# olFi95/image_search

Hardware: AMD Instinct MI355X
Metric: images/sec embedded (ViT-L/14 b=256) + queries/sec cosine top-10 over 10M x 768 (higher is better)
Workload: dtype bf16; 1 GPU; BASELINE config 4: per step, H2D of a pinned batch of 256 224x224x3 f32 images -> bf16 ViT-L/14 (random-init seeded weights) -> 256 rows appended to the table on the device -> cosine top-10 query over 10000000+ x 768 fp32 rows per GPU -> D2H of the k results; fused on HIP streams (the upload runs under the previous batch's tower; the scan is asynchronous to the host and runs between towers); query; batch=256, rows_per_gpu=10000000, k=10

## Files before the change

image_search_amd/_lib.py:

```python
from __future__ import annotations

import ctypes
import os

_PKG = os.path.dirname(os.path.abspath(__file__))
LIB_PATH = os.path.join(_PKG, "libmi355clip.so")

c_f = ctypes.POINTER(ctypes.c_float)
c_u64p = ctypes.POINTER(ctypes.c_uint64)
c_u8p = ctypes.POINTER(ctypes.c_uint8)
c_vp = ctypes.c_void_p



class KnnWhere(ctypes.Structure):
    _fields_ = [("all_of", ctypes.c_uint64), ("any_of", ctypes.c_uint64), ("none_of", ctypes.c_uint64),
                ("stamp_lo", ctypes.c_int64), ("stamp_hi", ctypes.c_int64), ("group", ctypes.c_uint32), ("flags", ctypes.c_uint32)]


c_wherep = ctypes.POINTER(KnnWhere)
MI_KNN_WHERE_GROUP = 1

SYMBOLS = {
    "mi_last_error": (ctypes.c_char_p, []),
    "mi_abi_version": (ctypes.c_int, []),
    "mi_device_count": (ctypes.c_int, []),
    "mi_clip_load": (ctypes.c_int, [ctypes.c_char_p, ctypes.c_int, ctypes.c_int, ctypes.POINTER(c_vp)]),
    "mi_clip_free": (None, [c_vp]),
    "mi_weights_list": (ctypes.c_int, [ctypes.c_char_p, ctypes.c_char_p, ctypes.c_size_t, ctypes.POINTER(ctypes.c_size_t)]),
    "mi_clip_set_option": (ctypes.c_int, [c_vp, ctypes.c_char_p, ctypes.c_int]),
    "mi_clip_info": (ctypes.c_int, [c_vp, ctypes.POINTER(ctypes.c_uint32)]),
    "mi_clip_ln_fold_stats": (ctypes.c_int, [c_vp, ctypes.POINTER(ctypes.c_uint64), ctypes.c_int]),
    "mi_clip_embed": (ctypes.c_int, [c_vp, c_vp, ctypes.c_size_t, c_vp]),
    "mi_clip_embed_device": (ctypes.c_int, [c_vp, c_vp, ctypes.c_size_t, c_vp, c_vp]),
    "mi_clip_embed_rgb8": (ctypes.c_int, [c_vp, c_vp, ctypes.c_size_t, c_vp]),
    "mi_clip_load_text": (ctypes.c_int, [ctypes.c_char_p, ctypes.c_int, ctypes.c_int, ctypes.POINTER(c_vp)]),
    "mi_clip_embed_text": (ctypes.c_int, [c_vp, c_vp, ctypes.c_size_t, c_vp]),
    "mi_preprocess_rgb8": (ctypes.c_int, [c_vp, ctypes.c_size_t, ctypes.c_uint32, ctypes.c_uint32, c_vp]),
    "mi_resize_catmullrom_rgb8": (ctypes.c_int, [ctypes.c_int, c_vp, ctypes.c_uint32, ctypes.c_uint32, ctypes.c_uint32,
                                                 ctypes.c_uint32, c_vp]),
    "mi_image_prepare_resnet": (ctypes.c_int, [ctypes.c_int, c_vp, ctypes.c_uint32, ctypes.c_uint32, c_vp]),
    "mi_clip_embed_images": (ctypes.c_int, [c_vp, ctypes.POINTER(c_vp), ctypes.POINTER(ctypes.c_uint32),
                                            ctypes.POINTER(ctypes.c_uint32), ctypes.c_size_t, c_vp]),
    "mi_knn_create": (ctypes.c_int, [ctypes.c_uint32, ctypes.c_int, ctypes.POINTER(c_vp)]),
    "mi_knn_free": (None, [c_vp]),
    "mi_knn_set_base": (ctypes.c_int, [c_vp, ctypes.c_uint64]),
    "mi_knn_set_option": (ctypes.c_int, [c_vp, ctypes.c_char_p, ctypes.c_int]),
    "mi_knn_prefilter_stats": (ctypes.c_int, [c_vp, c_vp, c_vp]),
    "mi_knn_prefilter_state": (ctypes.c_int, [c_vp, ctypes.POINTER(ctypes.c_uint32)]),
    "mi_knn_reserve": (ctypes.c_int, [c_vp, ctypes.c_uint64]),
    "mi_knn_size": (ctypes.c_int, [c_vp, c_u64p]),
    "mi_knn_append": (ctypes.c_int, [c_vp, c_vp, ctypes.c_uint64]),
    "mi_knn_append_device": (ctypes.c_int, [c_vp, c_vp, ctypes.c_uint64, c_vp]),
    "mi_knn_append_synthetic": (ctypes.c_int, [c_vp, ctypes.c_uint64, ctypes.c_uint64, ctypes.c_uint64]),
    "mi_knn_get_rows": (ctypes.c_int, [c_vp, ctypes.c_uint64, ctypes.c_uint64, c_vp]),
    "mi_knn_save": (ctypes.c_int, [c_vp, ctypes.c_char_p]),
    "mi_knn_load": (ctypes.c_int, [c_vp, ctypes.c_char_p]),
    "mi_knn_delete": (ctypes.c_int, [c_vp, c_vp, ctypes.c_uint64, c_u64p]),
    "mi_knn_deleted": (ctypes.c_int, [c_vp, c_vp, ctypes.c_uint64, c_u64p]),
    "mi_knn_search": (ctypes.c_int, [c_vp, c_vp, ctypes.c_uint32, ctypes.c_uint32, c_vp, c_vp]),
    "mi_knn_search_device": (ctypes.c_int, [c_vp, c_vp, ctypes.c_uint32, ctypes.c_uint32, c_vp, c_vp, c_vp]),
    "mi_knn_search_batched_device": (ctypes.c_int, [c_vp, c_vp, ctypes.c_uint32, ctypes.c_uint32, c_vp, c_vp, c_vp]),
    "mi_knn_search_filtered": (ctypes.c_int, [c_vp, c_vp, ctypes.c_uint32, ctypes.c_uint32, c_vp, ctypes.c_uint64, c_vp, c_vp]),
    "mi_knn_near_pairs": (ctypes.c_int, [c_vp, ctypes.c_float, ctypes.c_uint64, c_vp, c_vp, c_vp, ctypes.c_uint64, c_u64p]),
    "mi_knn_near_pairs_stats": (ctypes.c_int, [c_vp, c_u64p]),
    "mi_knn_assign": (ctypes.c_int, [c_vp, c_vp, ctypes.c_uint32, c_vp, c_vp]),
    "mi_knn_assign_stats": (ctypes.c_int, [c_vp, c_u64p]),
    "mi_knn_assign_multi": (ctypes.c_int, [c_vp, c_vp, ctypes.c_uint32, ctypes.c_uint32, ctypes.c_float, c_vp, c_vp]),
    "mi_knn_assign_multi_stats": (ctypes.c_int, [c_vp, c_u64p]),
    "mi_knn_search_many": (ctypes.c_int, [c_vp, c_vp, ctypes.c_uint32, ctypes.c_uint32, c_vp, c_vp]),
    "mi_knn_search_many_stats": (ctypes.c_int, [c_vp, c_u64p]),
    "mi_knn_neighbors": (ctypes.c_int, [c_vp, ctypes.c_uint64, ctypes.c_uint64, ctypes.c_uint32, c_vp, c_vp]),
    "mi_knn_kmeans": (ctypes.c_int, [c_vp, c_vp, ctypes.c_uint32, ctypes.c_uint32, c_vp, c_vp, ctypes.POINTER(ctypes.c_uint32),
                                     c_u64p, ctypes.POINTER(ctypes.c_double)]),
    "mi_knn_kmeans_seed": (ctypes.c_int, [c_vp, ctypes.c_uint32, ctypes.c_uint64, c_vp, ctypes.c_uint64, c_vp, c_vp,
                                          ctypes.POINTER(ctypes.c_double)]),
    "mi_knn_kmeans_seed_stats": (ctypes.c_int, [c_vp, c_u64p]),
    "mi_knn_search_diverse": (ctypes.c_int, [c_vp, c_vp, ctypes.c_uint32, ctypes.c_uint32, ctypes.c_float, c_vp, ctypes.c_uint64,
                                             c_vp, c_vp, c_vp, c_vp, ctypes.POINTER(ctypes.c_uint32)]),
    "mi_knn_search_diverse_stats": (ctypes.c_int, [c_vp, c_u64p]),
    "mi_knn_search_compound": (ctypes.c_int, [c_vp, c_vp, ctypes.c_uint32, ctypes.c_int, c_vp, c_vp, ctypes.c_uint32, ctypes.c_uint32,
                                              c_vp, ctypes.c_uint64, c_vp, c_vp, c_vp]),
    "mi_knn_search_compound_stats": (ctypes.c_int, [c_vp, c_u64p]),
    "mi_knn_search_page": (ctypes.c_int, [c_vp, c_vp, ctypes.c_uint32, ctypes.c_float, ctypes.c_uint64, ctypes.c_float, c_vp,
                                          ctypes.c_uint64, c_vp, c_vp, c_vp]),
    "mi_knn_set_groups": (ctypes.c_int, [c_vp, c_vp, ctypes.c_uint64, c_vp]),
    "mi_knn_get_groups": (ctypes.c_int, [c_vp, c_vp, ctypes.c_uint64, c_vp]),
    "mi_knn_groups_info": (ctypes.c_int, [c_vp, c_u64p]),
    "mi_knn_search_grouped": (ctypes.c_int, [c_vp, c_vp, ctypes.c_uint32, ctypes.c_float, c_vp, ctypes.c_uint64, c_vp, c_vp, c_vp, c_vp,
                                             c_vp, ctypes.c_uint64, c_vp]),
    "mi_knn_set_attrs": (ctypes.c_int, [c_vp, c_vp, ctypes.c_uint64, c_vp, c_vp]),
    "mi_knn_get_attrs": (ctypes.c_int, [c_vp, c_vp, ctypes.c_uint64, c_vp, c_vp]),
    "mi_knn_count_where": (ctypes.c_int, [c_vp, c_wherep, c_u64p]),
    "mi_knn_rows_where": (ctypes.c_int, [c_vp, c_wherep, c_vp, ctypes.c_uint64, c_u64p]),
    "mi_knn_search_where": (ctypes.c_int, [c_vp, c_vp, ctypes.c_uint32, ctypes.c_uint32, c_wherep, c_vp, c_vp, c_u64p]),
    "mi_pairs_to_groups": (ctypes.c_int, [c_vp, c_vp, ctypes.c_uint64, c_vp, ctypes.c_uint64, c_vp, ctypes.c_uint64, c_u64p,
                                          c_u64p]),
    "mi_index_duplicates": (ctypes.c_int, [c_vp, ctypes.c_float, ctypes.c_uint64, ctypes.c_uint64, c_vp, ctypes.c_uint64, c_vp,
                                           ctypes.c_uint64, c_u64p, c_u64p]),
    "mi_knn_sharded_create": (ctypes.c_int, [ctypes.c_uint32, ctypes.POINTER(ctypes.c_int), ctypes.c_int, ctypes.c_uint32,
                                             ctypes.POINTER(c_vp)]),
    "mi_knn_sharded_free": (None, [c_vp]),
    "mi_knn_sharded_info": (ctypes.c_int, [c_vp, c_u64p, ctypes.POINTER(ctypes.c_uint32), ctypes.POINTER(ctypes.c_uint32),
                                           ctypes.POINTER(ctypes.c_int)]),
    "mi_knn_sharded_stats": (ctypes.c_int, [c_vp, c_u64p]),
    "mi_knn_sharded_reserve": (ctypes.c_int, [c_vp, ctypes.c_uint64]),
    "mi_knn_sharded_set_option": (ctypes.c_int, [c_vp, ctypes.c_char_p, ctypes.c_int]),
    "mi_knn_sharded_append": (ctypes.c_int, [c_vp, c_vp, ctypes.c_uint64, c_u64p]),
    "mi_knn_sharded_append_device": (ctypes.c_int, [c_vp, c_vp, ctypes.c_uint64, ctypes.c_int, c_vp, c_u64p]),
    "mi_knn_sharded_shard": (c_vp, [c_vp, ctypes.c_uint32]),
    "mi_knn_sharded_search_async": (ctypes.c_int, [c_vp, c_vp, ctypes.c_uint32, ctypes.c_uint32, c_vp, c_vp]),
    "mi_knn_sharded_sync": (ctypes.c_int, [c_vp]),
    "mi_knn_sharded_rebalance": (ctypes.c_int, [c_vp, c_vp]),
    "mi_knn_sharded_append_synthetic": (ctypes.c_int, [c_vp, ctypes.c_uint64, ctypes.c_uint64, ctypes.c_uint64]),
    "mi_knn_sharded_get_rows": (ctypes.c_int, [c_vp, ctypes.c_uint64, ctypes.c_uint64, c_vp]),
    "mi_knn_sharded_search": (ctypes.c_int, [c_vp, c_vp, ctypes.c_uint32, ctypes.c_uint32, c_vp, c_vp]),
    "mi_knn_sharded_save": (ctypes.c_int, [c_vp, ctypes.c_char_p]),
    "mi_knn_sharded_load": (ctypes.c_int, [c_vp, ctypes.c_char_p]),
    "mi_knn_sharded_delete": (ctypes.c_int, [c_vp, c_vp, ctypes.c_uint64, c_u64p]),
    "mi_knn_sharded_deleted": (ctypes.c_int, [c_vp, c_vp, ctypes.c_uint64, c_u64p]),
    "mi_knn_sharded_search_filtered": (ctypes.c_int, [c_vp, c_vp, ctypes.c_uint32, ctypes.c_uint32, c_vp, ctypes.c_uint64, c_vp,
                                                      c_vp]),
    "mi_knn_sharded_search_compound": (ctypes.c_int, [c_vp, c_vp, ctypes.c_uint32, ctypes.c_int, c_vp, c_vp, ctypes.c_uint32,
                                                      ctypes.c_uint32, c_vp, ctypes.c_uint64, c_vp, c_vp]),
    "mi_knn_sharded_search_page": (ctypes.c_int, [c_vp, c_vp, ctypes.c_uint32, ctypes.c_float, ctypes.c_uint64, ctypes.c_float, c_vp,
                                                  ctypes.c_uint64, c_vp, c_vp, c_vp]),
    "mi_knn_sharded_set_groups": (ctypes.c_int, [c_vp, c_vp, ctypes.c_uint64, c_vp]),
    "mi_knn_sharded_get_groups": (ctypes.c_int, [c_vp, c_vp, ctypes.c_uint64, c_vp]),
    "mi_knn_sharded_groups_info": (ctypes.c_int, [c_vp, c_u64p]),
    "mi_knn_sharded_search_grouped": (ctypes.c_int, [c_vp, c_vp, ctypes.c_uint32, ctypes.c_float, c_vp, ctypes.c_uint64, c_vp, c_vp,
                                                     c_vp, c_vp, c_vp, ctypes.c_uint64, c_vp]),
    "mi_knn_sharded_set_attrs": (ctypes.c_int, [c_vp, c_vp, ctypes.c_uint64, c_vp, c_vp]),
# ... 115 lines not shown
```

image_search_amd/csrc/handles.h:

```cpp
#pragma once
#include <mutex>
#include <vector>

#include "common.h"

namespace mi {
typedef unsigned short bf16_t;

struct Layer {
    float *ln1w, *ln1b, *ln2w, *ln2b;
    void *wqkv, *wo, *w1, *w2;
    float *bqkv, *bo, *b1, *b2;
    void *wqkv_f = nullptr, *w1_f = nullptr;
    float *cqkv = nullptr, *bqkv_f = nullptr, *c1 = nullptr, *b1_f = nullptr;
};


}

struct mi_clip {
    int device = 0, precision = 0;
    int image = 0, patch = 0, grid = 0, S = 0, D = 0, L = 0, H = 0, FF = 0, E = 0, Kp = 0;
    float eps = 1e-5f;
    std::vector<void*> allocs;
// ... 40 lines not shown
    uint8_t* d_img_src[2] = {nullptr, nullptr};
    float* d_img_tmp = nullptr;
    size_t img_src_cap = 0, img_tmp_cap = 0;
    hipStream_t copy_stream = nullptr;
    hipEvent_t ev_up[2] = {nullptr, nullptr}, ev_used[2] = {nullptr, nullptr};
    hipStream_t stream = nullptr;
    size_t max_batch = 256;
    bool split_ln = false;
    int attn_ver = 2;
    bool q_prescaled = false;
    bool attn_shift = false;
    int qkv_pad = 128;
    int qkv_layout = 0;
    bool front_overlap = false;
    bool store_nt = true;
    bool attn_nt = false;
    int attn_order = 1;
    bool full_last = false;
    bool split_tail = true;
    int gemm_order = 4;
    bool text_fast = true;
    bool attn_f32_mfma = true;
    bool text_fuse = true;
    int ln_nt = 0;
    bool im2col_rows = true;
    mi::WorkOrder order;
    std::mutex mu;
};


struct mi_knn {
    int device = 0;
    uint32_t dim = 0;
    uint64_t base = 0, rows = 0, cap = 0;
    uint32_t cyc_block = 0, cyc_n = 0, cyc_rank = 0;
    float* table = nullptr;
    hipStream_t stream = nullptr;
    int n_cu = 0;
    float* d_q = nullptr;
    uint64_t* d_cand = nullptr;
    uint64_t* d_tmp = nullptr;
    uint64_t* d_keys = nullptr;
    uint64_t* d_idx = nullptr;
    float* d_dist = nullptr;
    size_t cand_keys = 0, tmp_keys = 0, keys_cap = 0, idx_cap = 0, dist_cap = 0;
    bool select_path = true;
    uint32_t* d_keys32 = nullptr;
    uint32_t* d_sel = nullptr;
    size_t keys32_cap = 0, sel_cap = 0;
    int prefilter = 0;
    int coarse_ring = 8;
    bool last_prefiltered = false;
    uint16_t* d_mirror = nullptr;
    float* d_scale8 = nullptr;
    float* d_cfac8 = nullptr;
    float* d_rho8 = nullptr;
    float* d_g8 = nullptr;
    bool g8_ready = false;
    size_t scale8_cap = 0, cfac8_cap = 0, rho8_cap = 0, g8_cap = 0;
    float* d_xx = nullptr;
    bool batch_stage1_mfma = true;
    int8_t* d_digits = nullptr;
    float* d_qs = nullptr;
    size_t digits_cap = 0, qs_cap = 0;
    int pref_sample = 1;
    uint32_t* d_skeys = nullptr;
    size_t skeys_cap = 0;
    uint64_t mirror_rows = 0;
    size_t mirror_cap = 0, xx_cap = 0;
    uint64_t g8_rows = 0;
    static constexpr int PREF_RING = 8, PREF_SKIP = 64;
    bool pref_adaptive = true;
    uint32_t* h_pref_ring = nullptr;
    hipEvent_t pref_ev[PREF_RING] = {};
    bool pref_ev_pending[PREF_RING] = {};
    uint32_t pref_consec = 0, pref_skip_left = 0;
    bool pref_probing = false;
    uint32_t pref_probes_left = 0, pref_reports_due = 0;
    uint64_t pref_seq = 0, pref_skipped = 0;
    uint32_t* d_pref_rows = nullptr;
    uint64_t* d_pref_keys = nullptr;
    uint32_t* d_pref_flag = nullptr;
    size_t pref_rows_cap = 0, pref_keys_cap = 0, pref_flag_cap = 0;
    mi::WorkOrder writes, reads;
    std::vector<uint32_t> dead;
    uint64_t* d_tomb = nullptr;
    uint32_t* d_dead = nullptr;
    size_t tomb_words = 0, dead_cap = 0;
    uint32_t* h_flist = nullptr;
    size_t n_flist = 0, h_flist_cap = 0;
    uint32_t* d_flist = nullptr;
    size_t flist_cap = 0;
    uint32_t join_cap = 1u << 22;
    uint64_t join_stats[4] = {0, 0, 0, 0};
    uint64_t assign_stats[4] = {0, 0, 0, 0};
    uint64_t assign_multi_stats[4] = {0, 0, 0, 0};
    uint64_t search_many_stats[4] = {0, 0, 0, 0};
    int many_segments = 0, many_sample = 0;
    uint64_t kmeans_seed_stats[4] = {0, 0, 0, 0};
    uint64_t diverse_stats[4] = {0, 0, 0, 0};
    uint64_t compound_stats[4] = {0, 0, 0, 0};
    int compound_blocks = 0;
    int page_blocks = 0;
    uint32_t* d_groups = nullptr;
    size_t groups_cap = 0;
    std::vector<uint32_t> h_groups;
    uint32_t n_groups = 0;
    uint64_t n_grouped = 0, groups_epoch = 0;
    uint32_t* d_gslots = nullptr;
    uint32_t* d_gwin = nullptr;
    size_t gslots_cap = 0, gwin_cap = 0;
    bool gslots_valid = false;
    uint32_t gslots_groups = 0;
    int group_blocks = 0, group_lds_max = 4096;
    uint64_t* d_tags = nullptr;
    int64_t* d_stamps = nullptr;
    size_t attrs_cap = 0;
    std::vector<uint64_t> h_tags;
    std::vector<int64_t> h_stamps;
    uint32_t* d_wcounts = nullptr;
    size_t wcounts_cap = 0;
    uint64_t* h_wtotal = nullptr;
    int where_chunk = 0;
    std::mutex mu;
};


typedef struct ncclComm* ncclComm_t;
namespace mi {
struct DevBuf {
    void* p = nullptr;
    size_t cap = 0;
    void reserve(size_t b) {
        if (b <= cap) return;
        if (p) HIP_CHECK(hipFree(p));
        p = nullptr; cap = 0;
        HIP_CHECK(hipMalloc(&p, b));
        cap = b;
    }
};
struct PinnedBuf2 {
    void* p = nullptr;
    size_t cap = 0;
    void reserve(size_t b) {
        if (b <= cap) return;
        if (p) HIP_CHECK(hipHostFree(p));
        p = nullptr; cap = 0;
        HIP_CHECK(hipHostMalloc(&p, b, hipHostMallocPortable));
        cap = b;
    }
};
struct ShardedSlot {
    std::vector<DevBuf> d_q, d_rec;
    std::vector<DevBuf> g_rec;
    DevBuf m_rec;
    PinnedBuf2 h_q, h_rec;
    std::vector<hipEvent_t> ev;
    hipEvent_t done = nullptr;
    uint32_t nq = 0, k = 0;
    uint64_t* user_idx = nullptr;
    float* user_dist = nullptr;
    bool busy = false;
};
}

struct mi_knn_sharded {
    static constexpr int N_SLOTS = 8;
    uint32_t dim = 0, block = 0;
    uint64_t rows = 0;
    std::vector<int> devices;
    std::vector<mi_knn*> shard;
    mi::ShardedSlot slots[N_SLOTS];
    int next_slot = 0;
    std::vector<ncclComm_t> comms;
    bool use_rccl = false;
    struct { uint64_t searches = 0, collectives = 0, copies = 0, merges = 0; } stats;
    uint64_t generation = 0;
    std::vector<hipEvent_t> ev_src;
    std::mutex mu;
    uint32_t n() const { return (uint32_t)shard.size(); }
};

namespace mi {
hipStream_t clip_own_stream(mi_clip* m);
void clip_ensure_workspace(mi_clip* m, size_t n);
void clip_ensure_copy_stream(mi_clip* m);
void clip_forward(mi_clip* m, const float* d_img, size_t n, float* d_out, hipStream_t s, hipStream_t front = nullptr);
hipStream_t knn_own_stream(mi_knn* t);
void knn_grow(mi_knn* t, uint64_t want_rows);
void knn_search_one(mi_knn* t, const float* d_q, uint32_t k, uint64_t* d_idx, float* d_dist, hipStream_t s);
void knn_search_many(mi_knn* t, const float* d_q, uint32_t nq, uint32_t k, uint64_t* d_idx, float* d_dist, hipStream_t s);
void knn_truncate(mi_knn* t, uint64_t rows);
void knn_search_filtered_many(mi_knn* t, const float* d_q, uint32_t nq, uint32_t k, const uint64_t* ids, uint64_t n_ids,
                              uint64_t* d_idx, float* d_dist, hipStream_t s);
void knn_reserve(mi_knn* t, void** p, size_t* have, size_t want, size_t elem);
void knn_filter_rows(mi_knn* t, const uint64_t* ids, uint64_t n_ids);
void knn_filter_upload(mi_knn* t, hipStream_t s);
void knn_filtered_many(mi_knn* t, const float* d_q, uint32_t nq, uint32_t k, uint64_t* d_idx, float* d_dist, hipStream_t s);
void knn_reduce_lists64(mi_knn* t, uint32_t lists, uint32_t k, uint64_t* keys_out, hipStream_t s);
void knn_select_keys32(mi_knn* t, uint64_t n, uint32_t k, uint64_t* keys_out, const uint32_t* list, hipStream_t s);
void knn_merge_lists_device(const uint64_t* d_idx_in, const float* d_dist_in, uint32_t lists, uint32_t nq, uint32_t k,
                            size_t idx_stride, size_t dist_stride, uint64_t* d_idx, float* d_dist, hipStream_t s);
void knn_search_compound(mi_knn* t, const float* pos, uint32_t n_pos, int mode, const float* neg, const float* neg_within, uint32_t n_neg,
                         uint32_t k, const uint64_t* among, uint64_t n_among, uint64_t* idx, float* dist, float* term_dist);
void knn_search_page(mi_knn* t, const float* q, uint32_t k, bool cursor_is_id, float after_dist, uint64_t after_id, uint64_t first_key,
                     float max_dist, const uint64_t* among, uint64_t n_among, uint64_t* idx, float* dist, uint64_t* counts);
void knn_page_scan_keys32(mi_knn* t, hipStream_t s, uint64_t n, const uint32_t* list, const uint64_t* tomb, uint64_t hi, uint32_t k,
                          uint32_t* keys32, unsigned long long* counts);
void knn_groups_fit(mi_knn* t);
void knn_search_grouped(mi_knn* t, const float* q, uint32_t k, float max_dist, const uint64_t* among, uint64_t n_among, uint64_t* idx,
                        float* dist, uint32_t* group, uint64_t* members, uint64_t* facets, uint64_t cap_facets, uint64_t* totals,
                        std::vector<uint32_t>* cnt_out);
void knn_grouped_members(mi_knn* t, const uint32_t* group, uint32_t k, uint32_t* out);
void knn_attrs_fit(mi_knn* t);
void knn_filter_where(mi_knn* t, const mi_knn_where* w, hipStream_t s);
void sharded_place(const mi_knn_sharded* t, uint64_t r, uint32_t* s, uint64_t* local);
uint64_t sharded_rows_of(const mi_knn_sharded* t, uint64_t total, uint32_t s);
void sharded_search_enqueue(mi_knn_sharded* t, const float* q, uint32_t nq, uint32_t k, uint64_t* idx, float* dist,
                            const std::vector<std::vector<uint64_t>>* filter = nullptr,
                            const mi_knn_where* where = nullptr);
void sharded_deliver_all(mi_knn_sharded* t);
}
```

image_search_amd/csrc/knn.hip:

```cpp
#include <algorithm>
#include <cmath>
#include <cstdio>
#include <cstring>
#include <unistd.h>

#include <iterator>
#include <mutex>
#include <string>
#include <vector>

#include "common.h"
#include "handles.h"
#include "knn_kernels.h"
#include "where_host.h"

using namespace mi;

namespace {

constexpr int MAX_BATCH_Q = 8;

IdMap id_map(const mi_knn* t) { return IdMap{t->base, t->cyc_block, t->cyc_n, t->cyc_rank}; }

void ensure(mi_knn* t, void** p, size_t* have, size_t want, size_t elem) {
// ... 113 lines not shown
    const uint64_t off = id - t->base;
    uint64_t l = off;
    if (t->cyc_n > 1 && t->cyc_block) {
        const uint64_t b = off / t->cyc_block;
        if (b % t->cyc_n != t->cyc_rank) return false;
        l = (b / t->cyc_n) * t->cyc_block + off % t->cyc_block;
    }
    if (l >= t->rows) return false;
    *local = l;
    return true;
}

void grow(mi_knn* t, uint64_t want_rows) {
    if (want_rows <= t->cap) return;
    uint64_t ncap = std::max<uint64_t>(want_rows, t->cap + t->cap / 2);
    ncap = (ncap + 63) & ~63ull;
    if (ncap > 0xFFFFFFFFull) fail(MI_ERR_UNSUPPORTED, "a shard holds at most 2^32-1 rows (asked %llu)",
                                    (unsigned long long)want_rows);
    t->writes.sync();
    t->reads.sync();
    float* nt = nullptr;
    HIP_CHECK(hipMalloc((void**)&nt, ncap * t->dim * sizeof(float)));
    if (t->rows) {
        HIP_CHECK(hipMemcpyAsync(nt, t->table, t->rows * t->dim * sizeof(float), hipMemcpyDeviceToDevice, own_stream(t)));
        HIP_CHECK(hipStreamSynchronize(t->stream));
    }
    if (t->table) HIP_CHECK(hipFree(t->table));
    t->table = nt;
    t->cap = ncap;
    if (t->d_tomb) tomb_fit(t);
    if (t->d_groups) groups_fit(t);
    if (t->d_tags) attrs_fit(t);
}

template <class K>
void allow_lds(K kernel, size_t bytes) {
    if (bytes > 48 * 1024)
        HIP_CHECK(hipFuncSetAttribute(reinterpret_cast<const void*>(kernel),
                                      hipFuncAttributeMaxDynamicSharedMemorySize, (int)bytes));
}

template <class Top>
void launch_scan(mi_knn* t, const float* d_q, uint32_t k, const uint64_t* lo, uint64_t* cand, uint32_t blocks,
                 hipStream_t s, const uint32_t* run_if = nullptr, uint32_t gy = 1, QGroup qg = QGroup{}) {
    const size_t lds = (size_t)4 * Top::LDS_KEYS * sizeof(uint64_t);
    const uint64_t* tomb = tomb_of(t);
    switch (t->dim / 64) {
#define MI_CASE(NCH)                                                                                   \
    case NCH:                                                                                          \
        if (tomb) {                                                                                    \
            allow_lds(knn_scan_kernel<NCH, Top, 0, true>, lds);                                        \
            hipLaunchKernelGGL((knn_scan_kernel<NCH, Top, 0, true>), dim3(blocks, gy), dim3(256), lds, s, \
                               t->table, t->rows, d_q, k, lo, cand, (uint32_t*)nullptr, run_if, qg, tomb); \
            break;                                                                                     \
        }                                                                                              \
        allow_lds(knn_scan_kernel<NCH, Top>, lds);                                                     \
        hipLaunchKernelGGL((knn_scan_kernel<NCH, Top>), dim3(blocks, gy), dim3(256), lds, s, t->table, \
                           t->rows, d_q, k, lo, cand, (uint32_t*)nullptr, run_if, qg);                 \
        break;
        MI_CASE(1) MI_CASE(2) MI_CASE(4) MI_CASE(8) MI_CASE(12) MI_CASE(16)
#undef MI_CASE
        default: fail(MI_ERR_UNSUPPORTED, "dim %u: built for dim/64 in {1,2,4,8,12,16}", t->dim);
    }
    HIP_CHECK(hipGetLastError());
}

template <class Top>
void launch_merge(const uint64_t* in, uint32_t n_lists, uint32_t k, uint32_t lpb, uint64_t* out, uint32_t nq,
                  size_t in_stride, size_t out_stride, hipStream_t s, const uint32_t* run_if = nullptr, uint32_t run_stride = 0) {
    const size_t lds = (size_t)4 * Top::LDS_KEYS * sizeof(uint64_t);
    allow_lds(knn_merge_kernel<Top>, lds + 4096);
    const uint32_t blocks = (n_lists + lpb - 1) / lpb;
    hipLaunchKernelGGL((knn_merge_kernel<Top>), dim3(blocks, nq), dim3(256), lds, s, in, n_lists, k, lpb, out,
                       in_stride, out_stride, run_if, run_stride);
    HIP_CHECK(hipGetLastError());
}

template <class Top>
void reduce_wave_lists(mi_knn* t, uint32_t lists, uint32_t kp, uint64_t* keys_out, hipStream_t s, const uint32_t* run_if,
                       uint32_t gy, const QGroup& qg);

template <class Top>
void one_pass(mi_knn* t, const float* d_q, uint32_t kp, const uint64_t* lo, uint64_t* keys_out, hipStream_t s,
              const uint32_t* run_if = nullptr, uint32_t gy = 1, QGroup qg = QGroup{}) {
    const uint32_t bpc = Top::LDS_KEYS == 0 ? 4 : (Top::KP <= 256 ? 4 : 2);
    const uint64_t n_tiles = (t->rows + 63) / 64;
    uint32_t blocks = (uint32_t)std::min<uint64_t>((uint64_t)t->n_cu * bpc, (n_tiles + 3) / 4);
    blocks = std::max(blocks, 1u);
    const uint32_t lists = blocks * 4;
    ensure(t, (void**)&t->d_cand, &t->cand_keys, (size_t)lists * kp * gy, sizeof(uint64_t));
    qg.lists = (uint64_t)lists * kp;
    launch_scan<Top>(t, d_q, kp, lo, t->d_cand, blocks, s, run_if, gy, qg);
    reduce_wave_lists<Top>(t, lists, kp, keys_out, s, run_if, gy, qg);
}

template <class Top>
void reduce_wave_lists(mi_knn* t, uint32_t lists, uint32_t kp, uint64_t* keys_out, hipStream_t s, const uint32_t* run_if,
                       uint32_t gy, const QGroup& qg) {
    if constexpr (Top::LDS_KEYS != 0) {
        constexpr uint32_t LPB = 16;
        ensure(t, (void**)&t->d_tmp, &t->tmp_keys, (size_t)2 * ((lists + LPB - 1) / LPB) * kp, sizeof(uint64_t));
        const uint64_t* in = t->d_cand;
        uint32_t n = lists, lvl = 0;
        while (true) {
            const uint32_t nb = (n + LPB - 1) / LPB;
            uint64_t* out = nb == 1 ? keys_out : t->d_tmp + (size_t)(lvl & 1) * ((lists + LPB - 1) / LPB) * kp;
            hipLaunchKernelGGL((knn_merge_block_kernel<Top::KP>), dim3(nb), dim3(256), 0, s, in, n, kp, LPB, out);
            HIP_CHECK(hipGetLastError());
            if (nb == 1) break;
            in = out; n = nb; ++lvl;
        }
        return;
    }
    if (lists <= 64) {
        launch_merge<Top>(t->d_cand, lists, kp, lists, keys_out, gy, qg.lists, qg.out, s, run_if, qg.flags);
    } else {
        const uint32_t lpb = 32, mid = (lists + lpb - 1) / lpb;
        ensure(t, (void**)&t->d_tmp, &t->tmp_keys, (size_t)mid * kp * gy, sizeof(uint64_t));
        launch_merge<Top>(t->d_cand, lists, kp, lpb, t->d_tmp, gy, qg.lists, (size_t)mid * kp, s, run_if, qg.flags);
        launch_merge<Top>(t->d_tmp, mid, kp, mid, keys_out, gy, (size_t)mid * kp, qg.out, s, run_if, qg.flags);
    }
}

constexpr uint64_t PREF_MIN_ROWS = 1u << 18;
bool prefilter_applies(const mi_knn* t, uint32_t k) {
    const uint32_t width = t->prefilter == 2 ? 256u : 128u;
    return t->prefilter && (k <= 64 || (k <= 4096 && t->select_path)) && t->dim % width == 0 && t->rows >= PREF_MIN_ROWS;
}
template <int NCH>
void launch_coarse8_batched(mi_knn* t, const uint8_t* m8, const float* d_q, float e0, uint32_t nq, uint32_t blocks, hipStream_t s,
                            int sample_shift = 0, uint64_t sample_stride = 0) {
    if constexpr (NCH == 12) {
        if (t->batch_stage1_mfma) {
            hipLaunchKernelGGL(knn_query_digits_kernel, dim3(nq), dim3(256), 0, s, d_q, t->d_g8, (int)t->dim, t->d_digits, t->d_qs, t->d_rho8);
            constexpr int LDS = c8m_lds_bytes(NCH * 64);
            const uint64_t n_tiles = (t->rows + 15) / 16;
            const uint32_t grid = (uint32_t)std::max<uint64_t>(1, std::min<uint64_t>((uint64_t)t->n_cu, (n_tiles + 3) / 4));
#define MI_C8M(NBLK, QPB)                                                                                                         \
    {                                                                                                                             \
        allow_lds(knn_scan_coarse8_mfma_kernel<NCH, NBLK, QPB>, LDS);                                                             \
        hipLaunchKernelGGL((knn_scan_coarse8_mfma_kernel<NCH, NBLK, QPB>), dim3(grid), dim3(256), LDS, s, m8, t->d_xx, t->d_scale8, \
                           t->d_cfac8, t->rows, t->d_digits, t->d_qs, (int)nq, e0, t->d_keys32, (uint64_t)t->cap,                 \
                           sample_shift ? t->d_skeys : (uint32_t*)nullptr, sample_shift, sample_stride);                          \
    }
            if (nq <= 5) MI_C8M(1, 5)
            else if (nq <= 10) MI_C8M(2, 5)
            else if (nq <= 15) MI_C8M(3, 5)
            else MI_C8M(4, 4)
#undef MI_C8M
            HIP_CHECK(hipGetLastError());
            return;
        }
        if (nq == 8)
            hipLaunchKernelGGL((knn_scan_coarse8_batched_kernel<NCH, 8>), dim3(blocks), dim3(256), 0, s, m8, t->d_xx, t->d_scale8, t->d_cfac8,
                               t->d_g8, t->rows, d_q, e0, t->d_keys32, (uint64_t)t->cap, t->d_rho8);
        else if (nq == 2)
            hipLaunchKernelGGL((knn_scan_coarse8_batched_kernel<NCH, 2>), dim3(blocks), dim3(256), 0, s, m8, t->d_xx, t->d_scale8, t->d_cfac8,
                               t->d_g8, t->rows, d_q, e0, t->d_keys32, (uint64_t)t->cap, t->d_rho8);
        else
            hipLaunchKernelGGL((knn_scan_coarse8_batched_kernel<NCH, 4>), dim3(blocks), dim3(256), 0, s, m8, t->d_xx, t->d_scale8, t->d_cfac8,
                               t->d_g8, t->rows, d_q, e0, t->d_keys32, (uint64_t)t->cap, t->d_rho8);
    } else {
        fail(MI_ERR_UNSUPPORTED, "the batched two-stage search is built for dim 768");
    }
}
constexpr uint32_t SEL_WORDS = 6 * SEL_BINS + 64;
constexpr uint32_t KNN_GROUP_MAX = 16;
uint32_t group_size(const mi_knn* t, uint32_t left) {
    if (t->batch_stage1_mfma) return std::min(left, KNN_GROUP_MAX);
    return left >= 8 ? 8 : left >= 4 ? 4 : 2;
}
QGroup group_of(const mi_knn* t, uint32_t gy) {
    QGroup g;
    if (gy <= 1) return g;
    g.q = t->dim; g.keys = t->cap; g.sel = SEL_WORDS; g.flags = 4; g.rows = (uint64_t)2 * PREF_CAP; g.coll = 4096; g.out = 4096; g.rho = 1;
    return g;
}
uint32_t* prefilter_pass(mi_knn* t, const float* d_q, uint32_t k, hipStream_t s, uint32_t nq_batch = 0) {
    const uint32_t gy = std::max(1u, nq_batch);
    const QGroup qg = group_of(t, gy);
    ensure(t, (void**)&t->d_keys32, &t->keys32_cap, (size_t)t->cap * gy, sizeof(uint32_t));
    ensure(t, (void**)&t->d_sel, &t->sel_cap, (size_t)SEL_WORDS * gy, sizeof(uint32_t));
    ensure(t, (void**)&t->d_cand, &t->cand_keys, (size_t)4096 * gy, sizeof(uint64_t));
    ensure(t, (void**)&t->d_pref_rows, &t->pref_rows_cap, (size_t)2 * PREF_CAP * gy, sizeof(uint32_t));
    ensure(t, (void**)&t->d_pref_keys, &t->pref_keys_cap, (size_t)4096 * gy, sizeof(uint64_t));
    ensure(t, (void**)&t->d_pref_flag, &t->pref_flag_cap, (size_t)4 * gy, sizeof(uint32_t));
    const bool bytes = t->prefilter == 2;
    const uint32_t tile_rows = (nq_batch && t->batch_stage1_mfma) ? 16 : 64;
    const uint64_t n_tiles_s = (t->rows + tile_rows - 1) / tile_rows;
    int sample_shift = (bytes && t->pref_sample && k <= 64 && ((nq_batch >= 2 && t->batch_stage1_mfma) || (nq_batch == 0 && t->pref_sample >= 2))) ? 3 : 0;
    uint64_t n_sample = ((n_tiles_s + (1u << sample_shift) - 1) >> sample_shift) * tile_rows;
    if (sample_shift && (t->rows >> sample_shift) < std::max<uint64_t>(4096, 64ull * k)) { sample_shift = 0; n_sample = 0; }
    const uint64_t sample_stride = sample_shift ? ((((t->cap + tile_rows - 1) / tile_rows + (1u << sample_shift) - 1) >> sample_shift) * tile_rows + 63) / 64 * 64 : 0;
    if (sample_shift) ensure(t, (void**)&t->d_skeys, &t->skeys_cap, (size_t)sample_stride * gy, sizeof(uint32_t));
    const size_t mirror_elems = bytes ? ((size_t)t->cap * t->dim + 1) / 2 : (size_t)t->cap * t->dim;
    t->mirror_rows = std::min(t->mirror_rows, t->rows);
    if (bytes && t->g8_ready && t->rows >= 4 * std::max<uint64_t>(t->g8_rows, 1)) t->g8_ready = false;
    if (bytes && !t->g8_ready) t->mirror_rows = 0;
    const size_t keep_m = bytes ? ((size_t)t->mirror_rows * t->dim + 1) / 2 : (size_t)t->mirror_rows * t->dim;
    ensure_keep(t, (void**)&t->d_mirror, &t->mirror_cap, mirror_elems, sizeof(uint16_t), keep_m);
    ensure_keep(t, (void**)&t->d_xx, &t->xx_cap, (size_t)t->cap, sizeof(float), (size_t)t->mirror_rows);
    if (bytes) {
        ensure_keep(t, (void**)&t->d_scale8, &t->scale8_cap, (size_t)t->cap, sizeof(float), (size_t)t->mirror_rows);
        ensure_keep(t, (void**)&t->d_cfac8, &t->cfac8_cap, (size_t)t->cap, sizeof(float), (size_t)t->mirror_rows);
        ensure(t, (void**)&t->d_rho8, &t->rho8_cap, (size_t)KNN_GROUP_MAX, sizeof(float));
        ensure(t, (void**)&t->d_digits, &t->digits_cap, (size_t)KNN_GROUP_MAX * 3 * t->dim + 64, sizeof(int8_t));
        ensure(t, (void**)&t->d_qs, &t->qs_cap, (size_t)KNN_GROUP_MAX * 4, sizeof(float));
        ensure(t, (void**)&t->d_g8, &t->g8_cap, (size_t)2 * t->dim, sizeof(float));
        if (!t->g8_ready) {
            const uint64_t sample = std::min<uint64_t>(t->rows, 1u << 16), stride = t->rows / sample;
            HIP_CHECK(hipMemsetAsync(t->d_g8 + t->dim, 0, t->dim * sizeof(float), s));
            hipLaunchKernelGGL(knn_channel_sumsq_kernel, dim3(256), dim3(256), 0, s, t->table, sample, stride, (int)t->dim, t->d_g8 + t->dim);
            hipLaunchKernelGGL(knn_channel_scale_kernel, dim3((t->dim + 255) / 256), dim3(256), 0, s, t->d_g8 + t->dim, sample,
                               (int)t->dim, t->d_g8);
            t->g8_ready = true;
            t->g8_rows = t->rows;
        }
    }
    const uint64_t n_tiles = (t->rows + 63) / 64;
    const uint32_t blocks = std::max<uint32_t>(1u, (uint32_t)std::min<uint64_t>((uint64_t)t->n_cu * 4, (n_tiles + 3) / 4));
    const uint32_t hb1 = (uint32_t)std::min<uint64_t>((uint64_t)t->n_cu * 8, (t->rows + 255) / 256);
    const uint32_t hb = std::max<uint32_t>(std::min<uint32_t>(hb1, (uint32_t)t->n_cu), (hb1 + gy - 1) / gy);
    uint32_t* flags = t->d_pref_flag;
    uint32_t* key32 = t->d_pref_rows + PREF_CAP;
    uint32_t* count2 = t->d_sel + 6 * SEL_BINS;
    SelState* states = reinterpret_cast<SelState*>(t->d_sel + 6 * SEL_BINS + 4);
    const size_t sel_bytes = (size_t)SEL_WORDS * gy * sizeof(uint32_t);
    HIP_CHECK(hipMemsetAsync(t->d_sel, 0, sel_bytes, s));
    HIP_CHECK(hipMemsetAsync(flags, 0, (size_t)4 * gy * sizeof(uint32_t), s));
    static const uint32_t ring8_bpc = [] { const char* e = std::getenv("MI_KNN_RING_BPC"); return e ? (uint32_t)std::max(1, std::atoi(e)) : 2u; }();
    const float e0 = 4.1f * (float)(t->dim + 8) * 0x1p-24f + 2e-6f;
    const float eps = 0x1p-8f + e0;
    const uint64_t* tomb = tomb_of(t);
    auto kill_keys = [&] {
        if (!tomb) return;
        const uint32_t nd = (uint32_t)t->dead.size();
        hipLaunchKernelGGL(knn_tomb_keys_kernel, dim3(std::max(1u, std::min<uint32_t>((nd + 255) / 256, (uint32_t)t->n_cu * 4))), dim3(256), 0, s,
                           t->d_dead, nd, t->rows, t->d_keys32, (uint64_t)t->cap, gy, sample_shift ? t->d_skeys : (uint32_t*)nullptr,
                           sample_stride, sample_shift, tile_rows);
    };
    if (bytes) {
        uint8_t* m8 = reinterpret_cast<uint8_t*>(t->d_mirror);
        const uint32_t* keys_q = t->d_keys32;
        const uint32_t* keys_h = sample_shift ? t->d_skeys : keys_q;
        const uint64_t n_h = sample_shift ? n_sample : t->rows;
        QGroup qgh = qg;
        if (sample_shift && gy > 1) qgh.keys = sample_stride;
        const uint32_t hbh = sample_shift ? std::max<uint32_t>(1u, (uint32_t)std::min<uint64_t>(hb, (n_h + 1023) / 1024)) : hb;
        switch (t->dim / 64) {
#define MI_CASE(NCH)                                                                                                     \
    case NCH:                                                                                                            \
        if (t->mirror_rows < t->rows) {                                                                                  \
            const uint64_t todo = t->rows - t->mirror_rows;                                                              \
            const uint32_t mb = (uint32_t)std::min<uint64_t>((uint64_t)t->n_cu * 8, (todo + 15) / 16);                   \
            hipLaunchKernelGGL((knn_mirror8_kernel<NCH>), dim3(std::max(mb, 1u)), dim3(256), 0, s, t->table, t->mirror_rows, \
                               t->rows, t->d_g8, m8, t->d_xx, t->d_scale8, t->d_cfac8);                                  \
            t->mirror_rows = t->rows;                                                                                    \
        }                                                                                                                \
        if (nq_batch == 0 && t->coarse_ring == 8)   \
            hipLaunchKernelGGL((knn_scan_coarse8_kernel<NCH, 8>), dim3(std::min(blocks, (uint32_t)t->n_cu * ring8_bpc)), dim3(256), 0, s, m8, t->d_xx, t->d_scale8, \
                               t->d_cfac8, t->d_g8, t->rows, d_q, e0, t->d_keys32, t->d_rho8,                            \
                               sample_shift ? t->d_skeys : (uint32_t*)nullptr, sample_shift);                            \
        else if (nq_batch == 0)                                                                                          \
            hipLaunchKernelGGL((knn_scan_coarse8_kernel<NCH, 4>), dim3(blocks), dim3(256), 0, s, m8, t->d_xx, t->d_scale8, \
                               t->d_cfac8, t->d_g8, t->rows, d_q, e0, t->d_keys32, t->d_rho8,                            \
                               sample_shift ? t->d_skeys : (uint32_t*)nullptr, sample_shift);                            \
        else                                                                                                             \
            launch_coarse8_batched<NCH>(t, m8, d_q, e0, nq_batch, blocks, s, sample_shift, sample_stride);               \
        kill_keys();                                                                                                     \
        for (int p = 0; p < 3; ++p)                                                                                      \
            hipLaunchKernelGGL(knn_select_hist_kernel, dim3(hbh, gy), dim3(256), 0, s, keys_h, n_h, k, p, t->d_sel, states, \
                               (const uint32_t*)nullptr, (const uint32_t*)nullptr, (const uint32_t*)nullptr, qgh, 0);    \
        hipLaunchKernelGGL(knn_prefilter_collect8_kernel, dim3(hb, gy), dim3(256), 0, s, keys_q, t->d_cfac8, t->rows, k, \
                           t->d_sel, states, t->d_rho8, e0, PREF_CAP, t->d_pref_rows, flags, qg, tomb);                  \
        hipLaunchKernelGGL((knn_rescore_kernel<NCH>), dim3(t->n_cu * (gy > 1 ? 2 : 8), gy), dim3(256), 0, s, t->table, d_q, \
                           t->d_pref_rows, flags, PREF_CAP, key32, qg);                                                  \
        break;
            MI_CASE(4) MI_CASE(8) MI_CASE(12) MI_CASE(16)
#undef MI_CASE
            default: fail(MI_ERR_UNSUPPORTED, "dim %u: the byte prefilter is built for dim/64 in {4,8,12,16}", t->dim);
        }
    } else
    switch (t->dim / 64) {
#define MI_CASE(NCH)                                                                                                     \
    case NCH:                                                                                                            \
        if (t->mirror_rows < t->rows) {                                                                                  \
            const uint64_t todo = t->rows - t->mirror_rows;                                                              \
            const uint32_t mb = (uint32_t)std::min<uint64_t>((uint64_t)t->n_cu * 8, (todo + 15) / 16);                   \
            hipLaunchKernelGGL((knn_mirror_kernel<NCH>), dim3(std::max(mb, 1u)), dim3(256), 0, s, t->table, t->mirror_rows, \
                               t->rows, t->d_mirror, t->d_xx);                                                           \
            t->mirror_rows = t->rows;                                                                                    \
        }                                                                                                                \
        hipLaunchKernelGGL((knn_scan_coarse_kernel<NCH>), dim3(blocks), dim3(256), 0, s, t->d_mirror, t->d_xx, t->rows,  \
                           d_q, t->d_keys32);                                                                            \
        kill_keys();                                                                                                     \
        for (int p = 0; p < 3; ++p)                                                                                      \
            hipLaunchKernelGGL(knn_select_hist_kernel, dim3(hb), dim3(256), 0, s, t->d_keys32, t->rows, k, p, t->d_sel, states); \
        hipLaunchKernelGGL(knn_prefilter_collect_kernel, dim3(hb), dim3(256), 0, s, t->d_keys32, t->rows, k, t->d_sel,   \
                           states, 2.0f * eps, PREF_CAP, t->d_pref_rows, flags, tomb);                                   \
        hipLaunchKernelGGL((knn_rescore_kernel<NCH>), dim3(t->n_cu * 8), dim3(256), 0, s, t->table, d_q, t->d_pref_rows, \
                           flags, PREF_CAP, key32);                                                                      \
        break;
        MI_CASE(2) MI_CASE(4) MI_CASE(8) MI_CASE(12) MI_CASE(16)
#undef MI_CASE
        default: fail(MI_ERR_UNSUPPORTED, "dim %u: the prefilter is built for dim/64 in {2,4,8,12,16}", t->dim);
    }
    HIP_CHECK(hipMemsetAsync(t->d_sel, 0, sel_bytes, s));
    const uint32_t* go = flags + 2;
    const uint32_t cb = (uint32_t)t->n_cu * 2;
    for (int p = 0; p < 6; ++p)
        hipLaunchKernelGGL(knn_select_hist_kernel, dim3(cb, gy), dim3(256), 0, s, key32, (uint64_t)PREF_CAP, k, p, t->d_sel, states, go, flags,
                           t->d_pref_rows, qg, 1);
    hipLaunchKernelGGL(knn_select_collect_kernel, dim3(cb, gy), dim3(256), 0, s, key32, (uint64_t)PREF_CAP, k, t->d_sel, states, t->d_cand, count2,
                       go, flags, t->d_pref_rows, qg, 1);
    hipLaunchKernelGGL(knn_select_sort_kernel, dim3(1, gy), dim3(1024), 0, s, t->d_cand, count2, k, t->d_pref_keys, go, qg);
    HIP_CHECK(hipGetLastError());
    return flags + 1;
}

void select_pass(mi_knn* t, const float* d_q, uint32_t k, uint64_t* keys_out, hipStream_t s, const uint32_t* run_if = nullptr, uint32_t gy = 1) {
    const QGroup qg = group_of(t, gy);
    const uint64_t n_tiles = (t->rows + 63) / 64;
    uint32_t blocks = (uint32_t)std::min<uint64_t>((uint64_t)t->n_cu * 4, (n_tiles + 3) / 4);
    blocks = std::max(blocks, 1u);
    ensure(t, (void**)&t->d_keys32, &t->keys32_cap, (size_t)t->cap * gy, sizeof(uint32_t));
    ensure(t, (void**)&t->d_sel, &t->sel_cap, (size_t)SEL_WORDS * gy, sizeof(uint32_t));
    ensure(t, (void**)&t->d_cand, &t->cand_keys, (size_t)4096 * gy, sizeof(uint64_t));
    HIP_CHECK(hipMemsetAsync(t->d_sel, 0, (size_t)SEL_WORDS * gy * sizeof(uint32_t), s));
    const uint64_t* tomb = tomb_of(t);
    const uint64_t n_dead = t->dead.size();
    switch (t->dim / 64) {
#define MI_CASE(NCH)                                                                                          \
    case NCH:                                                                                                 \
        hipLaunchKernelGGL((knn_scan_kernel<NCH, WaveTopReg, 1>), dim3(blocks, gy), dim3(256), 0, s, t->table, t->rows, d_q, k, \
                           (const uint64_t*)nullptr, (uint64_t*)nullptr, t->d_keys32, run_if, qg);            \
        break;
        MI_CASE(1) MI_CASE(2) MI_CASE(4) MI_CASE(8) MI_CASE(12) MI_CASE(16)
#undef MI_CASE
        default: fail(MI_ERR_UNSUPPORTED, "dim %u: built for dim/64 in {1,2,4,8,12,16}", t->dim);
    }
    HIP_CHECK(hipGetLastError());
    if (tomb) {
        const uint32_t nd = (uint32_t)t->dead.size();
        hipLaunchKernelGGL(knn_tomb_keys_kernel, dim3(std::max(1u, std::min<uint32_t>((nd + 255) / 256, (uint32_t)t->n_cu * 4))), dim3(256), 0, s,
                           t->d_dead, nd, t->rows, t->d_keys32, (uint64_t)t->cap, gy, (uint32_t*)nullptr, (uint64_t)0, 0, 64u);
        HIP_CHECK(hipGetLastError());
    }
    const uint32_t hb = (uint32_t)std::min<uint64_t>((uint64_t)t->n_cu * 8, (t->rows + 255) / 256);
    uint32_t* count = t->d_sel + 6 * SEL_BINS;
    SelState* states = reinterpret_cast<SelState*>(t->d_sel + 6 * SEL_BINS + 4);
    for (int p = 0; p < 6; ++p)
        hipLaunchKernelGGL(knn_select_hist_kernel, dim3(hb, gy), dim3(256), 0, s, t->d_keys32, t->rows, k, p, t->d_sel, states, run_if,
                           (const uint32_t*)nullptr, (const uint32_t*)nullptr, qg, 0, tomb, n_dead);
    hipLaunchKernelGGL(knn_select_collect_kernel, dim3(hb, gy), dim3(256), 0, s, t->d_keys32, t->rows, k, t->d_sel, states, t->d_cand, count, run_if,
                       (const uint32_t*)nullptr, (const uint32_t*)nullptr, qg, 0, tomb, n_dead);
    hipLaunchKernelGGL(knn_select_sort_kernel, dim3(1, gy), dim3(1024), 0, s, t->d_cand, count, k, keys_out, run_if, qg);
    HIP_CHECK(hipGetLastError());
}

void pref_window(mi_knn* t) {
    t->pref_skip_left = mi_knn::PREF_SKIP;
    t->pref_consec = 0;
    t->pref_probing = false;
}
void pref_fold(mi_knn* t, uint32_t cand, uint32_t fell_back) {
    t->pref_consec = fell_back ? t->pref_consec + 1 : 0;
    if (t->pref_probing) {
        if (t->pref_reports_due && --t->pref_reports_due == 0) {
            if (t->pref_consec >= 2) pref_window(t);
            else t->pref_probing = false;
        }
        return;
    }
    (void)cand;
    if (t->pref_consec >= 2) pref_window(t);
}
void pref_poll(mi_knn* t) {
    for (uint64_t q = t->pref_seq >= (uint64_t)mi_knn::PREF_RING ? t->pref_seq - mi_knn::PREF_RING : 0; q < t->pref_seq; ++q) {
        const int i = (int)(q % mi_knn::PREF_RING);
        if (!t->pref_ev_pending[i]) continue;
        if (hipEventQuery(t->pref_ev[i]) != hipSuccess) { (void)hipGetLastError(); break; }
        t->pref_ev_pending[i] = false;
        pref_fold(t, t->h_pref_ring[2 * i], t->h_pref_ring[2 * i + 1]);
    }
}
void pref_record(mi_knn* t, hipStream_t s) {
    if (!t->h_pref_ring) HIP_CHECK(hipHostMalloc((void**)&t->h_pref_ring, (size_t)mi_knn::PREF_RING * 2 * sizeof(uint32_t), hipHostMallocDefault));
    const int i = (int)(t->pref_seq % mi_knn::PREF_RING);
    if (t->pref_ev_pending[i]) {
        if (t->pref_probing && t->pref_reports_due && --t->pref_reports_due == 0) t->pref_probing = false;
        return;
    }
    if (!t->pref_ev[i]) HIP_CHECK(hipEventCreateWithFlags(&t->pref_ev[i], hipEventDisableTiming));
    HIP_CHECK(hipMemcpyAsync(t->h_pref_ring + 2 * i, t->d_pref_flag, 2 * sizeof(uint32_t), hipMemcpyDeviceToHost, s));
    HIP_CHECK(hipEventRecord(t->pref_ev[i], s));
    t->pref_ev_pending[i] = true;
    ++t->pref_seq;
}
void pref_reset(mi_knn* t) {
    for (int i = 0; i < mi_knn::PREF_RING; ++i) {
        if (t->pref_ev_pending[i]) (void)hipEventSynchronize(t->pref_ev[i]);
        t->pref_ev_pending[i] = false;
    }
    t->pref_consec = t->pref_skip_left = 0;
    t->pref_probing = false;
    t->pref_probes_left = t->pref_reports_due = 0;
}

uint32_t reg_pass_lists(const mi_knn* t) {
    const uint64_t n_tiles = (t->rows + 63) / 64;
    return 4 * std::max<uint32_t>(1u, (uint32_t)std::min<uint64_t>((uint64_t)t->n_cu * 4, (n_tiles + 3) / 4));
}

void two_stage(mi_knn* t, const float* d_q, uint32_t k, uint64_t* d_idx, float* d_dist, hipStream_t s, uint32_t nq_batch) {
    const uint32_t gy = std::max(1u, nq_batch);
    const QGroup qg = group_of(t, gy);
    if (k <= 64) {
        const uint32_t lists = reg_pass_lists(t);
        ensure(t, (void**)&t->d_cand, &t->cand_keys, std::max<size_t>((size_t)4096 * gy, (size_t)lists * k * gy), sizeof(uint64_t));
        if (lists > 64) ensure(t, (void**)&t->d_tmp, &t->tmp_keys, (size_t)((lists + 31) / 32) * k * gy, sizeof(uint64_t));
    }
    const uint32_t* fallback = prefilter_pass(t, d_q, k, s, nq_batch);
    if (k <= 64) one_pass<WaveTopReg>(t, d_q, k, nullptr, t->d_keys, s, fallback, gy, qg);
    else select_pass(t, d_q, k, t->d_keys, s, fallback, gy);
    hipLaunchKernelGGL(knn_finalize_kernel, dim3((k + 255) / 256, gy), dim3(256), 0, s, t->d_keys, k, id_map(t),
                       d_idx, d_dist, (size_t)qg.out, (size_t)(gy > 1 ? k : 0), t->d_pref_keys, fallback, qg.flags);
    HIP_CHECK(hipGetLastError());
}

bool batched_two_stage_applies(mi_knn* t, uint32_t k) {
    if (!(t->prefilter == 2 && t->dim == 768 && prefilter_applies(t, k))) return false;
    if (!t->pref_adaptive) return true;
    pref_poll(t);
    if (t->pref_skip_left) {
        if (k <= 64) {
            if (--t->pref_skip_left == 0) { t->pref_probing = true; t->pref_probes_left = t->pref_reports_due = 2; t->pref_consec = 0; }
            ++t->pref_skipped;
        }
        return false;
    }
    if (t->pref_probing) {
        if (t->pref_probes_left) { --t->pref_probes_left; return true; }
        if (k <= 64) ++t->pref_skipped;
        return false;
    }
    return true;
}
void search_batched_two_stage(mi_knn* t, const float* d_q, uint32_t nq, uint32_t k, uint64_t* d_idx, float* d_dist, hipStream_t s) {
    ensure(t, (void**)&t->d_keys, &t->keys_cap, (size_t)4096 * nq, sizeof(uint64_t));
    t->last_prefiltered = true;
    two_stage(t, d_q, k, d_idx, d_dist, s, nq);
    if (t->pref_adaptive) pref_record(t, s);
}

void search_one(mi_knn* t, const float* d_q, uint32_t k, uint64_t* d_idx, float* d_dist, hipStream_t s) {
    if (t->rows == 0) {
        hipLaunchKernelGGL(knn_finalize_kernel, dim3((k + 255) / 256, 1), dim3(256), 0, s,
                           (const uint64_t*)nullptr, k, id_map(t), d_idx, d_dist, (size_t)0, (size_t)0);
        HIP_CHECK(hipGetLastError());
        return;
    }
    const uint32_t passes = (k + 1023) / 1024;
    ensure(t, (void**)&t->d_keys, &t->keys_cap, (size_t)std::max<uint32_t>(passes * 1024, 4096), sizeof(uint64_t));
    t->last_prefiltered = prefilter_applies(t, k);
    if (t->last_prefiltered && t->pref_adaptive) {
        pref_poll(t);
        if (t->pref_skip_left) {
            if (--t->pref_skip_left == 0) { t->pref_probing = true; t->pref_probes_left = t->pref_reports_due = 2; t->pref_consec = 0; }
            ++t->pref_skipped;
            t->last_prefiltered = false;
        } else if (t->pref_probing) {
            if (t->pref_probes_left) --t->pref_probes_left;
            else { ++t->pref_skipped; t->last_prefiltered = false; }
        }
    }
    if (t->last_prefiltered) {
        two_stage(t, d_q, k, d_idx, d_dist, s, 0);
        if (t->pref_adaptive) pref_record(t, s);
        return;
    }
    if ((k > 64 || tomb_of(t)) && k <= 4096 && t->select_path) {
        select_pass(t, d_q, k, t->d_keys, s);
        hipLaunchKernelGGL(knn_finalize_kernel, dim3((k + 255) / 256, 1), dim3(256), 0, s, t->d_keys, k, id_map(t),
                           d_idx, d_dist, (size_t)0, (size_t)0);
        HIP_CHECK(hipGetLastError());
        return;
    }
    for (uint32_t p = 0; p < passes; ++p) {
        const uint32_t kp = std::min(1024u, k - p * 1024);
        uint64_t* out = t->d_keys + (size_t)p * 1024;
        const uint64_t* lo = p ? out - 1 : nullptr;
        if (kp <= 64) one_pass<WaveTopReg>(t, d_q, kp, lo, out, s);
        else if (kp <= 256) one_pass<WaveTopLds<256>>(t, d_q, kp, lo, out, s);
        else one_pass<WaveTopLds<1024>>(t, d_q, kp, lo, out, s);
    }
    hipLaunchKernelGGL(knn_finalize_kernel, dim3((k + 255) / 256, 1), dim3(256), 0, s, t->d_keys, k, id_map(t),
                       d_idx, d_dist, (size_t)0, (size_t)0);
    HIP_CHECK(hipGetLastError());
}

template <int NQ>
void launch_batched(mi_knn* t, const float* d_q, uint32_t k, uint64_t* cand, uint32_t blocks, hipStream_t s) {
    switch (t->dim / 64) {
        case 12:
            if (const uint64_t* tomb = tomb_of(t))
                hipLaunchKernelGGL((knn_scan_batched_kernel<12, NQ, true>), dim3(blocks), dim3(256), 0, s, t->table, t->rows,
                                   d_q, k, cand, tomb);
            else
                hipLaunchKernelGGL((knn_scan_batched_kernel<12, NQ>), dim3(blocks), dim3(256), 0, s, t->table, t->rows,
                                   d_q, k, cand);
            break;
        default: fail(MI_ERR_UNSUPPORTED, "batched search is built for dim 768 (got %u)", t->dim);
    }
    HIP_CHECK(hipGetLastError());
}

void search_batched(mi_knn* t, const float* d_q, uint32_t nq, uint32_t k, uint64_t* d_idx, float* d_dist,
                    hipStream_t s) {
    const uint64_t n_tiles = (t->rows + 63) / 64;
    uint32_t blocks = (uint32_t)std::min<uint64_t>((uint64_t)t->n_cu * 2, (n_tiles + 3) / 4);
    blocks = std::max(blocks, 1u);
    const uint32_t lists = blocks * 4;
    ensure(t, (void**)&t->d_cand, &t->cand_keys, (size_t)nq * lists * k, sizeof(uint64_t));
    ensure(t, (void**)&t->d_keys, &t->keys_cap, (size_t)std::max<uint32_t>(1024, nq * k), sizeof(uint64_t));
    if (nq == 2) launch_batched<2>(t, d_q, k, t->d_cand, blocks, s);
    else if (nq == 4) launch_batched<4>(t, d_q, k, t->d_cand, blocks, s);
    else launch_batched<8>(t, d_q, k, t->d_cand, blocks, s);
    const size_t cstride = (size_t)lists * k;
    if (lists <= 64) {
        launch_merge<WaveTopReg>(t->d_cand, lists, k, lists, t->d_keys, nq, cstride, k, s);
    } else {
        const uint32_t lpb = 32, mid = (lists + lpb - 1) / lpb;
        ensure(t, (void**)&t->d_tmp, &t->tmp_keys, (size_t)nq * mid * k, sizeof(uint64_t));
        launch_merge<WaveTopReg>(t->d_cand, lists, k, lpb, t->d_tmp, nq, cstride, (size_t)mid * k, s);
        launch_merge<WaveTopReg>(t->d_tmp, mid, k, mid, t->d_keys, nq, (size_t)mid * k, k, s);
    }
    hipLaunchKernelGGL(knn_finalize_kernel, dim3((k + 255) / 256, nq), dim3(256), 0, s, t->d_keys, k, id_map(t),
                       d_idx, d_dist, (size_t)k, (size_t)k);
    HIP_CHECK(hipGetLastError());
}

void check_search_args(const mi_knn* t, const void* q, uint32_t nq, uint32_t k, const void* idx, const void* dist) {
    if (!t) fail(MI_ERR_INVALID, "null table handle");
    if (nq && (!q || !idx || !dist)) fail(MI_ERR_INVALID, "null query/result pointer");
    if (k == 0) fail(MI_ERR_INVALID, "k must be >= 1");
}

void search_many(mi_knn* t, const float* d_q, uint32_t nq, uint32_t k, uint64_t* d_idx, float* d_dist, hipStream_t s) {
    uint32_t u = 0;
    while (u < nq) {
        const uint32_t left = nq - u;
        if (left >= 2 && t->rows && batched_two_stage_applies(t, k)) {
            const uint32_t b2 = group_size(t, left);
            search_batched_two_stage(t, d_q + (size_t)u * t->dim, b2, k, d_idx + (size_t)u * k, d_dist + (size_t)u * k, s);
            u += b2;
            continue;
        }
        const uint32_t b = (k <= 64 && t->rows && t->dim == 768) ? (left >= 8 ? 8 : left >= 4 ? 4 : left >= 2 ? 2 : 1) : 1;
        if (b == 1) search_one(t, d_q + (size_t)u * t->dim, k, d_idx + (size_t)u * k, d_dist + (size_t)u * k, s);
        else search_batched(t, d_q + (size_t)u * t->dim, b, k, d_idx + (size_t)u * k, d_dist + (size_t)u * k, s);
        u += b;
    }
}

constexpr uint32_t FILTER_K_MAX = 4096;

uint32_t* flist_reserve(mi_knn* t, size_t want) {
    if (want > t->h_flist_cap) {
        if (t->h_flist) HIP_CHECK(hipHostFree(t->h_flist));
        t->h_flist = nullptr;
        t->h_flist_cap = 0;
        const size_t cap = std::max(want, (size_t)4096);
        HIP_CHECK(hipHostMalloc((void**)&t->h_flist, cap * sizeof(uint32_t), hipHostMallocPortable));
        t->h_flist_cap = cap;
    }
    return t->h_flist;
}

void filter_rows(mi_knn* t, const uint64_t* ids, uint64_t n_ids) {
    std::vector<uint32_t> rows((size_t)n_ids);
    for (uint64_t i = 0; i < n_ids; ++i) {
        uint64_t local = 0;
        if (!local_of(t, ids[i], &local))
            fail(MI_ERR_INVALID, "id %llu is not a row of this table (base %llu, %llu rows)", (unsigned long long)ids[i],
                 (unsigned long long)t->base, (unsigned long long)t->rows);
        rows[i] = (uint32_t)local;
    }
    if (n_ids >= t->rows / 1024) {
        std::vector<uint64_t> bits((size_t)((t->rows + 63) / 64), 0ull);
        for (const uint32_t r : rows) bits[r >> 6] |= 1ull << (r & 63);
        for (const uint32_t r : t->dead)
            if (r < t->rows) bits[r >> 6] &= ~(1ull << (r & 63));
        size_t n = 0;
        for (const uint64_t b : bits) n += (size_t)__builtin_popcountll(b);
        uint32_t* out = flist_reserve(t, n);
        size_t at = 0;
        for (size_t w = 0; w < bits.size(); ++w)
            for (uint64_t b = bits[w]; b; b &= b - 1) out[at++] = (uint32_t)(w * 64 + (uint64_t)__builtin_ctzll(b));
        t->n_flist = n;
        return;
    }
    std::sort(rows.begin(), rows.end());
    rows.erase(std::unique(rows.begin(), rows.end()), rows.end());
    uint32_t* out = flist_reserve(t, rows.size());
    t->n_flist = (size_t)(std::set_difference(rows.begin(), rows.end(), t->dead.begin(), t->dead.end(), out) - out);
}

uint32_t gather_blocks(const mi_knn* t, uint32_t n, uint32_t bpc) {
    const uint64_t n_tiles = ((uint64_t)n + 63) / 64;
    return std::max(1u, (uint32_t)std::min<uint64_t>((uint64_t)t->n_cu * bpc, (n_tiles + 3) / 4));
}

template <class Top>
void gather_lists(mi_knn* t, const float* d_q, uint32_t n, uint32_t kp, uint64_t* keys_out, hipStream_t s) {
    const uint32_t blocks = gather_blocks(t, n, Top::LDS_KEYS == 0 ? 4 : (Top::KP <= 256 ? 4 : 2)), lists = blocks * 4;
    ensure(t, (void**)&t->d_cand, &t->cand_keys, (size_t)lists * kp, sizeof(uint64_t));
    const size_t lds = (size_t)4 * Top::LDS_KEYS * sizeof(uint64_t);
    switch (t->dim / 64) {
#define MI_CASE(NCH)                                                                                                    \
    case NCH:                                                                                                           \
        allow_lds(knn_scan_gather_kernel<NCH, Top>, lds);                                                               \
        hipLaunchKernelGGL((knn_scan_gather_kernel<NCH, Top>), dim3(blocks), dim3(256), lds, s, t->table, t->d_flist, n, d_q, kp, \
                           t->d_cand, (uint32_t*)nullptr);                                                              \
        break;
        MI_CASE(1) MI_CASE(2) MI_CASE(4) MI_CASE(8) MI_CASE(12) MI_CASE(16)
#undef MI_CASE
        default: fail(MI_ERR_UNSUPPORTED, "dim %u: built for dim/64 in {1,2,4,8,12,16}", t->dim);
    }
    HIP_CHECK(hipGetLastError());
    QGroup qg;
    qg.lists = (uint64_t)lists * kp;
    reduce_wave_lists<Top>(t, lists, kp, keys_out, s, nullptr, 1, qg);
}

void select_keys32(mi_knn* t, uint64_t n, uint32_t k, uint64_t* keys_out, const uint32_t* list, hipStream_t s) {
    const uint32_t hb = (uint32_t)std::max<uint64_t>(1, std::min<uint64_t>((uint64_t)t->n_cu * 8, (n + 255) / 256));
    uint32_t* count = t->d_sel + 6 * SEL_BINS;
    SelState* states = reinterpret_cast<SelState*>(t->d_sel + 6 * SEL_BINS + 4);
    for (int p = 0; p < 6; ++p)
        hipLaunchKernelGGL(knn_select_hist_kernel, dim3(hb), dim3(256), 0, s, t->d_keys32, n, k, p, t->d_sel, states);
    hipLaunchKernelGGL(knn_select_collect_kernel, dim3(hb), dim3(256), 0, s, t->d_keys32, n, k, t->d_sel, states, t->d_cand, count);
    hipLaunchKernelGGL(knn_select_sort_kernel, dim3(1), dim3(1024), 0, s, t->d_cand, count, k, keys_out);
    if (list) hipLaunchKernelGGL(knn_gather_rows_kernel, dim3((k + 255) / 256), dim3(256), 0, s, keys_out, k, list);
    HIP_CHECK(hipGetLastError());
}

void gather_select(mi_knn* t, const float* d_q, uint32_t n, uint32_t k, uint64_t* keys_out, hipStream_t s) {
    ensure(t, (void**)&t->d_keys32, &t->keys32_cap, (size_t)n, sizeof(uint32_t));
    ensure(t, (void**)&t->d_sel, &t->sel_cap, (size_t)SEL_WORDS, sizeof(uint32_t));
    ensure(t, (void**)&t->d_cand, &t->cand_keys, (size_t)4096, sizeof(uint64_t));
    HIP_CHECK(hipMemsetAsync(t->d_sel, 0, (size_t)SEL_WORDS * sizeof(uint32_t), s));
    const uint32_t blocks = gather_blocks(t, n, 4);
    switch (t->dim / 64) {
#define MI_CASE(NCH)                                                                                                    \
    case NCH:                                                                                                           \
        hipLaunchKernelGGL((knn_scan_gather_kernel<NCH, WaveTopReg, 1>), dim3(blocks), dim3(256), 0, s, t->table, t->d_flist, n, \
                           d_q, k, (uint64_t*)nullptr, t->d_keys32);                                                    \
        break;
        MI_CASE(1) MI_CASE(2) MI_CASE(4) MI_CASE(8) MI_CASE(12) MI_CASE(16)
#undef MI_CASE
        default: fail(MI_ERR_UNSUPPORTED, "dim %u: built for dim/64 in {1,2,4,8,12,16}", t->dim);
    }
    HIP_CHECK(hipGetLastError());
    select_keys32(t, n, k, keys_out, t->d_flist, s);
}

bool filter_takes_lists(const mi_knn* t, uint32_t n, uint32_t k) {
    if (k <= 64) return true;
    if (k > 1024) return false;
    if (!t->select_path) return true;
    const uint64_t waves = 4ull * t->n_cu * 2;
    return (uint64_t)n >= 16ull * k * waves;
}

void filtered_one(mi_knn* t, const float* d_q, uint32_t n, uint32_t k, uint64_t* d_idx, float* d_dist, hipStream_t s) {
    if (n == 0) {
        hipLaunchKernelGGL(knn_finalize_kernel, dim3((k + 255) / 256, 1), dim3(256), 0, s, (const uint64_t*)nullptr, k, id_map(t),
                           d_idx, d_dist, (size_t)0, (size_t)0);
        HIP_CHECK(hipGetLastError());
        return;
    }
    ensure(t, (void**)&t->d_keys, &t->keys_cap, (size_t)FILTER_K_MAX, sizeof(uint64_t));
    if (!filter_takes_lists(t, n, k)) gather_select(t, d_q, n, k, t->d_keys, s);
    else if (k <= 64) gather_lists<WaveTopReg>(t, d_q, n, k, t->d_keys, s);
    else gather_lists<WaveTopLds<1024>>(t, d_q, n, k, t->d_keys, s);
    hipLaunchKernelGGL(knn_finalize_kernel, dim3((k + 255) / 256, 1), dim3(256), 0, s, t->d_keys, k, id_map(t), d_idx, d_dist,
                       (size_t)0, (size_t)0);
    HIP_CHECK(hipGetLastError());
}

void filtered_batched(mi_knn* t, const float* d_q, uint32_t nq, uint32_t n, uint32_t k, uint64_t* d_idx, float* d_dist, hipStream_t s) {
    const uint32_t blocks = gather_blocks(t, n, 2), lists = blocks * 4;
    ensure(t, (void**)&t->d_cand, &t->cand_keys, (size_t)nq * lists * k, sizeof(uint64_t));
    ensure(t, (void**)&t->d_keys, &t->keys_cap, (size_t)std::max<uint32_t>(FILTER_K_MAX, nq * k), sizeof(uint64_t));
    if (nq == 2)
        hipLaunchKernelGGL((knn_scan_gather_batched_kernel<12, 2>), dim3(blocks), dim3(256), 0, s, t->table, t->d_flist, n, d_q, k, t->d_cand);
    else if (nq == 4)
        hipLaunchKernelGGL((knn_scan_gather_batched_kernel<12, 4>), dim3(blocks), dim3(256), 0, s, t->table, t->d_flist, n, d_q, k, t->d_cand);
    else
        hipLaunchKernelGGL((knn_scan_gather_batched_kernel<12, 8>), dim3(blocks), dim3(256), 0, s, t->table, t->d_flist, n, d_q, k, t->d_cand);
    HIP_CHECK(hipGetLastError());
    const size_t cstride = (size_t)lists * k;
    if (lists <= 64) {
        launch_merge<WaveTopReg>(t->d_cand, lists, k, lists, t->d_keys, nq, cstride, k, s);
    } else {
        const uint32_t lpb = 32, mid = (lists + lpb - 1) / lpb;
        ensure(t, (void**)&t->d_tmp, &t->tmp_keys, (size_t)nq * mid * k, sizeof(uint64_t));
        launch_merge<WaveTopReg>(t->d_cand, lists, k, lpb, t->d_tmp, nq, cstride, (size_t)mid * k, s);
        launch_merge<WaveTopReg>(t->d_tmp, mid, k, mid, t->d_keys, nq, (size_t)mid * k, k, s);
    }
    hipLaunchKernelGGL(knn_finalize_kernel, dim3((k + 255) / 256, nq), dim3(256), 0, s, t->d_keys, k, id_map(t), d_idx, d_dist,
                       (size_t)k, (size_t)k);
    HIP_CHECK(hipGetLastError());
}

void upload_filter(mi_knn* t, hipStream_t s) {
    const size_t n = t->n_flist;
    if (n == 0) return;
    ensure(t, (void**)&t->d_flist, &t->flist_cap, n, sizeof(uint32_t));
    HIP_CHECK(hipMemcpyAsync(t->d_flist, t->h_flist, n * sizeof(uint32_t), hipMemcpyHostToDevice, s));
}

void filtered_many(mi_knn* t, const float* d_q, uint32_t nq, uint32_t k, uint64_t* d_idx, float* d_dist, hipStream_t s) {
    const uint32_t n = (uint32_t)t->n_flist;
    uint32_t u = 0;
    while (u < nq) {
        const uint32_t left = nq - u;
        const uint32_t b = (k <= 64 && n && t->dim == 768) ? (left >= 8 ? 8 : left >= 4 ? 4 : left >= 2 ? 2 : 1) : 1;
        if (b == 1) filtered_one(t, d_q + (size_t)u * t->dim, n, k, d_idx + (size_t)u * k, d_dist + (size_t)u * k, s);
        else filtered_batched(t, d_q + (size_t)u * t->dim, b, n, k, d_idx + (size_t)u * k, d_dist + (size_t)u * k, s);
        u += b;
    }
}
}

namespace mi {
void knn_search_filtered_many(mi_knn* t, const float* d_q, uint32_t nq, uint32_t k, const uint64_t* ids, uint64_t n_ids,
                              uint64_t* d_idx, float* d_dist, hipStream_t s) {
    filter_rows(t, ids, n_ids);
    upload_filter(t, s);
    filtered_many(t, d_q, nq, k, d_idx, d_dist, s);
}
hipStream_t knn_own_stream(mi_knn* t) { return own_stream(t); }
void knn_reserve(mi_knn* t, void** p, size_t* have, size_t want, size_t elem) { ensure(t, p, have, want, elem); }
void knn_filter_rows(mi_knn* t, const uint64_t* ids, uint64_t n_ids) { filter_rows(t, ids, n_ids); }
void knn_filter_upload(mi_knn* t, hipStream_t s) { upload_filter(t, s); }
void knn_filtered_many(mi_knn* t, const float* d_q, uint32_t nq, uint32_t k, uint64_t* d_idx, float* d_dist, hipStream_t s) {
    filtered_many(t, d_q, nq, k, d_idx, d_dist, s);
}
void knn_reduce_lists64(mi_knn* t, uint32_t lists, uint32_t k, uint64_t* keys_out, hipStream_t s) {
    QGroup qg;
    qg.lists = (uint64_t)lists * k;
    reduce_wave_lists<WaveTopReg>(t, lists, k, keys_out, s, nullptr, 1, qg);
}
void knn_select_keys32(mi_knn* t, uint64_t n, uint32_t k, uint64_t* keys_out, const uint32_t* list, hipStream_t s) {
    ensure(t, (void**)&t->d_sel, &t->sel_cap, (size_t)SEL_WORDS, sizeof(uint32_t));
    ensure(t, (void**)&t->d_cand, &t->cand_keys, (size_t)4096, sizeof(uint64_t));
    HIP_CHECK(hipMemsetAsync(t->d_sel, 0, (size_t)SEL_WORDS * sizeof(uint32_t), s));
    select_keys32(t, n, k, keys_out, list, s);
}
void knn_search_many(mi_knn* t, const float* d_q, uint32_t nq, uint32_t k, uint64_t* d_idx, float* d_dist, hipStream_t s) {
    search_many(t, d_q, nq, k, d_idx, d_dist, s);
}
void knn_grow(mi_knn* t, uint64_t want_rows) { grow(t, want_rows); }
void knn_groups_fit(mi_knn* t) { groups_fit(t); }
void knn_attrs_fit(mi_knn* t) { attrs_fit(t); }
void knn_search_one(mi_knn* t, const float* d_q, uint32_t k, uint64_t* d_idx, float* d_dist, hipStream_t s) {
    search_one(t, d_q, k, d_idx, d_dist, s);
}
void knn_truncate(mi_knn* t, uint64_t rows) {
    std::lock_guard<std::mutex> l(t->mu);
    if (rows >= t->rows) return;
    t->rows = rows;
    t->mirror_rows = std::min(t->mirror_rows, rows);
    if (t->d_groups && rows < t->groups_cap) {
        DeviceGuard g(t->device);
        t->writes.sync();
        t->reads.sync();
        HIP_CHECK(hipMemsetAsync(t->d_groups + rows, 0xFF, (t->groups_cap - (size_t)rows) * sizeof(uint32_t), own_stream(t)));
        HIP_CHECK(hipStreamSynchronize(t->stream));
        for (size_t r = (size_t)rows; r < t->h_groups.size(); ++r) t->n_grouped -= t->h_groups[r] != MI_KNN_NO_GROUP;
        if (t->h_groups.size() > rows) t->h_groups.resize((size_t)rows);
        ++t->groups_epoch;
    }
    if (t->d_tags && rows < t->attrs_cap) {
        DeviceGuard g(t->device);
        t->writes.sync();
        t->reads.sync();
        HIP_CHECK(hipMemsetAsync(t->d_tags + rows, 0, (t->attrs_cap - (size_t)rows) * sizeof(uint64_t), own_stream(t)));
        HIP_CHECK(hipMemsetAsync(t->d_stamps + rows, 0, (t->attrs_cap - (size_t)rows) * sizeof(int64_t), t->stream));
        HIP_CHECK(hipStreamSynchronize(t->stream));
        if (t->h_tags.size() > rows) t->h_tags.resize((size_t)rows);
        if (t->h_stamps.size() > rows) t->h_stamps.resize((size_t)rows);
    }
    const auto cut = std::lower_bound(t->dead.begin(), t->dead.end(), (uint32_t)std::min<uint64_t>(rows, 0xFFFFFFFFull));
    if (cut != t->dead.end()) {
        t->dead.erase(cut, t->dead.end());
        DeviceGuard g(t->device);
        tomb_rebuild(t);
    }
}
void knn_merge_lists_device(const uint64_t* d_idx_in, const float* d_dist_in, uint32_t lists, uint32_t nq, uint32_t k,
                            size_t idx_stride, size_t dist_stride, uint64_t* d_idx, float* d_dist, hipStream_t s) {
    const uint32_t threads = std::max<uint32_t>(lists * k, k);
    for (uint32_t u0 = 0; u0 < nq; u0 += 65535) {
        const uint32_t nu = std::min<uint32_t>(65535, nq - u0);
        hipLaunchKernelGGL(knn_merge_lists_kernel, dim3((threads + 255) / 256, nu), dim3(256), 0, s, d_idx_in + (size_t)u0 * k,
                           d_dist_in + (size_t)u0 * k, lists, k, idx_stride, dist_stride, d_idx + (size_t)u0 * k, d_dist + (size_t)u0 * k);
        HIP_CHECK(hipGetLastError());
    }
}
}

extern "C" {

int mi_knn_create(uint32_t dim, int device, mi_knn** out) {
    return guarded([&] {
        if (!out) fail(MI_ERR_INVALID, "out is null");
        *out = nullptr;
        if (dim == 0 || dim % 64 != 0) fail(MI_ERR_UNSUPPORTED, "dim must be a positive multiple of 64 (got %u)", dim);
        DeviceGuard g(device);
        auto t = new mi_knn();
        t->device = device; t->dim = dim;
        hipDeviceProp_t prop;
        HIP_CHECK(hipGetDeviceProperties(&prop, device));
        t->n_cu = prop.multiProcessorCount;
        HIP_CHECK(hipMalloc((void**)&t->d_q, (size_t)16 * dim * sizeof(float)));
        if (const char* e = std::getenv("MI_KNN_SELECT")) t->select_path = std::atoi(e) != 0;
        if (const char* e = std::getenv("MI_KNN_RING")) t->coarse_ring = std::atoi(e) == 8 ? 8 : 4;
        if (const char* e = std::getenv("MI_KNN_BATCH_STAGE1")) t->batch_stage1_mfma = std::atoi(e) != 0;
        *out = t;
    });
}

void mi_knn_free(mi_knn* t) {
    if (!t) return;
    (void)hipSetDevice(t->device);
    (void)hipDeviceSynchronize();
    t->writes.destroy();
    t->reads.destroy();
    if (t->stream) { (void)hipStreamSynchronize(t->stream); (void)hipStreamDestroy(t->stream); }
    for (void* p : {(void*)t->table, (void*)t->d_q, (void*)t->d_cand, (void*)t->d_tmp, (void*)t->d_keys,
                    (void*)t->d_idx, (void*)t->d_dist, (void*)t->d_keys32, (void*)t->d_sel, (void*)t->d_mirror,
                    (void*)t->d_xx, (void*)t->d_pref_rows, (void*)t->d_pref_keys, (void*)t->d_pref_flag, (void*)t->d_scale8,
                    (void*)t->d_cfac8, (void*)t->d_rho8, (void*)t->d_g8, (void*)t->d_digits, (void*)t->d_qs, (void*)t->d_skeys, (void*)t->d_tomb, (void*)t->d_dead,
                    (void*)t->d_flist, (void*)t->d_groups, (void*)t->d_gslots, (void*)t->d_gwin, (void*)t->d_tags, (void*)t->d_stamps,
                    (void*)t->d_wcounts})
        if (p) (void)hipFree(p);
    for (hipEvent_t e : t->pref_ev)
        if (e) (void)hipEventDestroy(e);
    if (t->h_pref_ring) (void)hipHostFree(t->h_pref_ring);
    if (t->h_flist) (void)hipHostFree(t->h_flist);
    if (t->h_wtotal) (void)hipHostFree(t->h_wtotal);
    delete t;
}

int mi_knn_set_option(mi_knn* t, const char* key, int value) {
    return guarded([&] {
        if (!t || !key) fail(MI_ERR_INVALID, "null argument");
        std::lock_guard<std::mutex> l(t->mu);
        const std::string k(key);
        if (k == "prefilter") {
            if (value < 0 || value > 2) fail(MI_ERR_INVALID, "prefilter: 0, 1 or 2 (got %d)", value);
            if (value != t->prefilter && t->d_mirror) {
                DeviceGuard g(t->device);
                t->reads.sync();
                for (void** p : {(void**)&t->d_mirror, (void**)&t->d_xx, (void**)&t->d_scale8, (void**)&t->d_cfac8})
                    if (*p) { HIP_CHECK(hipFree(*p)); *p = nullptr; }
                t->mirror_cap = t->xx_cap = t->scale8_cap = t->cfac8_cap = 0;
                t->mirror_rows = 0;
                t->g8_ready = false;
            }
            if (value != t->prefilter) pref_reset(t);
            t->prefilter = value;
        } else if (k == "prefilter_sample") {
            if (value < 0 || value > 2) fail(MI_ERR_INVALID, "prefilter_sample must be 0, 1 or 2");
            t->pref_sample = value;
        } else if (k == "batch_stage1") {
            t->batch_stage1_mfma = value != 0;
        } else if (k == "prefilter_adaptive") {
            pref_reset(t);
            t->pref_adaptive = value != 0;
        } else if (k == "join_cap") {
            if (value < (1 << 14)) fail(MI_ERR_INVALID, "join_cap must be >= 16384 (got %d)", value);
            t->join_cap = (uint32_t)value;
        } else if (k == "many_segments") {
            if (value < 0) fail(MI_ERR_INVALID, "many_segments must be >= 0 (got %d)", value);
            t->many_segments = value;
        } else if (k == "many_sample") {
            if (value < 0) fail(MI_ERR_INVALID, "many_sample must be >= 0 (got %d)", value);
            t->many_sample = value;
        } else if (k == "compound_blocks") {
            if (value < 0) fail(MI_ERR_INVALID, "compound_blocks must be >= 0 (got %d)", value);
            t->compound_blocks = value;
        } else if (k == "page_blocks") {
            if (value < 0) fail(MI_ERR_INVALID, "page_blocks must be >= 0 (got %d)", value);
            t->page_blocks = value;
        } else if (k == "group_blocks") {
            if (value < 0) fail(MI_ERR_INVALID, "group_blocks must be >= 0 (got %d)", value);
            t->group_blocks = value;
        } else if (k == "group_lds_max") {
            if (value < 0 || value > 4096) fail(MI_ERR_INVALID, "group_lds_max must be in [0, 4096] (got %d)", value);
            t->group_lds_max = value;
        } else if (k == "where_chunk") {
            if (!where_chunk_ok(value)) fail(MI_ERR_INVALID, "where_chunk must be 0 or a multiple of 64 up to 65536 (got %d)", value);
            t->where_chunk = value;
        } else {
            fail(MI_ERR_INVALID, "unknown option '%s' (known: prefilter, prefilter_adaptive, prefilter_sample, batch_stage1, join_cap, many_segments, many_sample, compound_blocks, page_blocks, group_blocks, group_lds_max, where_chunk)", key);
        }
    });
}

int mi_knn_prefilter_stats(mi_knn* t, uint32_t* candidates, uint32_t* fell_back) {
    return guarded([&] {
        if (!t || !candidates || !fell_back) fail(MI_ERR_INVALID, "null argument");
        std::lock_guard<std::mutex> l(t->mu);
        *candidates = 0; *fell_back = 0;
        if (!t->last_prefiltered) return;
        DeviceGuard g(t->device);
        t->reads.sync();
        uint32_t w[2] = {0, 0};
        HIP_CHECK(hipMemcpy(w, t->d_pref_flag, sizeof w, hipMemcpyDeviceToHost));
        *candidates = w[0]; *fell_back = w[1];
    });
}

int mi_knn_prefilter_state(mi_knn* t, uint32_t out[4]) {
    return guarded([&] {
        if (!t || !out) fail(MI_ERR_INVALID, "null argument");
        std::lock_guard<std::mutex> l(t->mu);
        DeviceGuard g(t->device);
        t->reads.sync();
        pref_poll(t);
        out[0] = t->pref_skip_left;
        out[1] = t->pref_consec;
        out[2] = (uint32_t)std::min<uint64_t>(t->pref_skipped, 0xFFFFFFFFull);
        out[3] = (uint32_t)std::min<uint64_t>(t->g8_rows, 0xFFFFFFFFull);
    });
}

int mi_knn_set_base(mi_knn* t, uint64_t base) {
    return guarded([&] {
        if (!t) fail(MI_ERR_INVALID, "null table handle");
        std::lock_guard<std::mutex> l(t->mu);
        t->base = base;
    });
}

int mi_knn_reserve(mi_knn* t, uint64_t rows) {
    return guarded([&] {
        if (!t) fail(MI_ERR_INVALID, "null table handle");
        std::lock_guard<std::mutex> l(t->mu);
        DeviceGuard g(t->device);
        grow(t, rows);
    });
}

int mi_knn_size(const mi_knn* t, uint64_t* rows) {
    return guarded([&] {
        if (!t || !rows) fail(MI_ERR_INVALID, "null argument");
        *rows = t->rows;
    });
}

int mi_knn_append(mi_knn* t, const float* rows, uint64_t n) {
    return guarded([&] {
        if (!t) fail(MI_ERR_INVALID, "null table handle");
        if (n == 0) return;
        if (!rows) fail(MI_ERR_INVALID, "rows is null");
        std::lock_guard<std::mutex> l(t->mu);
        DeviceGuard g(t->device);
        own_stream(t);
        grow(t, t->rows + n);
        t->writes.begin(t->stream);
        HIP_CHECK(hipMemcpyAsync(t->table + t->rows * t->dim, rows, n * t->dim * sizeof(float), hipMemcpyHostToDevice,
                                 t->stream));
        t->writes.end(t->stream);
        HIP_CHECK(hipStreamSynchronize(t->stream));
        t->rows += n;
    });
}

int mi_knn_append_device(mi_knn* t, const float* d_rows, uint64_t n, void* stream) {
    return guarded([&] {
        if (!t) fail(MI_ERR_INVALID, "null table handle");
        if (n == 0) return;
        if (!d_rows) fail(MI_ERR_INVALID, "d_rows is null");
        std::lock_guard<std::mutex> l(t->mu);
        DeviceGuard g(t->device);
        hipStream_t s = stream ? (hipStream_t)stream : own_stream(t);
        grow(t, t->rows + n);
        t->writes.begin(s);
        HIP_CHECK(hipMemcpyAsync(t->table + t->rows * t->dim, d_rows, n * t->dim * sizeof(float),
                                 hipMemcpyDeviceToDevice, s));
        t->writes.end(s);
        t->rows += n;
    });
}

int mi_knn_append_synthetic(mi_knn* t, uint64_t seed, uint64_t first_row, uint64_t n) {
    return guarded([&] {
        if (!t) fail(MI_ERR_INVALID, "null table handle");
        if (n == 0) return;
        std::lock_guard<std::mutex> l(t->mu);
        DeviceGuard g(t->device);
        own_stream(t);
// ... 306 lines not shown
```

image_search_amd/csrc/knn_kernels.h:

```cpp
#pragma once
#include <hip/hip_runtime.h>

#include <cstdint>

#include "knn_shared.h"

namespace mi {

typedef __amdgpu_buffer_rsrc_t rsrc_c8;
__device__ __forceinline__ rsrc_c8 c8_rsrc(const void* p, uint32_t bytes) {
    return __builtin_amdgcn_make_buffer_rsrc(const_cast<void*>(p), 0, (int)bytes, 0x00020000);
}
__device__ __forceinline__ void c8_dma16_nt(rsrc_c8 r, uint32_t voff, void* lds_wave_base) {
    __builtin_amdgcn_raw_ptr_buffer_load_lds(r, (__attribute__((address_space(3))) void*)lds_wave_base, 16, voff, 0, 0, 2);
}
__device__ __forceinline__ void c8_dma4(rsrc_c8 r, uint32_t voff, void* lds_wave_base) {
    __builtin_amdgcn_raw_ptr_buffer_load_lds(r, (__attribute__((address_space(3))) void*)lds_wave_base, 4, voff, 0, 0, 0);
}


template <int KP_>
struct WaveTopLds {
    static constexpr int KP = KP_;
    static constexpr int LDS_KEYS = 2 * KP_;
// ... 143 lines not shown
    top.finish();
    top.store(cand + (size_t)wave * k);
}

constexpr int SEL_BINS = 2048;
__device__ __forceinline__ bool tomb_dead(const uint64_t* __restrict__ tomb, uint64_t key) {
    const uint32_t row = (uint32_t)key;
    return (uint32_t)(key >> 32) == 0xFFFFFFFFu && ((tomb[row >> 6] >> (row & 63)) & 1ull);
}
__device__ __forceinline__ int sel_shift(int p) { return p == 0 ? 53 : p == 1 ? 42 : p == 2 ? 32 : p == 3 ? 21 : p == 4 ? 10 : 0; }
__device__ __forceinline__ uint32_t sel_mask(int p) { return (p == 2 || p == 5) ? 0x3FFu : 0x7FFu; }

struct SelState { uint64_t prefix; uint32_t k_rem; int done; int fixed; };
static_assert(sizeof(SelState) == 24, "layout of the state words in d_sel");
__device__ inline SelState sel_advance(const uint32_t* __restrict__ hist, SelState* __restrict__ states, int n_pass, uint32_t k,
                                       uint64_t n_rows) {
    __shared__ uint32_t part[256];
    __shared__ uint32_t s_bin, s_rem, s_cnt;
    SelState st{0ull, k, 0, 0};
    if (n_rows < k) { st.done = 1; return st; }
    if (n_pass == 0) return st;
    if (n_pass >= 2) st = states[n_pass - 2];
    if (st.done) {
        if (threadIdx.x == 0) states[n_pass - 1] = st;
        return st;
    }
    const int p = n_pass - 1;
    const uint32_t* h = hist + p * SEL_BINS;
    uint32_t mine[8], loc = 0;
#pragma unroll
    for (int j = 0; j < 8; ++j) { mine[j] = h[threadIdx.x * 8 + j]; loc += mine[j]; }
    part[threadIdx.x] = loc;
    __syncthreads();
    for (int d = 1; d < 256; d <<= 1) {
        const uint32_t v = threadIdx.x >= (unsigned)d ? part[threadIdx.x - d] : 0u;
        __syncthreads();
        part[threadIdx.x] += v;
        __syncthreads();
    }
    const uint32_t incl = part[threadIdx.x], excl = incl - loc;
    if (excl < st.k_rem && st.k_rem <= incl) {
        uint32_t acc = excl;
        int j = 0;
        while (j < 7 && acc + mine[j] < st.k_rem) acc += mine[j++];
        s_bin = threadIdx.x * 8 + j; s_rem = st.k_rem - acc; s_cnt = mine[j];
    }
    __syncthreads();
    st.prefix |= (uint64_t)s_bin << sel_shift(p);
    st.k_rem = s_rem;
    st.done = s_cnt == s_rem;
    st.fixed = p + 1;
    if (threadIdx.x == 0) states[p] = st;
    __syncthreads();
    return st;
}

__global__ __launch_bounds__(256) void knn_select_hist_kernel(const uint32_t* __restrict__ keys, uint64_t n_rows, uint32_t k,
                                                              int p, uint32_t* __restrict__ hist, SelState* __restrict__ states,
                                                              const uint32_t* __restrict__ run_if = nullptr,
                                                              const uint32_t* __restrict__ n_dev = nullptr,
                                                              const uint32_t* __restrict__ row_of = nullptr, QGroup qg = QGroup{},
                                                              int keys_are_rows = 0, const uint64_t* __restrict__ tomb = nullptr,
                                                              uint64_t n_dead = 0) {
    __shared__ uint32_t lh[SEL_BINS];
    keys += (size_t)blockIdx.y * (keys_are_rows ? qg.rows : qg.keys);
    hist += (size_t)blockIdx.y * qg.sel;
    states = reinterpret_cast<SelState*>(reinterpret_cast<uint32_t*>(states) + (size_t)blockIdx.y * qg.sel);
    if (run_if) run_if += (size_t)blockIdx.y * qg.flags;
    if (n_dev) n_dev += (size_t)blockIdx.y * qg.flags;
    if (row_of) row_of += (size_t)blockIdx.y * qg.rows;
    if (run_if && *run_if == 0u) return;
    if (n_dev) n_rows = min(n_rows, (uint64_t)*n_dev);
    const SelState st = sel_advance(hist, states, p, k, n_rows - n_dead);
    if (st.done) return;
    for (int j = threadIdx.x; j < SEL_BINS; j += 256) lh[j] = 0;
    __syncthreads();
    const int sh = sel_shift(p);
    const uint32_t mk = sel_mask(p);
    const uint64_t hi_mask = p == 0 ? 0ull : ~0ull << sel_shift(p - 1);
    auto count_key = [&](uint64_t key, bool live) {
        if (tomb && live) live = !tomb_dead(tomb, key);
        const bool hit = live && (key & hi_mask) == st.prefix;
        const uint32_t bin = (uint32_t)(key >> sh) & mk;
        const unsigned long long hits = __ballot(hit);
        if (hits == 0ull) return;
        const uint32_t first = __builtin_amdgcn_readfirstlane(__shfl((int)bin, __ffsll((long long)hits) - 1, 64));
        if (__ballot(hit && bin != first) == 0ull) {
            if ((threadIdx.x & 63) == 0) atomicAdd(&lh[first], (uint32_t)__popcll(hits));
        } else if (hit) {
            atomicAdd(&lh[bin], 1u);
        }
    };
    const uint64_t n4 = n_rows >> 2;
    for (uint64_t q4 = (uint64_t)blockIdx.x * 256 + threadIdx.x; q4 < ((n4 + 63) & ~63ull); q4 += (uint64_t)gridDim.x * 256) {
        const bool live = q4 < n4;
        uint4 v = {0u, 0u, 0u, 0u};
        const uint64_t r0 = q4 << 2;
        uint4 lo = {(uint32_t)r0, (uint32_t)(r0 + 1), (uint32_t)(r0 + 2), (uint32_t)(r0 + 3)};
        if (live) {
            v = reinterpret_cast<const uint4*>(keys)[q4];
            if (row_of) lo = reinterpret_cast<const uint4*>(row_of)[q4];
        }
        count_key(((uint64_t)v.x << 32) | lo.x, live);
        count_key(((uint64_t)v.y << 32) | lo.y, live);
        count_key(((uint64_t)v.z << 32) | lo.z, live);
        count_key(((uint64_t)v.w << 32) | lo.w, live);
    }
    if (blockIdx.x == 0 && threadIdx.x < 64) {
        const uint64_t r = (n4 << 2) + threadIdx.x;
        const bool live = threadIdx.x < (n_rows & 3);
        count_key(live ? (((uint64_t)keys[r] << 32) | (row_of ? row_of[r] : (uint32_t)r)) : 0ull, live);
    }
    __syncthreads();
    for (int j = threadIdx.x; j < SEL_BINS; j += 256)
        if (lh[j]) atomicAdd(&hist[p * SEL_BINS + j], lh[j]);
}

__global__ __launch_bounds__(256) void knn_select_collect_kernel(const uint32_t* __restrict__ keys, uint64_t n_rows, uint32_t k,
                                                                 const uint32_t* __restrict__ hist, SelState* __restrict__ states,
                                                                 uint64_t* __restrict__ out, uint32_t* __restrict__ count,
                                                                 const uint32_t* __restrict__ run_if = nullptr,
                                                                 const uint32_t* __restrict__ n_dev = nullptr,
                                                                 const uint32_t* __restrict__ row_of = nullptr, QGroup qg = QGroup{},
                                                                 int keys_are_rows = 0, const uint64_t* __restrict__ tomb = nullptr,
                                                                 uint64_t n_dead = 0) {
    keys += (size_t)blockIdx.y * (keys_are_rows ? qg.rows : qg.keys);
    hist += (size_t)blockIdx.y * qg.sel;
    states = reinterpret_cast<SelState*>(reinterpret_cast<uint32_t*>(states) + (size_t)blockIdx.y * qg.sel);
    out += (size_t)blockIdx.y * qg.coll;
    count += (size_t)blockIdx.y * qg.sel;
    if (run_if) run_if += (size_t)blockIdx.y * qg.flags;
    if (n_dev) n_dev += (size_t)blockIdx.y * qg.flags;
    if (row_of) row_of += (size_t)blockIdx.y * qg.rows;
    if (run_if && *run_if == 0u) return;
    if (n_dev) n_rows = min(n_rows, (uint64_t)*n_dev);
    const SelState st = sel_advance(hist, states, 6, k, n_rows - n_dead);
    uint64_t T = KEY_MAX;
    if (n_rows - n_dead >= k) T = st.fixed == 6 ? st.prefix : (st.prefix | ((1ull << sel_shift(st.fixed - 1)) - 1ull));
    for (uint64_t r = (uint64_t)blockIdx.x * 256 + threadIdx.x; r < n_rows; r += (uint64_t)gridDim.x * 256) {
        const uint64_t key = ((uint64_t)keys[r] << 32) | (row_of ? row_of[r] : (uint32_t)r);
        if (key <= T && !(tomb && tomb_dead(tomb, key))) {
            const uint32_t at = atomicAdd(count, 1u);
            if (at < k) out[at] = key;
        }
    }
}

__global__ __launch_bounds__(1024) void knn_select_sort_kernel(const uint64_t* __restrict__ in, const uint32_t* __restrict__ count,
                                                               uint32_t k, uint64_t* __restrict__ out,
                                                               const uint32_t* __restrict__ run_if = nullptr, QGroup qg = QGroup{}) {
    __shared__ uint64_t buf[4096];
    in += (size_t)blockIdx.y * qg.coll;
    count += (size_t)blockIdx.y * qg.sel;
    out += (size_t)blockIdx.y * qg.out;
    if (run_if) run_if += (size_t)blockIdx.y * qg.flags;
    if (run_if && *run_if == 0u) return;
    const uint32_t n = min(*count, k);
    int np = 64;
    while ((uint32_t)np < k) np <<= 1;
    for (int j = threadIdx.x; j < np; j += 1024) buf[j] = (uint32_t)j < n ? in[j] : KEY_MAX;
    __syncthreads();
    for (int kk = 2; kk <= np; kk <<= 1)
        for (int j = kk >> 1; j > 0; j >>= 1) {
            for (int p = threadIdx.x; p < np / 2; p += 1024) {
                const int a = ((p & ~(j - 1)) << 1) | (p & (j - 1)), b = a | j;
                const uint64_t x = buf[a], y = buf[b];
                const bool up = (a & kk) == 0;
                if ((x > y) == up) { buf[a] = y; buf[b] = x; }
            }
            __syncthreads();
        }
    for (uint32_t j = threadIdx.x; j < k; j += 1024) out[j] = buf[j];
}

#ifndef PREF_DEPTH
#define PREF_DEPTH 3
#endif
constexpr uint32_t PREF_MARK = 0xFFFFFFFEu;
template <int NCH>
__global__ __launch_bounds__(256, 2) void knn_scan_coarse_kernel(const uint16_t* __restrict__ mirror, const float* __restrict__ xx,
                                                              uint64_t n_rows, const float* __restrict__ q,
                                                              uint32_t* __restrict__ all_keys) {
    static_assert(NCH % 2 == 0, "rows of whole 256-byte bf16 chunks");
    constexpr int DIM = NCH * 64, U = NCH / 2;
    const int lane = threadIdx.x & 63, wib = threadIdx.x >> 6;
    const int i = lane & 15, g = lane >> 4;
    const uint32_t wave = blockIdx.x * 4 + wib, n_waves = gridDim.x * 4;
    float qf[U][8];
    float sq;
    {
        float s = 0.0f;
#pragma unroll
        for (int u = 0; u < U; ++u)
#pragma unroll
            for (int e = 0; e < 8; ++e) {
                qf[u][e] = q[128 * u + 8 * i + e];
                s = __builtin_fmaf(qf[u][e], qf[u][e], s);
            }
        sq = sqrtf(row16_sum(s));
    }
    const uint64_t n_tiles = (n_rows + 63) >> 6;
    auto load_row = [&](u32x4 (&x)[U], uint64_t r) {
        r = r < n_rows ? r : n_rows - 1;
        const u32x4* p = reinterpret_cast<const u32x4*>(mirror + r * DIM) + i;
#pragma unroll
        for (int u = 0; u < U; ++u) x[u] = __builtin_nontemporal_load(p + 16 * u);
    };
    for (uint64_t tile = wave; tile < n_tiles; tile += n_waves) {
        float mydot = 0.0f;
        const uint64_t row0 = (tile << 6) + 16 * g;
        auto reduce_row = [&](const u32x4 (&x)[U], int it) {
            float a[8] = {0.0f, 0.0f, 0.0f, 0.0f, 0.0f, 0.0f, 0.0f, 0.0f};
#pragma unroll
            for (int u = 0; u < U; ++u) {
                const uint32_t w[4] = {x[u].x, x[u].y, x[u].z, x[u].w};
#pragma unroll
                for (int j = 0; j < 4; ++j) {
                    a[2 * j] = __builtin_fmaf(qf[u][2 * j], __uint_as_float(w[j] << 16), a[2 * j]);
                    a[2 * j + 1] = __builtin_fmaf(qf[u][2 * j + 1], __uint_as_float(w[j] & 0xFFFF0000u), a[2 * j + 1]);
                }
            }
            const float d = row16_sum(((a[0] + a[1]) + (a[2] + a[3])) + ((a[4] + a[5]) + (a[6] + a[7])));
            if (i == it) mydot = d;
        };
        u32x4 xr[PREF_DEPTH][U];
#pragma unroll
        for (int d = 0; d < PREF_DEPTH - 1; ++d) load_row(xr[d], row0 + d);
#pragma unroll
        for (int it = 0; it < 16; ++it) {
            if (it + PREF_DEPTH - 1 < 16) load_row(xr[(it + PREF_DEPTH - 1) % PREF_DEPTH], row0 + it + PREF_DEPTH - 1);
            reduce_row(xr[it % PREF_DEPTH], it);
        }
        const uint64_t r = (tile << 6) + lane;
        if (r < n_rows) {
            const float s = xx[r];
            all_keys[r] = s < 0.0f ? PREF_MARK : dist_to_u32(1.0f - mydot / (sq * sqrtf(s)));
        }
    }
}

__global__ __launch_bounds__(256) void knn_prefilter_collect_kernel(const uint32_t* __restrict__ keys, uint64_t n_rows, uint32_t k,
                                                                    const uint32_t* __restrict__ hist, SelState* __restrict__ states,
                                                                    float band, uint32_t cap, uint32_t* __restrict__ cand_rows,
                                                                    uint32_t* __restrict__ count, const uint64_t* __restrict__ tomb = nullptr) {
    const SelState st = sel_advance(hist, states, 3, k, n_rows);
    uint32_t B = 0xFFFFFFFFu;
    if (n_rows >= k && st.fixed >= 1) {
        const uint64_t T = st.prefix | ((1ull << sel_shift(st.fixed - 1)) - 1ull);
        const uint32_t T32 = (uint32_t)(T >> 32);
        const float t = u32_to_dist(T32);
        if (T32 < PREF_MARK && t == t) B = dist_to_u32(t + band);
    }
    const uint64_t stride = (uint64_t)gridDim.x * 256;
    for (uint64_t r0 = (uint64_t)blockIdx.x * 256 + (threadIdx.x & ~63u); r0 < n_rows; r0 += stride) {
        const uint64_t r = r0 + (threadIdx.x & 63);
        const uint32_t key = r < n_rows ? keys[r] : 0xFFFFFFFFu;
        const bool take = r < n_rows && (key <= B || key == PREF_MARK) && !(tomb && tomb_dead(tomb, ((uint64_t)key << 32) | r));
// ... 19 lines not shown
        }
        atomicAdd(&acc[c], s);
    }
}
__global__ void knn_channel_scale_kernel(const float* __restrict__ acc, uint64_t n_rows, int dim, float* __restrict__ g) {
    const int c = blockIdx.x * blockDim.x + threadIdx.x;
    if (c >= dim) return;
    const float rms = sqrtf(acc[c] / (float)n_rows);
    g[c] = (rms >= 1.0e-18f && rms <= 1.0e18f) ? rms : 1.0f;
}

__device__ __forceinline__ float row16_max(float v) {
    v = fmaxf(v, dpp_mov<0xB1>(v));
    v = fmaxf(v, dpp_mov<0x4E>(v));
    v = fmaxf(v, dpp_mov<0x141>(v));
    v = fmaxf(v, dpp_mov<0x140>(v));
    return v;
}

template <int NCH>
__global__ __launch_bounds__(256) void knn_mirror8_kernel(const float* __restrict__ table, uint64_t first, uint64_t end,
                                                          const float* __restrict__ gch, uint8_t* __restrict__ mirror,
                                                          float* __restrict__ xx, float* __restrict__ scale,
                                                          float* __restrict__ cfac) {
    constexpr int DIM = NCH * 64;
    const int lane = threadIdx.x & 63, i = lane & 15;
    const uint64_t group = ((uint64_t)blockIdx.x * 256 + threadIdx.x) >> 4, n_groups = ((uint64_t)gridDim.x * 256) >> 4;
    f32x4 ginv[NCH];
#pragma unroll
    for (int t = 0; t < NCH; ++t) {
        const f32x4 gv = *reinterpret_cast<const f32x4*>(gch + 64 * t + 4 * i);
        ginv[t] = f32x4{1.0f / gv.x, 1.0f / gv.y, 1.0f / gv.z, 1.0f / gv.w};
    }
    for (uint64_t r0 = first + group; r0 < ((end - first + n_groups - 1) / n_groups) * n_groups + first; r0 += n_groups) {
        const bool live = r0 < end;
        const uint64_t r = live ? r0 : end - 1;
        const f32x4* p = reinterpret_cast<const f32x4*>(table + r * DIM) + i;
        f32x4 v[NCH];
        float s2 = 0.0f, a = 0.0f;
        bool bad = false;
#pragma unroll
        for (int t = 0; t < NCH; ++t) {
            v[t] = p[16 * t];
            const float e[4] = {v[t].x, v[t].y, v[t].z, v[t].w};
#pragma unroll
            for (int j = 0; j < 4; ++j) {
                bad |= !(fabsf(e[j]) <= 3.0e38f);
                s2 = __builtin_fmaf(e[j], e[j], s2);
            }
            v[t] = v[t] * ginv[t];
            a = fmaxf(a, fmaxf(fmaxf(fabsf(v[t].x), fabsf(v[t].y)), fmaxf(fabsf(v[t].z), fabsf(v[t].w))));
        }
        s2 = row16_sum(s2);
        a = row16_max(a);
        bad |= !(a <= 3.0e38f && a >= 1.0e-30f);
        const unsigned long long bm = __ballot(bad);
        const bool marked = ((bm >> (lane & 48)) & 0xFFFFull) != 0ull || !(s2 >= 1.0e-30f && s2 <= 1.0e30f);
        const float inv = marked ? 0.0f : 127.0f / a, sc = marked ? 0.0f : a / 127.0f;
#pragma unroll
        for (int t = 0; t < NCH; ++t) {
            const float e[4] = {v[t].x, v[t].y, v[t].z, v[t].w};
            uint32_t w = 0;
#pragma unroll
            for (int j = 0; j < 4; ++j) {
                const int q8 = (int)rintf(fminf(fmaxf(e[j] * inv, -127.0f), 127.0f)) + 128;
                w |= (uint32_t)(q8 & 0xFF) << (8 * j);
            }
            if (live) *reinterpret_cast<uint32_t*>(mirror + r * DIM + 64 * t + 4 * i) = w;
        }
        if (live && i == 0) {
            xx[r] = marked ? -1.0f : s2;
            scale[r] = sc;
            cfac[r] = marked ? 0.0f : 0.53f * sc / sqrtf(s2) * 1.000001f;
        }
    }
}

template <int NCH, int RING = 4>
__global__ __launch_bounds__(256, 2) void knn_scan_coarse8_kernel(const uint8_t* __restrict__ mirror, const float* __restrict__ xx,
                                                               const float* __restrict__ scale, const float* __restrict__ cfac,
                                                               const float* __restrict__ gch, uint64_t n_rows,
                                                               const float* __restrict__ q, float e0,
                                                               uint32_t* __restrict__ all_keys, float* __restrict__ rho_out,
                                                               uint32_t* __restrict__ sample_keys = nullptr, int sample_shift = 0) {
    static_assert(NCH % 4 == 0, "rows of whole 256-byte chunks of bytes");
    constexpr int DIM = NCH * 64, U = NCH / 4;
    const int lane = threadIdx.x & 63, wib = threadIdx.x >> 6;
    const int i = lane & 15, g = lane >> 4;
    const uint32_t wave = blockIdx.x * 4 + wib, n_waves = gridDim.x * 4;
    float qf[U][16];
    float sq, rho, qsum128;
    {
        float s2 = 0.0f, s1 = 0.0f, ss = 0.0f;
#pragma unroll
        for (int u = 0; u < U; ++u)
#pragma unroll
            for (int e = 0; e < 16; ++e) {
                const float qe = q[256 * u + 16 * i + e];
                s2 = __builtin_fmaf(qe, qe, s2);
                qf[u][e] = qe * gch[256 * u + 16 * i + e];
                s1 += fabsf(qf[u][e]);
                ss += qf[u][e];
            }
        sq = sqrtf(row16_sum(s2));
        rho = row16_sum(s1) / sq * 1.000001f;
        qsum128 = 128.0f * row16_sum(ss);
        if (blockIdx.x == 0 && threadIdx.x == 0) rho_out[0] = rho;
    }
    const uint64_t n_tiles = (n_rows + 63) >> 6;
    auto load_row = [&](u32x4 (&x)[U], uint64_t r) {
        r = r < n_rows ? r : n_rows - 1;
        const u32x4* p = reinterpret_cast<const u32x4*>(mirror + r * DIM) + i;
#pragma unroll
        for (int u = 0; u < U; ++u) x[u] = __builtin_nontemporal_load(p + 16 * u);
    };
    for (uint64_t tile = wave; tile < n_tiles; tile += n_waves) {
        float mydot = 0.0f;
        const uint64_t row0 = (tile << 6) + 16 * g;
        auto reduce_row = [&](const u32x4 (&x)[U], int it) {
            float a[4] = {0.0f, 0.0f, 0.0f, 0.0f};
#pragma unroll
            for (int u = 0; u < U; ++u) {
                const uint32_t w[4] = {x[u].x, x[u].y, x[u].z, x[u].w};
#pragma unroll
                for (int j = 0; j < 4; ++j) {
                    a[0] = __builtin_fmaf(qf[u][4 * j + 0], (float)(w[j] & 0xFFu), a[0]);
                    a[1] = __builtin_fmaf(qf[u][4 * j + 1], (float)((w[j] >> 8) & 0xFFu), a[1]);
                    a[2] = __builtin_fmaf(qf[u][4 * j + 2], (float)((w[j] >> 16) & 0xFFu), a[2]);
                    a[3] = __builtin_fmaf(qf[u][4 * j + 3], (float)(w[j] >> 24), a[3]);
                }
            }
            const float d = row16_sum((a[0] + a[1]) + (a[2] + a[3]));
            if (i == it) mydot = d;
        };
        u32x4 xr[RING][U];
#pragma unroll
        for (int d = 0; d < RING - 1; ++d) load_row(xr[d], row0 + d);
#pragma unroll
        for (int it = 0; it < 16; ++it) {
            if (it + RING - 1 < 16) load_row(xr[(it + RING - 1) % RING], row0 + it + RING - 1);
            reduce_row(xr[it % RING], it);
        }
        const uint64_t r = (tile << 6) + lane;
        if (r < n_rows) {
            const float s = xx[r];
            const float dot = scale[r] * (mydot - qsum128);
            const float upper = (1.0f - dot / (sq * sqrtf(s))) + (cfac[r] * rho + e0);
            all_keys[r] = s < 0.0f ? PREF_MARK : dist_to_u32(upper);
        }
        if (sample_keys && (tile & ((1ull << sample_shift) - 1)) == 0) {
            uint32_t key = 0xFFFFFFFFu;
            if (r < n_rows) {
                const float s = xx[r];
                const float dot = scale[r] * (mydot - qsum128);
                const float upper = (1.0f - dot / (sq * sqrtf(s))) + (cfac[r] * rho + e0);
                key = s < 0.0f ? PREF_MARK : dist_to_u32(upper);
            }
            sample_keys[((tile >> sample_shift) << 6) + lane] = key;
        }
    }
}

template <int NCH, int NQ>
__global__ __launch_bounds__(256, 2) void knn_scan_coarse8_batched_kernel(const uint8_t* __restrict__ mirror, const float* __restrict__ xx,
                                                                        const float* __restrict__ scale, const float* __restrict__ cfac,
                                                                        const float* __restrict__ gch, uint64_t n_rows,
                                                                        const float* __restrict__ q, float e0,
                                                                        uint32_t* __restrict__ all_keys, uint64_t key_stride,
                                                                        float* __restrict__ rho_out) {
    static_assert(NCH % 4 == 0 && (NQ == 2 || NQ == 4 || NQ == 8), "whole 256-byte chunks; 2, 4 or 8 queries");
    constexpr int DIM = NCH * 64, U = NCH / 4, GQ = NQ < 4 ? NQ : 4, QPG = NQ / GQ, RPS = 4 / GQ, STEPS = 64 / RPS;
    constexpr int AHEAD = NQ == 8 ? 4 : 8;
    typedef float f32x2 __attribute__((ext_vector_type(2)));
    const int lane = threadIdx.x & 63, wib = threadIdx.x >> 6;
    const int i = lane & 15, g = lane >> 4;
    const int qg = g % GQ, rs = g / GQ;
    const uint32_t wave = blockIdx.x * 4 + wib, n_waves = gridDim.x * 4;
    f32x2 qf[QPG][U][8];
    float sq[QPG], rho[QPG], qsum128[QPG];
#pragma unroll
    for (int c = 0; c < QPG; ++c) {
        const float* qq = q + (size_t)(qg + GQ * c) * DIM;
        float s2 = 0.0f, s1 = 0.0f, ss = 0.0f;
#pragma unroll
        for (int u = 0; u < U; ++u)
#pragma unroll
            for (int e = 0; e < 16; ++e) {
                const float qe = qq[256 * u + 16 * i + e];
                s2 = __builtin_fmaf(qe, qe, s2);
                const float qg = qe * gch[256 * u + 16 * i + e];
                qf[c][u][e >> 1][e & 1] = qg;
                s1 += fabsf(qg);
                ss += qg;
            }
        sq[c] = sqrtf(row16_sum(s2));
        rho[c] = row16_sum(s1) / sq[c] * 1.000001f;
        qsum128[c] = 128.0f * row16_sum(ss);
        if (blockIdx.x == 0 && wib == 0 && i == 0 && rs == 0) rho_out[qg + GQ * c] = rho[c];
    }
    const uint64_t n_tiles = (n_rows + 63) >> 6;
    auto load_row = [&](u32x4 (&x)[U], uint64_t r) {
        r = r < n_rows ? r : n_rows - 1;
        const u32x4* p = reinterpret_cast<const u32x4*>(mirror + r * DIM) + i;
#pragma unroll
        for (int u = 0; u < U; ++u) x[u] = __builtin_nontemporal_load(p + 16 * u);
    };
    for (uint64_t tile = wave; tile < n_tiles; tile += n_waves) {
        const uint64_t row0 = tile << 6;
        u32x4 xr[AHEAD][U];
#pragma unroll
        for (int d = 0; d < AHEAD; ++d) load_row(xr[d], row0 + RPS * d + rs);
        float mydot[QPG];
#pragma unroll
        for (int c = 0; c < QPG; ++c) mydot[c] = 0.0f;
#pragma unroll 1
        for (int s0 = 0; s0 < STEPS; s0 += AHEAD) {
#pragma unroll
            for (int e = 0; e < AHEAD; ++e) {
                const int it = s0 + e, row = RPS * it + rs;
                u32x4(&x)[U] = xr[e];
                f32x2 a01[QPG], a23[QPG];
#pragma unroll
                for (int c = 0; c < QPG; ++c) { a01[c] = (f32x2){0.0f, 0.0f}; a23[c] = (f32x2){0.0f, 0.0f}; }
#pragma unroll
                for (int u = 0; u < U; ++u) {
                    const uint32_t w[4] = {x[u].x, x[u].y, x[u].z, x[u].w};
#pragma unroll
                    for (int j = 0; j < 4; ++j) {
                        const f32x2 b01 = (f32x2){(float)(w[j] & 0xFFu), (float)((w[j] >> 8) & 0xFFu)};
                        const f32x2 b23 = (f32x2){(float)((w[j] >> 16) & 0xFFu), (float)(w[j] >> 24)};
#pragma unroll
                        for (int c = 0; c < QPG; ++c) {
                            a01[c] = __builtin_elementwise_fma(qf[c][u][2 * j], b01, a01[c]);
                            a23[c] = __builtin_elementwise_fma(qf[c][u][2 * j + 1], b23, a23[c]);
                        }
                    }
                }
                if (it + AHEAD < STEPS) load_row(x, row0 + RPS * (it + AHEAD) + rs);
#pragma unroll
                for (int c = 0; c < QPG; ++c) {
                    const float d = row16_sum((a01[c].x + a01[c].y) + (a23[c].x + a23[c].y));
                    if (i == (row & 15)) mydot[c] = d;
// ... 531 lines not shown
                top.offer(wave_best[w][lane]);
            } else {
                const uint64_t* other = reinterpret_cast<uint64_t*>(smem) + (size_t)w * Top::LDS_KEYS;
                for (uint32_t j = 0; j < (uint32_t)Top::KP; j += 64) {
                    const uint32_t idx = j + lane;
                    top.offer(idx < k ? other[idx] : KEY_MAX);
                }
            }
        }
        top.finish();
        top.store(out + (size_t)blockIdx.x * k);
    }
}

template <int KP>
__global__ __launch_bounds__(256) void knn_merge_block_kernel(const uint64_t* __restrict__ in, uint32_t n_lists,
                                                              uint32_t k, uint32_t lpb, uint64_t* __restrict__ out) {
    __shared__ uint64_t buf[2 * KP];
    __shared__ uint64_t s_thr;
    __shared__ uint32_t s_cnt;
    const int tid = threadIdx.x, lane = tid & 63;
    const uint32_t l0 = blockIdx.x * lpb;
    const uint32_t l1 = l0 + lpb < n_lists ? l0 + lpb : n_lists;
    const uint64_t* src = in + (size_t)l0 * k;
    const uint32_t n_keys = (l1 - l0) * k;
    for (int j = tid; j < 2 * KP; j += 256) buf[j] = KEY_MAX;
    {
        const uint32_t nl = l1 - l0, m = (k + nl - 1) / nl;
        uint64_t v = 0;
        for (uint32_t l = tid; l < nl; l += 256) { const uint64_t x = src[(size_t)l * k + (m - 1)]; v = x > v ? x : v; }
#pragma unroll
        for (int off = 1; off < 64; off <<= 1) { const uint64_t o = shfl_xor64(v, off); v = o > v ? o : v; }
        if (lane == 0) buf[tid >> 6] = v;
        __syncthreads();
        if (tid == 0) {
            uint64_t t0 = buf[0];
            for (int w = 1; w < 4; ++w) t0 = buf[w] > t0 ? buf[w] : t0;
            s_thr = t0 == KEY_MAX ? KEY_MAX : t0 + 1;
            s_cnt = 0;
        }
        __syncthreads();
        if (tid < 4) buf[tid] = KEY_MAX;
    }
    __syncthreads();
    auto block_sort = [&]() {
        for (int kk = 2; kk <= 2 * KP; kk <<= 1)
            for (int j = kk >> 1; j > 0; j >>= 1) {
                for (int p = tid; p < KP; p += 256) {
                    const int a = ((p & ~(j - 1)) << 1) | (p & (j - 1));
                    const int b = a | j;
                    const uint64_t x = buf[a], y = buf[b];
                    const bool up = (a & kk) == 0;
                    if ((x > y) == up) { buf[a] = y; buf[b] = x; }
                }
                __syncthreads();
            }
        if (tid == 0) { s_thr = buf[k - 1]; s_cnt = 0; }
        for (int j = KP + tid; j < 2 * KP; j += 256) buf[j] = KEY_MAX;
        __syncthreads();
    };
    for (uint32_t j0 = 0; j0 < n_keys; j0 += 256) {
        const uint32_t j = j0 + tid;
        const uint64_t key = j < n_keys ? src[j] : KEY_MAX;
        const bool pass = key < s_thr;
        const unsigned long long mask = __ballot(pass);
        uint32_t base = 0;
        if (lane == 0 && mask) base = atomicAdd(&s_cnt, (uint32_t)__popcll(mask));
        base = __shfl(base, 0, 64);
        if (pass) {
            const uint32_t rank = __builtin_amdgcn_mbcnt_hi((uint32_t)(mask >> 32), __builtin_amdgcn_mbcnt_lo((uint32_t)mask, 0));
            buf[KP + base + rank] = key;
        }
        __syncthreads();
        if (s_cnt + 256 > (uint32_t)KP) block_sort();
    }
    if (s_cnt) block_sort();
    for (uint32_t j = tid; j < k; j += 256) out[(size_t)blockIdx.x * k + j] = buf[j];
}

__global__ void knn_finalize_kernel(const uint64_t* __restrict__ keys, uint32_t n, IdMap map,
                                    uint64_t* __restrict__ idx, float* __restrict__ dist,
                                    size_t key_stride, size_t out_stride,
                                    const uint64_t* __restrict__ prefilter_keys = nullptr,
                                    const uint32_t* __restrict__ fallback = nullptr, uint32_t fallback_stride = 0) {
    const uint32_t j = blockIdx.x * blockDim.x + threadIdx.x;
    if (j >= n) return;
    if (fallback) fallback += (size_t)blockIdx.y * fallback_stride;
    if (fallback && *fallback == 0u) keys = prefilter_keys;
    const uint64_t key = keys ? keys[blockIdx.y * key_stride + j] : KEY_MAX;
    uint64_t* oi = idx + blockIdx.y * out_stride;
    float* od = dist + blockIdx.y * out_stride;
    if (key == KEY_MAX) {
        oi[j] = MI_KNN_NO_ID;
        od[j] = __uint_as_float(0x7F800000u);
    } else {
        oi[j] = id_of_local(map, (uint32_t)key);
        od[j] = u32_to_dist((uint32_t)(key >> 32));
    }
}

__device__ __forceinline__ bool merge_less(uint32_t ka, uint64_t ia, uint32_t kb, uint64_t ib) {
    return ka < kb || (ka == kb && ia < ib);
}
__global__ __launch_bounds__(256) void knn_merge_lists_kernel(const uint64_t* __restrict__ idx_in, const float* __restrict__ dist_in,
                                                              uint32_t lists, uint32_t k, size_t idx_stride, size_t dist_stride,
                                                              uint64_t* __restrict__ idx, float* __restrict__ dist) {
    const uint32_t u = blockIdx.y;
    const uint64_t* qi = idx_in + (size_t)u * k;
    const float* qd = dist_in + (size_t)u * k;
    const uint32_t e = blockIdx.x * blockDim.x + threadIdx.x;
    if (e < k) {
        uint32_t valid = 0;
        for (uint32_t l = 0; l < lists; ++l) {
            const uint64_t* li = qi + l * idx_stride;
            uint32_t lo = 0, hi = k;
            while (lo < hi) {
                const uint32_t mid = (lo + hi) >> 1;
                if (li[mid] != MI_KNN_NO_ID) lo = mid + 1; else hi = mid;
            }
            valid += lo;
        }
        if (e >= valid) {
            idx[(size_t)u * k + e] = MI_KNN_NO_ID;
            dist[(size_t)u * k + e] = __uint_as_float(0x7F800000u);
        }
    }
    if (e >= lists * k) return;
    const uint32_t l = e / k, p = e % k;
    const uint64_t id = qi[l * idx_stride + p];
    if (id == MI_KNN_NO_ID) return;
    const float d = qd[l * dist_stride + p];
    const uint32_t key = dist_to_u32(d);
    uint32_t rank = p;
    for (uint32_t o = 0; o < lists && rank < k; ++o) {
        if (o == l) continue;
        const uint64_t* li = qi + o * idx_stride;
        const float* ld = qd + o * dist_stride;
        uint32_t lo = 0, hi = k;
        while (lo < hi) {
            const uint32_t mid = (lo + hi) >> 1;
            const uint64_t mi_ = li[mid];
            const uint32_t mk = dist_to_u32(ld[mid]);
            const bool front = mi_ != MI_KNN_NO_ID && (o < l ? !merge_less(key, id, mk, mi_) : merge_less(mk, mi_, key, id));
            if (front) lo = mid + 1; else hi = mid;
        }
        rank += lo;
    }
    if (rank < k) {
        idx[(size_t)u * k + rank] = id;
        dist[(size_t)u * k + rank] = d;
    }
}

__device__ __forceinline__ uint64_t mix64(uint64_t z) {
    z = (z ^ (z >> 30)) * 0xBF58476D1CE4E5B9ull;
    z = (z ^ (z >> 27)) * 0x94D049BB133111EBull;
    return z ^ (z >> 31);
}
__device__ __forceinline__ float gen1(uint64_t key, uint64_t i, float scale) {
    const uint64_t h = mix64(i + key);
    const int s = (int)((h & 0xffff) + ((h >> 16) & 0xffff) + ((h >> 32) & 0xffff) + (h >> 48));
    return (float)(s - 131070) * scale;
}
__global__ void gen_f32_kernel(float* __restrict__ out, uint64_t key, uint64_t first, uint64_t n, float scale) {
    const uint64_t stride = (uint64_t)gridDim.x * blockDim.x * 4;
    for (uint64_t j = ((uint64_t)blockIdx.x * blockDim.x + threadIdx.x) * 4; j < n; j += stride) {
        f32x4 v;
        v.x = gen1(key, first + j, scale); v.y = gen1(key, first + j + 1, scale);
        v.z = gen1(key, first + j + 2, scale); v.w = gen1(key, first + j + 3, scale);
        *reinterpret_cast<f32x4*>(out + j) = v;
// ... 5 lines not shown
```

image_search_amd/csrc/pipeline.hip:

```cpp
#include <cstdlib>
#include <cstring>
#include <mutex>
#include <vector>

#include "common.h"
#include "handles.h"

using namespace mi;

namespace {
constexpr int N_SLOTS = 16;
constexpr int N_SPANS = 32;
struct QuerySlot {
    float* h_q = nullptr;
    float* d_q = nullptr;
    uint64_t *d_idx = nullptr, *h_idx = nullptr;
    float *d_dist = nullptr, *h_dist = nullptr;
    uint32_t cap_k = 0, k = 0;
    uint64_t* user_idx = nullptr;
    float* user_dist = nullptr;
    hipEvent_t done = nullptr;
    bool busy = false;
};
struct Span { hipEvent_t a = nullptr, b = nullptr; bool used = false; };
struct Lane {
    mi_clip* m = nullptr;
    mi_knn* t = nullptr;
    int device = 0;
    hipStream_t ingest = nullptr, copy = nullptr;
    hipEvent_t ev_up[2] = {nullptr, nullptr}, ev_used[2] = {nullptr, nullptr};
    float* d_in[2] = {nullptr, nullptr};
    size_t in_cap = 0;
    uint64_t seq = 0;
    Span fwd[N_SPANS];
    uint64_t n_fwd = 0;
};
}

struct mi_pipeline {
    std::vector<Lane> lanes;
    mi_knn_sharded* st = nullptr;
    int device = 0;
    hipStream_t search = nullptr;
    QuerySlot slots[N_SLOTS];
    int next_slot = 0;
    Span scan[N_SPANS];
    uint64_t n_scan = 0;
    double st_n[2] = {0, 0}, st_ms[2] = {0, 0};
    std::vector<std::pair<int, int>> prev_uploads;
    std::mutex mu;
};

namespace {

void deliver(QuerySlot& s) {
    if (!s.busy) return;
    HIP_CHECK(hipEventSynchronize(s.done));
    if (s.user_idx) {
        std::memcpy(s.user_idx, s.h_idx, (size_t)s.k * sizeof(uint64_t));
        std::memcpy(s.user_dist, s.h_dist, (size_t)s.k * sizeof(float));
    }
    s.busy = false;
}

void slot_reserve(QuerySlot& s, uint32_t dim, uint32_t k) {
    if (!s.done) HIP_CHECK(hipEventCreateWithFlags(&s.done, hipEventDisableTiming));
    if (!s.h_q) {
        HIP_CHECK(hipHostMalloc((void**)&s.h_q, (size_t)dim * 4, hipHostMallocDefault));
        HIP_CHECK(hipMalloc((void**)&s.d_q, (size_t)dim * 4));
    }
    if (k <= s.cap_k) return;
    if (s.d_idx) { HIP_CHECK(hipFree(s.d_idx)); HIP_CHECK(hipFree(s.d_dist)); HIP_CHECK(hipHostFree(s.h_idx)); HIP_CHECK(hipHostFree(s.h_dist)); }
    s.d_idx = nullptr; s.d_dist = nullptr; s.h_idx = nullptr; s.h_dist = nullptr; s.cap_k = 0;
    const uint32_t cap = (k + 63) / 64 * 64;
    HIP_CHECK(hipMalloc((void**)&s.d_idx, (size_t)cap * 8));
    HIP_CHECK(hipMalloc((void**)&s.d_dist, (size_t)cap * 4));
    HIP_CHECK(hipHostMalloc((void**)&s.h_idx, (size_t)cap * 8, hipHostMallocDefault));
    HIP_CHECK(hipHostMalloc((void**)&s.h_dist, (size_t)cap * 4, hipHostMallocDefault));
    s.cap_k = cap;
}

void collect(mi_pipeline* p, Span& sp, int kind) {
    if (!sp.used) return;
    HIP_CHECK(hipEventSynchronize(sp.b));
    float ms = 0.0f;
    HIP_CHECK(hipEventElapsedTime(&ms, sp.a, sp.b));
    p->st_n[kind] += 1;
    p->st_ms[kind] += ms;
    sp.used = false;
}

Span& span_begin(mi_pipeline* p, Span* ring, uint64_t* count, int kind, hipStream_t s) {
    Span& sp = ring[(*count)++ % N_SPANS];
    collect(p, sp, kind);
    if (!sp.a) { HIP_CHECK(hipEventCreate(&sp.a)); HIP_CHECK(hipEventCreate(&sp.b)); }
    HIP_CHECK(hipEventRecord(sp.a, s));
    return sp;
}

void span_end(Span& sp, hipStream_t s) {
    HIP_CHECK(hipEventRecord(sp.b, s));
    sp.used = true;
}

void free_spans(Span* ring) {
    for (int i = 0; i < N_SPANS; ++i) {
        if (ring[i].a) (void)hipEventDestroy(ring[i].a);
        if (ring[i].b) (void)hipEventDestroy(ring[i].b);
    }
}

void free_pipeline(mi_pipeline* p) {
    if (!p) return;
    for (Lane& ln : p->lanes) {
        (void)hipSetDevice(ln.device);
        for (hipStream_t s : {ln.ingest, ln.copy})
            if (s) (void)hipStreamSynchronize(s);
    }
    if (p->st) (void)mi_knn_sharded_sync(p->st);
    (void)hipSetDevice(p->device);
    if (p->search) (void)hipStreamSynchronize(p->search);
    free_spans(p->scan);
    for (auto& s : p->slots) {
        if (s.done) (void)hipEventDestroy(s.done);
        if (s.h_q) (void)hipHostFree(s.h_q);
        if (s.d_q) (void)hipFree(s.d_q);
        if (s.d_idx) (void)hipFree(s.d_idx);
        if (s.d_dist) (void)hipFree(s.d_dist);
        if (s.h_idx) (void)hipHostFree(s.h_idx);
        if (s.h_dist) (void)hipHostFree(s.h_dist);
    }
    if (p->search) (void)hipStreamDestroy(p->search);
    for (Lane& ln : p->lanes) {
        (void)hipSetDevice(ln.device);
        free_spans(ln.fwd);
        for (int b = 0; b < 2; ++b) {
            if (ln.ev_up[b]) (void)hipEventDestroy(ln.ev_up[b]);
            if (ln.ev_used[b]) (void)hipEventDestroy(ln.ev_used[b]);
            if (ln.d_in[b]) (void)hipFree(ln.d_in[b]);
        }
        for (hipStream_t s : {ln.ingest, ln.copy})
            if (s) (void)hipStreamDestroy(s);
    }
    delete p;
}

void lane_init(Lane& ln, mi_clip* model, mi_knn* table) {
    if (!model || !table) fail(MI_ERR_INVALID, "null handle");
    if (model->text) fail(MI_ERR_INVALID, "the pipeline ingests images: pass the image tower");
    if (model->device != table->device)
        fail(MI_ERR_INVALID, "model on device %d, table shard on device %d: a tower replica feeds the shard on its own GPU", model->device,
             table->device);
    if ((uint32_t)model->E != table->dim)
        fail(MI_ERR_INVALID, "the model embeds into %d dimensions, the table holds %u", model->E, table->dim);
    ln.m = model; ln.t = table; ln.device = model->device;
    DeviceGuard g(ln.device);
    HIP_CHECK(hipStreamCreateWithFlags(&ln.ingest, hipStreamNonBlocking));
    HIP_CHECK(hipStreamCreateWithFlags(&ln.copy, hipStreamNonBlocking));
    for (int b = 0; b < 2; ++b) {
        HIP_CHECK(hipEventCreateWithFlags(&ln.ev_up[b], hipEventDisableTiming));
        HIP_CHECK(hipEventCreateWithFlags(&ln.ev_used[b], hipEventDisableTiming));
    }
}

void lane_ingest(mi_pipeline* p, int li, const float* nchw, size_t n) {
    Lane& ln = p->lanes[(size_t)li];
    mi_clip* m = ln.m;
    mi_knn* t = ln.t;
    std::scoped_lock l(m->mu, t->mu);
    DeviceGuard g(ln.device);
    const size_t px = (size_t)m->image * m->image * 3;
    const size_t chunk = std::min(n, m->max_batch);
    clip_ensure_workspace(m, chunk);
    if (chunk > ln.in_cap) {
        for (hipStream_t s : {ln.ingest, ln.copy}) HIP_CHECK(hipStreamSynchronize(s));
        for (int b = 0; b < 2; ++b) {
            if (ln.d_in[b]) HIP_CHECK(hipFree(ln.d_in[b]));
            ln.d_in[b] = nullptr;
            HIP_CHECK(hipMalloc((void**)&ln.d_in[b], chunk * px * 4));
        }
        ln.in_cap = chunk;
    }
    knn_grow(t, t->rows + n);
    for (size_t i = 0; i < n; i += chunk) {
        const size_t c = std::min(chunk, n - i);
        const int b = (int)(ln.seq & 1);
        if (ln.seq >= 1) HIP_CHECK(hipEventSynchronize(ln.ev_up[b ^ 1]));
        if (ln.seq >= 2) HIP_CHECK(hipStreamWaitEvent(ln.copy, ln.ev_used[b], 0));
        HIP_CHECK(hipMemcpyAsync(ln.d_in[b], nchw + i * px, c * px * 4, hipMemcpyHostToDevice, ln.copy));
        HIP_CHECK(hipEventRecord(ln.ev_up[b], ln.copy));
        p->prev_uploads.emplace_back(li, b);
        m->order.begin(ln.ingest);
        t->writes.begin(ln.ingest);
        HIP_CHECK(hipStreamWaitEvent(ln.ingest, ln.ev_up[b], 0));
        auto& sp = span_begin(p, ln.fwd, &ln.n_fwd, 0, ln.ingest);
        clip_forward(m, ln.d_in[b], c, t->table + t->rows * t->dim, ln.ingest, m->front_overlap ? ln.copy : nullptr);
        span_end(sp, ln.ingest);
        HIP_CHECK(hipEventRecord(ln.ev_used[b], ln.ingest));
        m->order.end(ln.ingest);
        t->writes.end(ln.ingest);
        t->rows += c;
        ++ln.seq;
    }
}

}

extern "C" {

int mi_pipeline_create(mi_clip* model, mi_knn* table, mi_pipeline** out) {
    mi_pipeline* p = nullptr;
    const int rc = guarded([&] {
        if (!out) fail(MI_ERR_INVALID, "out is null");
// ... 6 lines not shown
        HIP_CHECK(hipStreamCreateWithFlags(&p->search, hipStreamNonBlocking));
        *out = p;
    });
    if (rc != MI_OK && p) free_pipeline(p);
    return rc;
}

int mi_pipeline_create_sharded(mi_clip* const* models, int n_models, mi_knn_sharded* table, mi_pipeline** out) {
    mi_pipeline* p = nullptr;
    const int rc = guarded([&] {
        if (!out) fail(MI_ERR_INVALID, "out is null");
        *out = nullptr;
        if (!models || !table) fail(MI_ERR_INVALID, "null handle");
        if (n_models != (int)table->n()) fail(MI_ERR_INVALID, "%d models for %u shards: one tower replica per shard", n_models, table->n());
        p = new mi_pipeline();
        p->st = table;
        p->lanes.resize((size_t)n_models);
        for (int s = 0; s < n_models; ++s) lane_init(p->lanes[(size_t)s], models[s], table->shard[(size_t)s]);
        p->device = p->lanes[0].device;
        *out = p;
    });
    if (rc != MI_OK && p) free_pipeline(p);
    return rc;
}

void mi_pipeline_free(mi_pipeline* p) { free_pipeline(p); }

int mi_pipeline_ingest(mi_pipeline* p, const float* nchw, size_t n, uint64_t* first_id) {
    return guarded([&] {
        if (!p) fail(MI_ERR_INVALID, "null pipeline handle");
        std::lock_guard<std::mutex> lp(p->mu);
        for (auto [li, b] : p->prev_uploads) HIP_CHECK(hipEventSynchronize(p->lanes[(size_t)li].ev_up[b]));
        p->prev_uploads.clear();
        if (!p->st) {
            mi_knn* t = p->lanes[0].t;
            if (first_id) *first_id = t->base + t->rows;
            if (n == 0) return;
            if (!nchw) fail(MI_ERR_INVALID, "nchw is null");
            lane_ingest(p, 0, nchw, n);
            return;
        }
        mi_knn_sharded* st = p->st;
        std::lock_guard<std::mutex> lt(st->mu);
        if (first_id) *first_id = st->rows;
        if (n == 0) return;
        if (!nchw) fail(MI_ERR_INVALID, "nchw is null");
        const size_t px = (size_t)p->lanes[0].m->image * p->lanes[0].m->image * 3;
        uint64_t r = st->rows;
        const uint64_t end = st->rows + n;
        try {
            while (r < end) {
                const uint64_t len = std::min<uint64_t>(st->block - r % st->block, end - r);
                uint32_t s; uint64_t local;
                sharded_place(st, r, &s, &local);
                if (local != st->shard[s]->rows) fail(MI_ERR_INVALID, "shard %u out of step (%llu rows, expected %llu)", s,
                                                      (unsigned long long)st->shard[s]->rows, (unsigned long long)local);
                lane_ingest(p, (int)s, nchw + (r - st->rows) * px, (size_t)len);
                r += len;
            }
        } catch (...) {
            for (uint32_t s = 0; s < st->n(); ++s) knn_truncate(st->shard[s], sharded_rows_of(st, st->rows, s));
            throw;
        }
        st->rows = end;
    });
}

int mi_pipeline_query(mi_pipeline* p, const float* q, uint32_t k, uint64_t* idx, float* dist) {
    return guarded([&] {
        if (!p) fail(MI_ERR_INVALID, "null pipeline handle");
        if (!q || !idx || !dist) fail(MI_ERR_INVALID, "null query/result pointer");
        if (k == 0) fail(MI_ERR_INVALID, "k must be >= 1");
        std::lock_guard<std::mutex> lp(p->mu);
        if (p->st) {
            std::lock_guard<std::mutex> lt(p->st->mu);
            sharded_search_enqueue(p->st, q, 1, k, idx, dist);
            return;
        }
        mi_knn* t = p->lanes[0].t;
        std::lock_guard<std::mutex> l(t->mu);
        DeviceGuard g(p->device);
        QuerySlot& s = p->slots[p->next_slot];
        p->next_slot = (p->next_slot + 1) % N_SLOTS;
        deliver(s);
        slot_reserve(s, t->dim, k);
        std::memcpy(s.h_q, q, (size_t)t->dim * 4);
        s.k = k; s.user_idx = idx; s.user_dist = dist;
        HIP_CHECK(hipMemcpyAsync(s.d_q, s.h_q, (size_t)t->dim * 4, hipMemcpyHostToDevice, p->search));
        t->writes.begin(p->search);
        t->reads.begin(p->search);
        auto& sp = span_begin(p, p->scan, &p->n_scan, 1, p->search);
        knn_search_one(t, s.d_q, k, s.d_idx, s.d_dist, p->search);
        span_end(sp, p->search);
        t->reads.end(p->search);
        HIP_CHECK(hipMemcpyAsync(s.h_idx, s.d_idx, (size_t)k * 8, hipMemcpyDeviceToHost, p->search));
        HIP_CHECK(hipMemcpyAsync(s.h_dist, s.d_dist, (size_t)k * 4, hipMemcpyDeviceToHost, p->search));
        HIP_CHECK(hipEventRecord(s.done, p->search));
        s.busy = true;
    });
}

int mi_pipeline_query_device(mi_pipeline* p, const float* q, uint32_t k, uint64_t* d_idx, float* d_dist, void* consumer_stream) {
    return guarded([&] {
        if (!p) fail(MI_ERR_INVALID, "null pipeline handle");
        if (!q || !d_idx || !d_dist) fail(MI_ERR_INVALID, "null query/result pointer");
        if (k == 0) fail(MI_ERR_INVALID, "k must be >= 1");
        std::lock_guard<std::mutex> lp(p->mu);
        if (p->st) fail(MI_ERR_UNSUPPORTED, "a sharded pipeline gathers and merges its shards' lists itself: use mi_pipeline_query");
        mi_knn* t = p->lanes[0].t;
        std::lock_guard<std::mutex> l(t->mu);
        DeviceGuard g(p->device);
        QuerySlot& s = p->slots[p->next_slot];
        p->next_slot = (p->next_slot + 1) % N_SLOTS;
        deliver(s);
        slot_reserve(s, t->dim, 0);
        std::memcpy(s.h_q, q, (size_t)t->dim * 4);
        s.k = k; s.user_idx = nullptr; s.user_dist = nullptr;
        HIP_CHECK(hipMemcpyAsync(s.d_q, s.h_q, (size_t)t->dim * 4, hipMemcpyHostToDevice, p->search));
        t->writes.begin(p->search);
        t->reads.begin(p->search);
        auto& sp = span_begin(p, p->scan, &p->n_scan, 1, p->search);
        knn_search_one(t, s.d_q, k, d_idx, d_dist, p->search);
        span_end(sp, p->search);
        t->reads.end(p->search);
        HIP_CHECK(hipEventRecord(s.done, p->search));
        HIP_CHECK(hipStreamWaitEvent((hipStream_t)consumer_stream, s.done, 0));
        s.busy = true;
    });
}

int mi_pipeline_sync(mi_pipeline* p) {
    return guarded([&] {
        if (!p) fail(MI_ERR_INVALID, "null pipeline handle");
        std::lock_guard<std::mutex> lp(p->mu);
        for (Lane& ln : p->lanes) {
            DeviceGuard g(ln.device);
            HIP_CHECK(hipStreamSynchronize(ln.copy));
            HIP_CHECK(hipStreamSynchronize(ln.ingest));
            for (auto& sp : ln.fwd) collect(p, sp, 0);
        }
        p->prev_uploads.clear();
        if (p->st) {
            std::lock_guard<std::mutex> lt(p->st->mu);
            sharded_deliver_all(p->st);
            return;
        }
        DeviceGuard g(p->device);
        HIP_CHECK(hipStreamSynchronize(p->search));
        for (auto& s : p->slots) deliver(s);
        for (auto& sp : p->scan) collect(p, sp, 1);
    });
}

int mi_pipeline_drain(mi_pipeline* p, uint32_t leave_pending) {
    return guarded([&] {
        if (!p) fail(MI_ERR_INVALID, "null pipeline handle");
        std::lock_guard<std::mutex> lp(p->mu);
        if (p->st) {
            std::lock_guard<std::mutex> lt(p->st->mu);
            sharded_deliver_all(p->st);
            return;
        }
        DeviceGuard g(p->device);
        uint32_t busy = 0;
        for (auto& s : p->slots) busy += s.busy ? 1 : 0;
        for (int i = 0; i < N_SLOTS && busy > leave_pending; ++i) {
            QuerySlot& s = p->slots[(p->next_slot + i) % N_SLOTS];
            if (s.busy) { deliver(s); --busy; }
        }
    });
}

int mi_pipeline_stats(mi_pipeline* p, double out[4], int reset) {
    return guarded([&] {
        if (!p || !out) fail(MI_ERR_INVALID, "null argument");
        std::lock_guard<std::mutex> lp(p->mu);
        out[0] = p->st_n[0]; out[1] = p->st_ms[0]; out[2] = p->st_n[1]; out[3] = p->st_ms[1];
        if (reset) { p->st_n[0] = p->st_n[1] = 0; p->st_ms[0] = p->st_ms[1] = 0; }
    });
}

int mi_host_alloc(size_t bytes, void** out) {
    return guarded([&] {
        if (!out) fail(MI_ERR_INVALID, "out is null");
        *out = nullptr;
        int n = 0;
        if (hipGetDeviceCount(&n) != hipSuccess || n <= 0) fail(MI_ERR_NO_DEVICE, "no HIP device visible: pinned memory needs the runtime");
        HIP_CHECK(hipHostMalloc(out, std::max<size_t>(bytes, 1), hipHostMallocPortable));
    });
}

void mi_host_free(void* p) {
    if (p) (void)hipHostFree(p);
}

}
```

image_search_amd/search.py:

```python
from __future__ import annotations

import ctypes
from typing import Optional, Sequence

import numpy as np

from ._lib import MI_KNN_WHERE_GROUP, KnnWhere, c_f, c_vp, check, lib

K_REFERENCE = 1000
NO_ID = np.uint64(0xFFFFFFFFFFFFFFFF)
NO_LABEL = np.uint32(0xFFFFFFFF)


def _f32(a) -> np.ndarray:
    return np.ascontiguousarray(a, dtype=np.float32)


COMPOUND_MODES = {"all": 0, "any": 1}


def _compound_args(dim: int, terms, mode, without, without_within):
    if mode not in COMPOUND_MODES:
        raise ValueError(f"mode must be 'all' or 'any' (got {mode!r})")
    pos = _f32(terms).reshape(-1, dim)
# ... 119 lines not shown


def _search_where(fn, h, dim, reference, k, where):
    q = _f32(reference)
    single = q.ndim == 1
    q = q.reshape(-1, dim)
    k = int(k)
    idx, dist = np.empty((q.shape[0], max(k, 1)), np.uint64), np.empty((q.shape[0], max(k, 1)), np.float32)
    matched = ctypes.c_uint64()
    check(fn(h, q.ctypes.data, q.shape[0], k, ctypes.byref(where), idx.ctypes.data, dist.ctypes.data, ctypes.byref(matched)))
    idx, dist = idx[:, :k], dist[:, :k]
    return (idx[0], dist[0], matched.value) if single else (idx, dist, matched.value)


def _ptrs(vecs):
    arr = (c_f * len(vecs))()
    for i, v in enumerate(vecs):
        arr[i] = v.ctypes.data_as(c_f)
    return arr


def average_slices(vectors: Sequence[np.ndarray]) -> np.ndarray:
    if len(vectors) == 0:
        raise AssertionError("Input must not be empty")
    vecs = [_f32(v).reshape(-1) for v in vectors]
    n = vecs[0].size
    if any(v.size != n for v in vecs):
        raise AssertionError("All vectors must have the same length")
    out = np.empty(n, np.float32)
    check(lib().mi_average_slices(_ptrs(vecs), len(vecs), n, out.ctypes.data_as(c_f)))
    return out


def refine_query(text_embedding: np.ndarray, selected: Sequence[np.ndarray]) -> np.ndarray:
    text = _f32(text_embedding).reshape(-1)
    sel = [_f32(v).reshape(-1) for v in selected]
    if any(v.size != text.size for v in sel):
        raise AssertionError("All vectors must have the same length")
    out = np.empty_like(text)
    check(lib().mi_refine(text.ctypes.data_as(c_f), _ptrs(sel), len(sel), text.size, out.ctypes.data_as(c_f)))
    return out


class EmbeddingTable:

    def __init__(self, dim: int = 768, device: int = 0, base: int = 0):
        self._h = c_vp()
        self.dim, self.device = dim, device
        check(lib().mi_knn_create(dim, device, ctypes.byref(self._h)))
        if base:
            self.set_base(base)

    def close(self):
        if getattr(self, "_h", None) and self._h.value:
            lib().mi_knn_free(self._h)
            self._h = c_vp()

    __del__ = close

    def __len__(self) -> int:
        n = ctypes.c_uint64()
        check(lib().mi_knn_size(self._h, ctypes.byref(n)))
        return n.value

    def set_base(self, base: int):
        check(lib().mi_knn_set_base(self._h, base))
        self._base_id = int(base)

    def reserve(self, rows: int):
        check(lib().mi_knn_reserve(self._h, rows))

    def set_option(self, key: str, value: int):
        check(lib().mi_knn_set_option(self._h, key.encode(), int(value)))

    def prefilter_stats(self):
        c, f = ctypes.c_uint32(), ctypes.c_uint32()
        check(lib().mi_knn_prefilter_stats(self._h, ctypes.byref(c), ctypes.byref(f)))
        return c.value, bool(f.value)

    def prefilter_state(self):
        out = (ctypes.c_uint32 * 4)()
        check(lib().mi_knn_prefilter_state(self._h, out))
        return {"skips_left": out[0], "consecutive_fallbacks": out[1], "searches_skipped": out[2], "scales_taken_at_rows": out[3]}

    def insert(self, embeddings: np.ndarray):
        e = _f32(embeddings).reshape(-1, self.dim)
        check(lib().mi_knn_append(self._h, e.ctypes.data, e.shape[0]))

    def insert_device(self, d_ptr: int, n: int, stream: int = 0):
        check(lib().mi_knn_append_device(self._h, d_ptr, n, stream))

    def insert_synthetic(self, seed: int, first_row: int, n: int):
        check(lib().mi_knn_append_synthetic(self._h, seed, first_row, n))

    def rows(self, first: int, n: int) -> np.ndarray:
        out = np.empty((n, self.dim), np.float32)
        check(lib().mi_knn_get_rows(self._h, first, n, out.ctypes.data))
        return out

    def delete(self, ids) -> int:
        return _delete(lib().mi_knn_delete, self._h, ids)

    def deleted(self) -> np.ndarray:
        return _deleted(lib().mi_knn_deleted, self._h)

    def knn(self, reference: np.ndarray, k: int = K_REFERENCE, within=None):
        q = _f32(reference)
        single = q.ndim == 1
        q = q.reshape(-1, self.dim)
        idx = np.empty((q.shape[0], k), np.uint64)
        dist = np.empty((q.shape[0], k), np.float32)
        if within is None:
            check(lib().mi_knn_search(self._h, q.ctypes.data, q.shape[0], k, idx.ctypes.data, dist.ctypes.data))
        else:
            ids = _ids(within)
            check(lib().mi_knn_search_filtered(self._h, q.ctypes.data, q.shape[0], k, ids.ctypes.data if ids.size else None,
                                               ids.size, idx.ctypes.data, dist.ctypes.data))
        return (idx[0], dist[0]) if single else (idx, dist)

    def knn_device(self, d_q: int, nq: int, k: int, d_idx: int, d_dist: int, stream: int = 0, batched: bool = False):
        fn = lib().mi_knn_search_batched_device if batched else lib().mi_knn_search_device
        check(fn(self._h, d_q, nq, k, d_idx, d_dist, stream))

    def near_pairs(self, max_dist: float, first_new: int = 0, cap: int = 1 << 20):
        a, b = np.empty(cap, np.uint64), np.empty(cap, np.uint64)
        dist = np.empty(cap, np.float32)
        n = ctypes.c_uint64()
        check(lib().mi_knn_near_pairs(self._h, float(max_dist), int(first_new), a.ctypes.data if cap else None,
                                      b.ctypes.data if cap else None, dist.ctypes.data if cap else None, cap, ctypes.byref(n)))
        return a[:n.value].copy(), b[:n.value].copy(), dist[:n.value].copy()

    def near_pairs_stats(self):
        out = (ctypes.c_uint64 * 4)()
        check(lib().mi_knn_near_pairs_stats(self._h, out))
        return {"candidates": out[0], "pairs": out[1], "strips": out[2], "tiles": out[3]}

    def assign(self, vectors: np.ndarray):
        v = _f32(vectors).reshape(-1, self.dim)
        n = len(self)
        labels, dist = np.empty(n, np.uint32), np.empty(n, np.float32)
        check(lib().mi_knn_assign(self._h, v.ctypes.data, v.shape[0], labels.ctypes.data, dist.ctypes.data))
        return labels, dist

    def assign_stats(self):
        out = (ctypes.c_uint64 * 4)()
        check(lib().mi_knn_assign_stats(self._h, out))
        return {"candidates": out[0], "rows": out[1], "launches": out[2], "tiles": out[3]}

    def assign_multi(self, vectors: np.ndarray, m: int, max_dist: float = float("inf")):
        v = _f32(vectors).reshape(-1, self.dim)
        n = len(self)
        labels, dist = np.empty((n, int(m)), np.uint32), np.empty((n, int(m)), np.float32)
        check(lib().mi_knn_assign_multi(self._h, v.ctypes.data, v.shape[0], int(m), float(max_dist), labels.ctypes.data,
                                        dist.ctypes.data))
        return labels, dist

    def assign_multi_stats(self):
        out = (ctypes.c_uint64 * 4)()
        check(lib().mi_knn_assign_multi_stats(self._h, out))
        return {"candidates": out[0], "hits": out[1], "launches": out[2], "tiles": out[3]}

    def knn_many(self, queries: np.ndarray, k: int):
        q = _f32(queries).reshape(-1, self.dim)
        idx, dist = np.empty((q.shape[0], int(k)), np.uint64), np.empty((q.shape[0], int(k)), np.float32)
        check(lib().mi_knn_search_many(self._h, q.ctypes.data, q.shape[0], int(k), idx.ctypes.data, dist.ctypes.data))
        return idx, dist
# ... 979 lines not shown
```

include/mi355clip.h:

```cpp
#ifndef MI355CLIP_H
#define MI355CLIP_H

#include <stddef.h>
#include <stdint.h>

#ifdef __cplusplus
extern "C" {
#endif

#define MI_OK 0
#define MI_ERR_INVALID (-1)
#define MI_ERR_IO (-2)
#define MI_ERR_HIP (-3)
#define MI_ERR_NO_DEVICE (-4)
#define MI_ERR_UNSUPPORTED (-5)
#define MI_ERR_OOM (-6)

#define MI_PRECISION_F32 0
#define MI_PRECISION_BF16 1
#define MI_PRECISION_BF16_SPLIT 2
#define MI_PRECISION_BF16X3 3

#define MI_KNN_NO_ID UINT64_MAX

typedef struct mi_clip mi_clip;
typedef struct mi_knn mi_knn;
typedef struct mi_pipeline mi_pipeline;
typedef struct mi_knn_sharded mi_knn_sharded;
typedef struct mi_index mi_index;

const char* mi_last_error(void);
int mi_abi_version(void);
int mi_device_count(void);


int mi_clip_load(const char* weights_path, int device, int precision, mi_clip** out);
void mi_clip_free(mi_clip* m);
int mi_weights_list(const char* weights_path, char* buf, size_t cap, size_t* needed);

int mi_clip_set_option(mi_clip* m, const char* key, int value);

int mi_clip_info(const mi_clip* m, uint32_t out[8]);

int mi_clip_ln_fold_stats(mi_clip* m, uint64_t out[2], int reset);

int mi_clip_embed(mi_clip* m, const float* nchw, size_t n, float* out);

int mi_clip_embed_device(mi_clip* m, const float* d_nchw, size_t n, float* d_out, void* stream);

int mi_clip_embed_rgb8(mi_clip* m, const uint8_t* rgb8, size_t n, float* out);

int mi_preprocess_rgb8(const uint8_t* rgb8, size_t n, uint32_t height, uint32_t width, float* chw);

int mi_resize_catmullrom_rgb8(int device, const uint8_t* rgb8, uint32_t width, uint32_t height, uint32_t new_width,
                              uint32_t new_height, uint8_t* out);

int mi_image_prepare_resnet(int device, const uint8_t* rgb8, uint32_t width, uint32_t height, float* chw);

int mi_clip_embed_images(mi_clip* m, const uint8_t* const* rgb8, const uint32_t* widths, const uint32_t* heights,
                         size_t n, float* out);

int mi_clip_load_text(const char* weights_path, int device, int precision, mi_clip** out);
int mi_clip_embed_text(mi_clip* m, const int32_t* input_ids, size_t n, float* out);


int mi_knn_create(uint32_t dim, int device, mi_knn** out);
void mi_knn_free(mi_knn* t);
int mi_knn_set_base(mi_knn* t, uint64_t base);
int mi_knn_set_option(mi_knn* t, const char* key, int value);
int mi_knn_prefilter_stats(mi_knn* t, uint32_t* candidates, uint32_t* fell_back);
int mi_knn_prefilter_state(mi_knn* t, uint32_t out[4]);
int mi_knn_reserve(mi_knn* t, uint64_t rows);
int mi_knn_size(const mi_knn* t, uint64_t* rows);

int mi_knn_append(mi_knn* t, const float* rows, uint64_t n);
int mi_knn_append_device(mi_knn* t, const float* d_rows, uint64_t n, void* stream);
int mi_knn_append_synthetic(mi_knn* t, uint64_t seed, uint64_t first_row, uint64_t n);
int mi_knn_get_rows(mi_knn* t, uint64_t first, uint64_t n, float* out);

int mi_knn_save(mi_knn* t, const char* path);
int mi_knn_load(mi_knn* t, const char* path);

int mi_knn_delete(mi_knn* t, const uint64_t* ids, uint64_t n, uint64_t* newly);
int mi_knn_deleted(mi_knn* t, uint64_t* ids, uint64_t cap, uint64_t* count);

int mi_knn_search(mi_knn* t, const float* q, uint32_t nq, uint32_t k, uint64_t* idx, float* dist);
int mi_knn_search_device(mi_knn* t, const float* d_q, uint32_t nq, uint32_t k, uint64_t* d_idx,
                         float* d_dist, void* stream);
int mi_knn_search_batched_device(mi_knn* t, const float* d_q, uint32_t nq, uint32_t k, uint64_t* d_idx,
                                 float* d_dist, void* stream);
int mi_knn_search_filtered(mi_knn* t, const float* q, uint32_t nq, uint32_t k, const uint64_t* ids, uint64_t n_ids,
                           uint64_t* idx, float* dist);
int mi_knn_near_pairs(mi_knn* t, float max_dist, uint64_t first_new, uint64_t* a, uint64_t* b, float* dist,
                      uint64_t cap, uint64_t* count);
int mi_knn_near_pairs_stats(mi_knn* t, uint64_t out[4]);
#define MI_KNN_NO_LABEL UINT32_MAX
int mi_knn_assign(mi_knn* t, const float* vectors, uint32_t C, uint32_t* labels, float* dist);
int mi_knn_assign_stats(mi_knn* t, uint64_t out[4]);
int mi_knn_assign_multi(mi_knn* t, const float* vectors, uint32_t C, uint32_t m, float max_dist, uint32_t* labels, float* dist);
int mi_knn_assign_multi_stats(mi_knn* t, uint64_t out[4]);
int mi_knn_search_many(mi_knn* t, const float* q, uint32_t nq, uint32_t k, uint64_t* idx, float* dist);
int mi_knn_search_many_stats(mi_knn* t, uint64_t out[4]);
int mi_knn_neighbors(mi_knn* t, uint64_t first, uint64_t n, uint32_t k, uint64_t* idx, float* dist);
int mi_knn_kmeans(mi_knn* t, float* centroids, uint32_t C, uint32_t max_iters, uint32_t* labels, float* dist,
                  uint32_t* iters_run, uint64_t* changed_last, double* objective);
int mi_knn_kmeans_seed(mi_knn* t, uint32_t C, uint64_t seed, const uint64_t* among, uint64_t n_among, uint64_t* rows,
                       float* centroids, double* potential);
int mi_knn_kmeans_seed_stats(mi_knn* t, uint64_t out[4]);
int mi_knn_search_diverse(mi_knn* t, const float* q, uint32_t k, uint32_t pool, float min_gap, const uint64_t* among,
                          uint64_t n_among, uint64_t* idx, float* dist, uint32_t* hidden, uint32_t* rep, uint32_t* n_kept);
int mi_knn_search_diverse_stats(mi_knn* t, uint64_t out[4]);
#define MI_COMPOUND_ALL 0
#define MI_COMPOUND_ANY 1
int mi_knn_search_compound(mi_knn* t, const float* pos, uint32_t n_pos, int mode, const float* neg, const float* neg_within,
                           uint32_t n_neg, uint32_t k, const uint64_t* among, uint64_t n_among, uint64_t* idx, float* dist,
                           float* term_dist );
int mi_knn_search_compound_stats(mi_knn* t, uint64_t out[4]);
int mi_knn_search_page(mi_knn* t, const float* q, uint32_t k,
                       float after_dist, uint64_t after_id,
                       float max_dist,
                       const uint64_t* among, uint64_t n_among,
                       uint64_t* idx, float* dist, uint64_t counts[4] );
#define MI_KNN_NO_GROUP 0xFFFFFFFFu
#define MI_KNN_GROUPS_MAX (1u << 24)
int mi_knn_set_groups(mi_knn* t, const uint64_t* ids, uint64_t n, const uint32_t* groups);
int mi_knn_get_groups(mi_knn* t, const uint64_t* ids, uint64_t n, uint32_t* groups);
int mi_knn_groups_info(mi_knn* t, uint64_t info[2]);
int mi_knn_search_grouped(mi_knn* t, const float* q, uint32_t k, float max_dist, const uint64_t* among, uint64_t n_among,
                          uint64_t* idx, float* dist, uint32_t* group , uint64_t* members ,
                          uint64_t* facets , uint64_t cap_facets, uint64_t totals[4] );
int mi_knn_set_attrs(mi_knn* t, const uint64_t* ids, uint64_t n, const uint64_t* tags ,
                     const int64_t* stamps );
int mi_knn_get_attrs(mi_knn* t, const uint64_t* ids, uint64_t n, uint64_t* tags , int64_t* stamps );
#define MI_KNN_WHERE_GROUP 1u
typedef struct mi_knn_where {
    uint64_t all_of, any_of, none_of;
    int64_t stamp_lo, stamp_hi;
    uint32_t group;
    uint32_t flags;
} mi_knn_where;
int mi_knn_count_where(mi_knn* t, const mi_knn_where* w, uint64_t* count);
int mi_knn_rows_where(mi_knn* t, const mi_knn_where* w, uint64_t* ids, uint64_t cap, uint64_t* count);
int mi_knn_search_where(mi_knn* t, const float* q, uint32_t nq, uint32_t k, const mi_knn_where* w, uint64_t* idx, float* dist,
                        uint64_t* matched );
int mi_pairs_to_groups(const uint64_t* a, const uint64_t* b, uint64_t n_pairs, uint64_t* ids, uint64_t cap_ids,
                       uint64_t* group_start, uint64_t cap_groups, uint64_t* n_ids, uint64_t* n_groups);


int mi_knn_sharded_create(uint32_t dim, const int* devices, int n_dev, uint32_t block_rows, mi_knn_sharded** out);
void mi_knn_sharded_free(mi_knn_sharded* t);
int mi_knn_sharded_info(const mi_knn_sharded* t, uint64_t* rows, uint32_t* n_shards, uint32_t* block_rows, int* transport);
int mi_knn_sharded_stats(const mi_knn_sharded* t, uint64_t out[4]);
int mi_knn_sharded_set_option(mi_knn_sharded* t, const char* key, int value);
int mi_knn_sharded_reserve(mi_knn_sharded* t, uint64_t rows);
// ... 109 lines not shown
```

Before: 6453 images/s.

## Shorten kNN prefilter kernel chain using feedback from the previous query

The single-query prefilter path now uses the candidate count and fallback flag reported by the previous query. When the last query had few candidates it runs one small-select kernel instead of the six-pass histogram select. It also fuses the first histogram pass into the coarse8 scan kernel, and skips the selection-state memsets when the previous chain left them clean. When no fallback is expected, the guarded fallback one_pass is launched with only a few blocks. The per-query report is copied back together with idx and dist in a single D2H copy from a merged buffer. The changes depend on the previous query's state and on atomics in the scan kernel, which risks correctness or extra work if the candidate count jumps.

```diff
diff --git a/image_search_amd/_lib.py b/image_search_amd/_lib.py
--- a/image_search_amd/_lib.py
+++ b/image_search_amd/_lib.py
@@ -48,6 +48,7 @@
     "mi_knn_set_option": (ctypes.c_int, [c_vp, ctypes.c_char_p, ctypes.c_int]),
     "mi_knn_prefilter_stats": (ctypes.c_int, [c_vp, c_vp, c_vp]),
     "mi_knn_prefilter_state": (ctypes.c_int, [c_vp, ctypes.POINTER(ctypes.c_uint32)]),
+    "mi_knn_chain_stats": (ctypes.c_int, [c_vp, c_u64p]),
     "mi_knn_reserve": (ctypes.c_int, [c_vp, ctypes.c_uint64]),
     "mi_knn_size": (ctypes.c_int, [c_vp, c_u64p]),
     "mi_knn_append": (ctypes.c_int, [c_vp, c_vp, ctypes.c_uint64]),
diff --git a/image_search_amd/csrc/handles.h b/image_search_amd/csrc/handles.h
--- a/image_search_amd/csrc/handles.h
+++ b/image_search_amd/csrc/handles.h
@@ -146,6 +146,13 @@
     uint64_t* d_pref_keys = nullptr;
     uint32_t* d_pref_flag = nullptr;
     size_t pref_rows_cap = 0, pref_keys_cap = 0, pref_flag_cap = 0;
+    static constexpr uint32_t PREF_REPORT = 64;
+    bool chain_clean = false;
+    uint64_t pref_min_rows = 1u << 18;
+    uint32_t pref_cap = 1u << 22;
+    uint32_t pref_last_cand = 0;
+    bool pref_last_fell = false;
+    uint64_t chain_stats[4] = {0, 0, 0, 0};
     mi::WorkOrder writes, reads;
     std::vector<uint32_t> dead;
     uint64_t* d_tomb = nullptr;
@@ -252,7 +259,8 @@
 void clip_forward(mi_clip* m, const float* d_img, size_t n, float* d_out, hipStream_t s, hipStream_t front = nullptr);
 hipStream_t knn_own_stream(mi_knn* t);
 void knn_grow(mi_knn* t, uint64_t want_rows);
-void knn_search_one(mi_knn* t, const float* d_q, uint32_t k, uint64_t* d_idx, float* d_dist, hipStream_t s);
+bool knn_search_one(mi_knn* t, const float* d_q, uint32_t k, uint64_t* d_idx, float* d_dist, hipStream_t s, uint32_t* d_report = nullptr);
+void knn_pref_report(mi_knn* t, uint32_t candidates, uint32_t fell_back);
 void knn_search_many(mi_knn* t, const float* d_q, uint32_t nq, uint32_t k, uint64_t* d_idx, float* d_dist, hipStream_t s);
 void knn_truncate(mi_knn* t, uint64_t rows);
 void knn_search_filtered_many(mi_knn* t, const float* d_q, uint32_t nq, uint32_t k, const uint64_t* ids, uint64_t n_ids,
diff --git a/image_search_amd/csrc/knn.hip b/image_search_amd/csrc/knn.hip
--- a/image_search_amd/csrc/knn.hip
+++ b/image_search_amd/csrc/knn.hip
@@ -219,10 +219,11 @@
 
 template <class Top>
 void one_pass(mi_knn* t, const float* d_q, uint32_t kp, const uint64_t* lo, uint64_t* keys_out, hipStream_t s,
-              const uint32_t* run_if = nullptr, uint32_t gy = 1, QGroup qg = QGroup{}) {
+              const uint32_t* run_if = nullptr, uint32_t gy = 1, QGroup qg = QGroup{}, uint32_t max_blocks = 0) {
     const uint32_t bpc = Top::LDS_KEYS == 0 ? 4 : (Top::KP <= 256 ? 4 : 2);
     const uint64_t n_tiles = (t->rows + 63) / 64;
     uint32_t blocks = (uint32_t)std::min<uint64_t>((uint64_t)t->n_cu * bpc, (n_tiles + 3) / 4);
+    if (max_blocks) blocks = std::min(blocks, max_blocks);
     blocks = std::max(blocks, 1u);
     const uint32_t lists = blocks * 4;
     ensure(t, (void**)&t->d_cand, &t->cand_keys, (size_t)lists * kp * gy, sizeof(uint64_t));
@@ -259,10 +260,9 @@
     }
 }
 
-constexpr uint64_t PREF_MIN_ROWS = 1u << 18;
 bool prefilter_applies(const mi_knn* t, uint32_t k) {
     const uint32_t width = t->prefilter == 2 ? 256u : 128u;
-    return t->prefilter && (k <= 64 || (k <= 4096 && t->select_path)) && t->dim % width == 0 && t->rows >= PREF_MIN_ROWS;
+    return t->prefilter && (k <= 64 || (k <= 4096 && t->select_path)) && t->dim % width == 0 && t->rows >= t->pref_min_rows;
 }
 template <int NCH>
 void launch_coarse8_batched(mi_knn* t, const uint8_t* m8, const float* d_q, float e0, uint32_t nq, uint32_t blocks, hipStream_t s,
@@ -313,15 +313,17 @@
     g.q = t->dim; g.keys = t->cap; g.sel = SEL_WORDS; g.flags = 4; g.rows = (uint64_t)2 * PREF_CAP; g.coll = 4096; g.out = 4096; g.rho = 1;
     return g;
 }
-uint32_t* prefilter_pass(mi_knn* t, const float* d_q, uint32_t k, hipStream_t s, uint32_t nq_batch = 0) {
+uint32_t* prefilter_pass(mi_knn* t, const float* d_q, uint32_t k, hipStream_t s, uint32_t nq_batch, bool* select_left_clean) {
     const uint32_t gy = std::max(1u, nq_batch);
     const QGroup qg = group_of(t, gy);
+    const size_t sel_was = t->sel_cap, flag_was = t->pref_flag_cap;
     ensure(t, (void**)&t->d_keys32, &t->keys32_cap, (size_t)t->cap * gy, sizeof(uint32_t));
     ensure(t, (void**)&t->d_sel, &t->sel_cap, (size_t)SEL_WORDS * gy, sizeof(uint32_t));
     ensure(t, (void**)&t->d_cand, &t->cand_keys, (size_t)4096 * gy, sizeof(uint64_t));
     ensure(t, (void**)&t->d_pref_rows, &t->pref_rows_cap, (size_t)2 * PREF_CAP * gy, sizeof(uint32_t));
     ensure(t, (void**)&t->d_pref_keys, &t->pref_keys_cap, (size_t)4096 * gy, sizeof(uint64_t));
-    ensure(t, (void**)&t->d_pref_flag, &t->pref_flag_cap, (size_t)4 * gy, sizeof(uint32_t));
+    ensure(t, (void**)&t->d_pref_flag, &t->pref_flag_cap, (size_t)mi_knn::PREF_REPORT + 4, sizeof(uint32_t));
+    if (t->sel_cap != sel_was || t->pref_flag_cap != flag_was) t->chain_clean = false;
     const bool bytes = t->prefilter == 2;
     const uint32_t tile_rows = (nq_batch && t->batch_stage1_mfma) ? 16 : 64;
     const uint64_t n_tiles_s = (t->rows + tile_rows - 1) / tile_rows;
@@ -360,11 +362,17 @@
     const uint32_t hb = std::max<uint32_t>(std::min<uint32_t>(hb1, (uint32_t)t->n_cu), (hb1 + gy - 1) / gy);
     uint32_t* flags = t->d_pref_flag;
     uint32_t* key32 = t->d_pref_rows + PREF_CAP;
+    const uint32_t pcap = t->pref_cap;
     uint32_t* count2 = t->d_sel + 6 * SEL_BINS;
     SelState* states = reinterpret_cast<SelState*>(t->d_sel + 6 * SEL_BINS + 4);
     const size_t sel_bytes = (size_t)SEL_WORDS * gy * sizeof(uint32_t);
-    HIP_CHECK(hipMemsetAsync(t->d_sel, 0, sel_bytes, s));
-    HIP_CHECK(hipMemsetAsync(flags, 0, (size_t)4 * gy * sizeof(uint32_t), s));
+    if (!t->chain_clean) {
+        HIP_CHECK(hipMemsetAsync(t->d_sel, 0, t->sel_cap * sizeof(uint32_t), s));
+        HIP_CHECK(hipMemsetAsync(flags, 0, t->pref_flag_cap * sizeof(uint32_t), s));
+    }
+    t->chain_clean = false;
+    static const bool stage1_hist = [] { const char* e = std::getenv("MI_KNN_STAGE1_HIST"); return e ? std::atoi(e) != 0 : true; }();
+    const bool fuse_hist0 = stage1_hist && bytes && nq_batch == 0 && !sample_shift && !tomb_of(t);
     static const uint32_t ring8_bpc = [] { const char* e = std::getenv("MI_KNN_RING_BPC"); return e ? (uint32_t)std::max(1, std::atoi(e)) : 2u; }();
     const float e0 = 4.1f * (float)(t->dim + 8) * 0x1p-24f + 2e-6f;
     const float eps = 0x1p-8f + e0;
@@ -397,21 +405,21 @@
         if (nq_batch == 0 && t->coarse_ring == 8)   \
             hipLaunchKernelGGL((knn_scan_coarse8_kernel<NCH, 8>), dim3(std::min(blocks, (uint32_t)t->n_cu * ring8_bpc)), dim3(256), 0, s, m8, t->d_xx, t->d_scale8, \
                                t->d_cfac8, t->d_g8, t->rows, d_q, e0, t->d_keys32, t->d_rho8,                            \
-                               sample_shift ? t->d_skeys : (uint32_t*)nullptr, sample_shift);                            \
+                               sample_shift ? t->d_skeys : (uint32_t*)nullptr, sample_shift, fuse_hist0 ? t->d_sel : (uint32_t*)nullptr); \
         else if (nq_batch == 0)                                                                                          \
             hipLaunchKernelGGL((knn_scan_coarse8_kernel<NCH, 4>), dim3(blocks), dim3(256), 0, s, m8, t->d_xx, t->d_scale8, \
                                t->d_cfac8, t->d_g8, t->rows, d_q, e0, t->d_keys32, t->d_rho8,                            \
-                               sample_shift ? t->d_skeys : (uint32_t*)nullptr, sample_shift);                            \
+                               sample_shift ? t->d_skeys : (uint32_t*)nullptr, sample_shift, fuse_hist0 ? t->d_sel : (uint32_t*)nullptr); \
         else                                                                                                             \
             launch_coarse8_batched<NCH>(t, m8, d_q, e0, nq_batch, blocks, s, sample_shift, sample_stride);               \
         kill_keys();                                                                                                     \
-        for (int p = 0; p < 3; ++p)                                                                                      \
+        for (int p = fuse_hist0 ? 1 : 0; p < 3; ++p)                                                                       \
             hipLaunchKernelGGL(knn_select_hist_kernel, dim3(hbh, gy), dim3(256), 0, s, keys_h, n_h, k, p, t->d_sel, states, \
                                (const uint32_t*)nullptr, (const uint32_t*)nullptr, (const uint32_t*)nullptr, qgh, 0);    \
         hipLaunchKernelGGL(knn_prefilter_collect8_kernel, dim3(hb, gy), dim3(256), 0, s, keys_q, t->d_cfac8, t->rows, k, \
-                           t->d_sel, states, t->d_rho8, e0, PREF_CAP, t->d_pref_rows, flags, qg, tomb);                  \
+                           t->d_sel, states, t->d_rho8, e0, pcap, t->d_pref_rows, flags, qg, tomb);                      \
         hipLaunchKernelGGL((knn_rescore_kernel<NCH>), dim3(t->n_cu * (gy > 1 ? 2 : 8), gy), dim3(256), 0, s, t->table, d_q, \
-                           t->d_pref_rows, flags, PREF_CAP, key32, qg);                                                  \
+                           t->d_pref_rows, flags, pcap, key32, qg);                                                      \
         break;
             MI_CASE(4) MI_CASE(8) MI_CASE(12) MI_CASE(16)
 #undef MI_CASE
@@ -434,21 +442,36 @@
         for (int p = 0; p < 3; ++p)                                                                                      \
             hipLaunchKernelGGL(knn_select_hist_kernel, dim3(hb), dim3(256), 0, s, t->d_keys32, t->rows, k, p, t->d_sel, states); \
         hipLaunchKernelGGL(knn_prefilter_collect_kernel, dim3(hb), dim3(256), 0, s, t->d_keys32, t->rows, k, t->d_sel,   \
-                           states, 2.0f * eps, PREF_CAP, t->d_pref_rows, flags, tomb);                                   \
+                           states, 2.0f * eps, pcap, t->d_pref_rows, flags, tomb);                                       \
         hipLaunchKernelGGL((knn_rescore_kernel<NCH>), dim3(t->n_cu * 8), dim3(256), 0, s, t->table, d_q, t->d_pref_rows, \
-                           flags, PREF_CAP, key32);                                                                      \
+                           flags, pcap, key32);                                                                          \
         break;
         MI_CASE(2) MI_CASE(4) MI_CASE(8) MI_CASE(12) MI_CASE(16)
 #undef MI_CASE
         default: fail(MI_ERR_UNSUPPORTED, "dim %u: the prefilter is built for dim/64 in {2,4,8,12,16}", t->dim);
     }
+    if (t->pref_last_cand <= SMALL_SELECT_MAX) {
+        const uint32_t nt = k <= 256 ? 256u : 1024u;
+        uint32_t np = nt;
+        while (np < k) np <<= 1;
+        const size_t lds = (size_t)2 * np * sizeof(uint64_t);
+        allow_lds(knn_select_small_kernel, lds);
+        hipLaunchKernelGGL(knn_select_small_kernel, dim3(1, gy), dim3(nt), lds, s, t->d_pref_rows, key32, flags, pcap, k, np,
+                           t->d_pref_keys, t->d_sel, SEL_WORDS, qg);
+        HIP_CHECK(hipGetLastError());
+        ++t->chain_stats[0];
+        *select_left_clean = true;
+        return flags + 1;
+    }
+    ++t->chain_stats[1];
+    *select_left_clean = false;
     HIP_CHECK(hipMemsetAsync(t->d_sel, 0, sel_bytes, s));
     const uint32_t* go = flags + 2;
     const uint32_t cb = (uint32_t)t->n_cu * 2;
     for (int p = 0; p < 6; ++p)
-        hipLaunchKernelGGL(knn_select_hist_kernel, dim3(cb, gy), dim3(256), 0, s, key32, (uint64_t)PREF_CAP, k, p, t->d_sel, states, go, flags,
+        hipLaunchKernelGGL(knn_select_hist_kernel, dim3(cb, gy), dim3(256), 0, s, key32, (uint64_t)pcap, k, p, t->d_sel, states, go, flags,
                            t->d_pref_rows, qg, 1);
-    hipLaunchKernelGGL(knn_select_collect_kernel, dim3(cb, gy), dim3(256), 0, s, key32, (uint64_t)PREF_CAP, k, t->d_sel, states, t->d_cand, count2,
+    hipLaunchKernelGGL(knn_select_collect_kernel, dim3(cb, gy), dim3(256), 0, s, key32, (uint64_t)pcap, k, t->d_sel, states, t->d_cand, count2,
                        go, flags, t->d_pref_rows, qg, 1);
     hipLaunchKernelGGL(knn_select_sort_kernel, dim3(1, gy), dim3(1024), 0, s, t->d_cand, count2, k, t->d_pref_keys, go, qg);
     HIP_CHECK(hipGetLastError());
@@ -463,6 +486,7 @@
     ensure(t, (void**)&t->d_keys32, &t->keys32_cap, (size_t)t->cap * gy, sizeof(uint32_t));
     ensure(t, (void**)&t->d_sel, &t->sel_cap, (size_t)SEL_WORDS * gy, sizeof(uint32_t));
     ensure(t, (void**)&t->d_cand, &t->cand_keys, (size_t)4096 * gy, sizeof(uint64_t));
+    t->chain_clean = false;
     HIP_CHECK(hipMemsetAsync(t->d_sel, 0, (size_t)SEL_WORDS * gy * sizeof(uint32_t), s));
     const uint64_t* tomb = tomb_of(t);
     const uint64_t n_dead = t->dead.size();
@@ -501,6 +525,9 @@
     t->pref_probing = false;
 }
 void pref_fold(mi_knn* t, uint32_t cand, uint32_t fell_back) {
+    t->pref_last_cand = cand;
+    t->pref_last_fell = fell_back != 0;
+    if (!t->pref_adaptive) return;
     t->pref_consec = fell_back ? t->pref_consec + 1 : 0;
     if (t->pref_probing) {
         if (t->pref_reports_due && --t->pref_reports_due == 0) {
@@ -529,7 +556,7 @@
         return;
     }
     if (!t->pref_ev[i]) HIP_CHECK(hipEventCreateWithFlags(&t->pref_ev[i], hipEventDisableTiming));
-    HIP_CHECK(hipMemcpyAsync(t->h_pref_ring + 2 * i, t->d_pref_flag, 2 * sizeof(uint32_t), hipMemcpyDeviceToHost, s));
+    HIP_CHECK(hipMemcpyAsync(t->h_pref_ring + 2 * i, t->d_pref_flag + mi_knn::PREF_REPORT, 2 * sizeof(uint32_t), hipMemcpyDeviceToHost, s));
     HIP_CHECK(hipEventRecord(t->pref_ev[i], s));
     t->pref_ev_pending[i] = true;
     ++t->pref_seq;
@@ -542,6 +569,8 @@
     t->pref_consec = t->pref_skip_left = 0;
     t->pref_probing = false;
     t->pref_probes_left = t->pref_reports_due = 0;
+    t->pref_last_cand = 0;
+    t->pref_last_fell = false;
 }
 
 uint32_t reg_pass_lists(const mi_knn* t) {
@@ -549,7 +578,9 @@
     return 4 * std::max<uint32_t>(1u, (uint32_t)std::min<uint64_t>((uint64_t)t->n_cu * 4, (n_tiles + 3) / 4));
 }
 
-void two_stage(mi_knn* t, const float* d_q, uint32_t k, uint64_t* d_idx, float* d_dist, hipStream_t s, uint32_t nq_batch) {
+constexpr uint32_t TOKEN_FALLBACK_BLOCKS = 16;
+void two_stage(mi_knn* t, const float* d_q, uint32_t k, uint64_t* d_idx, float* d_dist, hipStream_t s, uint32_t nq_batch,
+               uint32_t* d_report = nullptr) {
     const uint32_t gy = std::max(1u, nq_batch);
     const QGroup qg = group_of(t, gy);
     if (k <= 64) {
@@ -557,18 +588,28 @@
         ensure(t, (void**)&t->d_cand, &t->cand_keys, std::max<size_t>((size_t)4096 * gy, (size_t)lists * k * gy), sizeof(uint64_t));
         if (lists > 64) ensure(t, (void**)&t->d_tmp, &t->tmp_keys, (size_t)((lists + 31) / 32) * k * gy, sizeof(uint64_t));
     }
-    const uint32_t* fallback = prefilter_pass(t, d_q, k, s, nq_batch);
-    if (k <= 64) one_pass<WaveTopReg>(t, d_q, k, nullptr, t->d_keys, s, fallback, gy, qg);
-    else select_pass(t, d_q, k, t->d_keys, s, fallback, gy);
+    bool clean = false;
+    uint32_t* fallback = prefilter_pass(t, d_q, k, s, nq_batch, &clean);
+    if (k <= 64) {
+        const bool token = !(t->pref_last_fell || t->pref_consec || t->pref_probing);
+        ++t->chain_stats[token ? 2 : 3];
+        one_pass<WaveTopReg>(t, d_q, k, nullptr, t->d_keys, s, fallback, gy, qg, token ? TOKEN_FALLBACK_BLOCKS : 0u);
+    } else {
+        ++t->chain_stats[3];
+        select_pass(t, d_q, k, t->d_keys, s, fallback, gy);
+        clean = false;
+    }
     hipLaunchKernelGGL(knn_finalize_kernel, dim3((k + 255) / 256, gy), dim3(256), 0, s, t->d_keys, k, id_map(t),
-                       d_idx, d_dist, (size_t)qg.out, (size_t)(gy > 1 ? k : 0), t->d_pref_keys, fallback, qg.flags);
+                       d_idx, d_dist, (size_t)qg.out, (size_t)(gy > 1 ? k : 0), t->d_pref_keys, fallback, qg.flags,
+                       fallback - 1, t->d_pref_flag + mi_knn::PREF_REPORT, d_report);
     HIP_CHECK(hipGetLastError());
+    t->chain_clean = clean;
 }
 
 bool batched_two_stage_applies(mi_knn* t, uint32_t k) {
     if (!(t->prefilter == 2 && t->dim == 768 && prefilter_applies(t, k))) return false;
+    pref_poll(t);
     if (!t->pref_adaptive) return true;
-    pref_poll(t);
     if (t->pref_skip_left) {
         if (k <= 64) {
             if (--t->pref_skip_left == 0) { t->pref_probing = true; t->pref_probes_left = t->pref_reports_due = 2; t->pref_consec = 0; }
@@ -587,21 +628,21 @@
     ensure(t, (void**)&t->d_keys, &t->keys_cap, (size_t)4096 * nq, sizeof(uint64_t));
     t->last_prefiltered = true;
     two_stage(t, d_q, k, d_idx, d_dist, s, nq);
-    if (t->pref_adaptive) pref_record(t, s);
-}
-
-void search_one(mi_knn* t, const float* d_q, uint32_t k, uint64_t* d_idx, float* d_dist, hipStream_t s) {
+    pref_record(t, s);
+}
+
+bool search_one(mi_knn* t, const float* d_q, uint32_t k, uint64_t* d_idx, float* d_dist, hipStream_t s, uint32_t* d_report = nullptr) {
     if (t->rows == 0) {
         hipLaunchKernelGGL(knn_finalize_kernel, dim3((k + 255) / 256, 1), dim3(256), 0, s,
                            (const uint64_t*)nullptr, k, id_map(t), d_idx, d_dist, (size_t)0, (size_t)0);
         HIP_CHECK(hipGetLastError());
-        return;
+        return false;
     }
     const uint32_t passes = (k + 1023) / 1024;
     ensure(t, (void**)&t->d_keys, &t->keys_cap, (size_t)std::max<uint32_t>(passes * 1024, 4096), sizeof(uint64_t));
     t->last_prefiltered = prefilter_applies(t, k);
+    if (t->last_prefiltered) pref_poll(t);
     if (t->last_prefiltered && t->pref_adaptive) {
-        pref_poll(t);
         if (t->pref_skip_left) {
             if (--t->pref_skip_left == 0) { t->pref_probing = true; t->pref_probes_left = t->pref_reports_due = 2; t->pref_consec = 0; }
             ++t->pref_skipped;
@@ -612,16 +653,16 @@
         }
     }
     if (t->last_prefiltered) {
-        two_stage(t, d_q, k, d_idx, d_dist, s, 0);
-        if (t->pref_adaptive) pref_record(t, s);
-        return;
+        two_stage(t, d_q, k, d_idx, d_dist, s, 0, d_report);
+        if (!d_report) pref_record(t, s);
+        return true;
     }
     if ((k > 64 || tomb_of(t)) && k <= 4096 && t->select_path) {
         select_pass(t, d_q, k, t->d_keys, s);
         hipLaunchKernelGGL(knn_finalize_kernel, dim3((k + 255) / 256, 1), dim3(256), 0, s, t->d_keys, k, id_map(t),
                            d_idx, d_dist, (size_t)0, (size_t)0);
         HIP_CHECK(hipGetLastError());
-        return;
+        return false;
     }
     for (uint32_t p = 0; p < passes; ++p) {
         const uint32_t kp = std::min(1024u, k - p * 1024);
@@ -634,6 +675,7 @@
     hipLaunchKernelGGL(knn_finalize_kernel, dim3((k + 255) / 256, 1), dim3(256), 0, s, t->d_keys, k, id_map(t),
                        d_idx, d_dist, (size_t)0, (size_t)0);
     HIP_CHECK(hipGetLastError());
+    return false;
 }
 
 template <int NQ>
@@ -786,6 +828,7 @@
     ensure(t, (void**)&t->d_keys32, &t->keys32_cap, (size_t)n, sizeof(uint32_t));
     ensure(t, (void**)&t->d_sel, &t->sel_cap, (size_t)SEL_WORDS, sizeof(uint32_t));
     ensure(t, (void**)&t->d_cand, &t->cand_keys, (size_t)4096, sizeof(uint64_t));
+    t->chain_clean = false;
     HIP_CHECK(hipMemsetAsync(t->d_sel, 0, (size_t)SEL_WORDS * sizeof(uint32_t), s));
     const uint32_t blocks = gather_blocks(t, n, 4);
     switch (t->dim / 64) {
@@ -893,6 +936,7 @@
 void knn_select_keys32(mi_knn* t, uint64_t n, uint32_t k, uint64_t* keys_out, const uint32_t* list, hipStream_t s) {
     ensure(t, (void**)&t->d_sel, &t->sel_cap, (size_t)SEL_WORDS, sizeof(uint32_t));
     ensure(t, (void**)&t->d_cand, &t->cand_keys, (size_t)4096, sizeof(uint64_t));
+    t->chain_clean = false;
     HIP_CHECK(hipMemsetAsync(t->d_sel, 0, (size_t)SEL_WORDS * sizeof(uint32_t), s));
     select_keys32(t, n, k, keys_out, list, s);
 }
@@ -902,9 +946,10 @@
 void knn_grow(mi_knn* t, uint64_t want_rows) { grow(t, want_rows); }
 void knn_groups_fit(mi_knn* t) { groups_fit(t); }
 void knn_attrs_fit(mi_knn* t) { attrs_fit(t); }
-void knn_search_one(mi_knn* t, const float* d_q, uint32_t k, uint64_t* d_idx, float* d_dist, hipStream_t s) {
-    search_one(t, d_q, k, d_idx, d_dist, s);
-}
+bool knn_search_one(mi_knn* t, const float* d_q, uint32_t k, uint64_t* d_idx, float* d_dist, hipStream_t s, uint32_t* d_report) {
+    return search_one(t, d_q, k, d_idx, d_dist, s, d_report);
+}
+void knn_pref_report(mi_knn* t, uint32_t candidates, uint32_t fell_back) { pref_fold(t, candidates, fell_back); }
 void knn_truncate(mi_knn* t, uint64_t rows) {
     std::lock_guard<std::mutex> l(t->mu);
     if (rows >= t->rows) return;
@@ -1018,6 +1063,12 @@
         } else if (k == "prefilter_adaptive") {
             pref_reset(t);
             t->pref_adaptive = value != 0;
+        } else if (k == "prefilter_min_rows") {
+            if (value < 1) fail(MI_ERR_INVALID, "prefilter_min_rows must be >= 1 (got %d)", value);
+            t->pref_min_rows = (uint64_t)value;
+        } else if (k == "prefilter_cap") {
+            if (value < 1 || (uint32_t)value > PREF_CAP) fail(MI_ERR_INVALID, "prefilter_cap must be in [1, %u] (got %d)", PREF_CAP, value);
+            t->pref_cap = (uint32_t)value;
         } else if (k == "join_cap") {
             if (value < (1 << 14)) fail(MI_ERR_INVALID, "join_cap must be >= 16384 (got %d)", value);
             t->join_cap = (uint32_t)value;
@@ -1043,7 +1094,7 @@
             if (!where_chunk_ok(value)) fail(MI_ERR_INVALID, "where_chunk must be 0 or a multiple of 64 up to 65536 (got %d)", value);
             t->where_chunk = value;
         } else {
-            fail(MI_ERR_INVALID, "unknown option '%s' (known: prefilter, prefilter_adaptive, prefilter_sample, batch_stage1, join_cap, many_segments, many_sample, compound_blocks, page_blocks, group_blocks, group_lds_max, where_chunk)", key);
+            fail(MI_ERR_INVALID, "unknown option '%s' (known: prefilter, prefilter_adaptive, prefilter_sample, prefilter_min_rows, prefilter_cap, batch_stage1, join_cap, many_segments, many_sample, compound_blocks, page_blocks, group_blocks, group_lds_max, where_chunk)", key);
         }
     });
 }
@@ -1057,8 +1108,20 @@
         DeviceGuard g(t->device);
         t->reads.sync();
         uint32_t w[2] = {0, 0};
-        HIP_CHECK(hipMemcpy(w, t->d_pref_flag, sizeof w, hipMemcpyDeviceToHost));
+        HIP_CHECK(hipMemcpy(w, t->d_pref_flag + mi_knn::PREF_REPORT, sizeof w, hipMemcpyDeviceToHost));
         *candidates = w[0]; *fell_back = w[1];
+    });
+}
+
+int mi_knn_chain_stats(mi_knn* t, uint64_t out[6]) {
+    return guarded([&] {
+        if (!t || !out) fail(MI_ERR_INVALID, "null argument");
+        std::lock_guard<std::mutex> l(t->mu);
+        DeviceGuard g(t->device);
+        pref_poll(t);
+        for (int i = 0; i < 4; ++i) out[i] = t->chain_stats[i];
+        out[4] = t->pref_last_cand;
+        out[5] = t->pref_last_fell ? 1 : 0;
     });
 }
 
diff --git a/image_search_amd/csrc/knn_kernels.h b/image_search_amd/csrc/knn_kernels.h
--- a/image_search_amd/csrc/knn_kernels.h
+++ b/image_search_amd/csrc/knn_kernels.h
@@ -249,14 +249,14 @@
         if (tomb && live) live = !tomb_dead(tomb, key);
         const bool hit = live && (key & hi_mask) == st.prefix;
         const uint32_t bin = (uint32_t)(key >> sh) & mk;
-        const unsigned long long hits = __ballot(hit);
-        if (hits == 0ull) return;
-        const uint32_t first = __builtin_amdgcn_readfirstlane(__shfl((int)bin, __ffsll((long long)hits) - 1, 64));
-        if (__ballot(hit && bin != first) == 0ull) {
-            if ((threadIdx.x & 63) == 0) atomicAdd(&lh[first], (uint32_t)__popcll(hits));
-        } else if (hit) {
-            atomicAdd(&lh[bin], 1u);
-        }
+        unsigned long long left = __ballot(hit);
+        for (int round = 0; round < (p == 0 ? 4 : 1) && left; ++round) {
+            const uint32_t first = __builtin_amdgcn_readfirstlane(__shfl((int)bin, __ffsll((long long)left) - 1, 64));
+            const unsigned long long same = __ballot(hit && bin == first) & left;
+            if ((threadIdx.x & 63) == 0) atomicAdd(&lh[first], (uint32_t)__popcll(same));
+            left &= ~same;
+        }
+        if ((left >> (threadIdx.x & 63)) & 1ull) atomicAdd(&lh[bin], 1u);
     };
     const uint64_t n4 = n_rows >> 2;
     for (uint64_t q4 = (uint64_t)blockIdx.x * 256 + threadIdx.x; q4 < ((n4 + 63) & ~63ull); q4 += (uint64_t)gridDim.x * 256) {
@@ -340,6 +340,68 @@
     for (uint32_t j = threadIdx.x; j < k; j += 1024) out[j] = buf[j];
 }
 
+constexpr uint32_t SMALL_SELECT_MAX = 4096;
+__global__ __launch_bounds__(1024) void knn_select_small_kernel(const uint32_t* __restrict__ cand_rows, const uint32_t* __restrict__ key32,
+                                                                const uint32_t* __restrict__ flags, uint32_t cap, uint32_t k, uint32_t np,
+                                                                uint64_t* __restrict__ out, uint32_t* __restrict__ zero,
+                                                                uint32_t zero_words, QGroup qg = QGroup{}) {
+    extern __shared__ __attribute__((aligned(16))) unsigned char smem[];
+    __shared__ uint32_t s_cnt;
+    uint64_t* buf = reinterpret_cast<uint64_t*>(smem);
+    cand_rows += (size_t)blockIdx.y * qg.rows;
+    key32 += (size_t)blockIdx.y * qg.rows;
+    flags += (size_t)blockIdx.y * qg.flags;
+    out += (size_t)blockIdx.y * qg.out;
+    const uint32_t tid = threadIdx.x, nt = blockDim.x, lane = tid & 63;
+    if (zero) {
+        zero += (size_t)blockIdx.y * qg.sel;
+        for (uint32_t j = tid; j < zero_words; j += nt) zero[j] = 0u;
+    }
+    if (flags[2] == 0u) return;
+    const uint32_t C = min(flags[0], cap);
+    uint32_t have = 0;
+    uint64_t thr = KEY_MAX;
+    if (tid == 0) s_cnt = 0;
+    __syncthreads();
+    auto flush = [&](uint32_t cnt) {
+        const uint32_t tot = have + cnt;
+        uint32_t m = 64;
+        while (m < tot) m <<= 1;
+        for (uint32_t j = tot + tid; j < m; j += nt) buf[j] = KEY_MAX;
+        __syncthreads();
+        for (uint32_t kk = 2; kk <= m; kk <<= 1)
+            for (uint32_t j = kk >> 1; j > 0; j >>= 1) {
+                for (uint32_t p = tid; p < m / 2; p += nt) {
+                    const uint32_t a = ((p & ~(j - 1)) << 1) | (p & (j - 1)), b = a | j;
+                    const uint64_t x = buf[a], y = buf[b];
+                    const bool up = (a & kk) == 0;
+                    if ((x > y) == up) { buf[a] = y; buf[b] = x; }
+                }
+                __syncthreads();
+            }
+        have = min(tot, k);
+        thr = have == k ? buf[k - 1] : KEY_MAX;
+        if (tid == 0) s_cnt = 0;
+        __syncthreads();
+    };
+    for (uint32_t c0 = 0; c0 < C; c0 += nt) {
+        const uint32_t c = c0 + tid;
+        const uint64_t key = c < C ? (((uint64_t)key32[c] << 32) | cand_rows[c]) : KEY_MAX;
+        const bool pass = c < C && key < thr;
+        const unsigned long long mask = __ballot(pass);
+        uint32_t base = 0;
+        if (lane == 0 && mask) base = atomicAdd(&s_cnt, (uint32_t)__popcll(mask));
+        base = __shfl(base, 0, 64);
+        if (pass) buf[have + base + __builtin_amdgcn_mbcnt_hi((uint32_t)(mask >> 32), __builtin_amdgcn_mbcnt_lo((uint32_t)mask, 0))] = key;
+        __syncthreads();
+        const uint32_t cnt = s_cnt;
+        __syncthreads();
+        if (have + cnt + nt > 2 * np) flush(cnt);
+    }
+    if (s_cnt) flush(s_cnt);
+    for (uint32_t j = tid; j < k; j += nt) out[j] = j < have ? buf[j] : KEY_MAX;
+}
+
 #ifndef PREF_DEPTH
 #define PREF_DEPTH 3
 #endif
@@ -525,12 +587,18 @@
                                                                const float* __restrict__ gch, uint64_t n_rows,
                                                                const float* __restrict__ q, float e0,
                                                                uint32_t* __restrict__ all_keys, float* __restrict__ rho_out,
-                                                               uint32_t* __restrict__ sample_keys = nullptr, int sample_shift = 0) {
+                                                               uint32_t* __restrict__ sample_keys = nullptr, int sample_shift = 0,
+                                                               uint32_t* __restrict__ hist0 = nullptr) {
     static_assert(NCH % 4 == 0, "rows of whole 256-byte chunks of bytes");
     constexpr int DIM = NCH * 64, U = NCH / 4;
+    __shared__ uint32_t lh[SEL_BINS];
     const int lane = threadIdx.x & 63, wib = threadIdx.x >> 6;
     const int i = lane & 15, g = lane >> 4;
     const uint32_t wave = blockIdx.x * 4 + wib, n_waves = gridDim.x * 4;
+    if (hist0) {
+        for (int j = threadIdx.x; j < SEL_BINS; j += 256) lh[j] = 0u;
+        __syncthreads();
+    }
     float qf[U][16];
     float sq, rho, qsum128;
     {
@@ -585,11 +653,24 @@
             reduce_row(xr[it % RING], it);
         }
         const uint64_t r = (tile << 6) + lane;
+        uint32_t mykey = 0u;
         if (r < n_rows) {
             const float s = xx[r];
             const float dot = scale[r] * (mydot - qsum128);
             const float upper = (1.0f - dot / (sq * sqrtf(s))) + (cfac[r] * rho + e0);
-            all_keys[r] = s < 0.0f ? PREF_MARK : dist_to_u32(upper);
+            mykey = s < 0.0f ? PREF_MARK : dist_to_u32(upper);
+            all_keys[r] = mykey;
+        }
+        if (hist0) {
+            const uint32_t bin = mykey >> 21;
+            unsigned long long left = __ballot(r < n_rows);
+            for (int round = 0; round < 4 && left; ++round) {
+                const uint32_t first = __builtin_amdgcn_readfirstlane(__shfl((int)bin, __ffsll((long long)left) - 1, 64));
+                const unsigned long long same = __ballot(r < n_rows && bin == first) & left;
+                if (lane == 0) atomicAdd(&lh[first], (uint32_t)__popcll(same));
+                left &= ~same;
+            }
+            if ((left >> lane) & 1ull) atomicAdd(&lh[bin], 1u);
         }
         if (sample_keys && (tile & ((1ull << sample_shift) - 1)) == 0) {
             uint32_t key = 0xFFFFFFFFu;
@@ -601,6 +682,11 @@
             }
             sample_keys[((tile >> sample_shift) << 6) + lane] = key;
         }
+    }
+    if (hist0) {
+        __syncthreads();
+        for (int j = threadIdx.x; j < SEL_BINS; j += 256)
+            if (lh[j]) atomicAdd(&hist0[j], lh[j]);
     }
 }
 
@@ -1298,10 +1384,21 @@
                                     uint64_t* __restrict__ idx, float* __restrict__ dist,
                                     size_t key_stride, size_t out_stride,
                                     const uint64_t* __restrict__ prefilter_keys = nullptr,
-                                    const uint32_t* __restrict__ fallback = nullptr, uint32_t fallback_stride = 0) {
+                                    const uint32_t* __restrict__ fallback = nullptr, uint32_t fallback_stride = 0,
+                                    uint32_t* __restrict__ count = nullptr, uint32_t* __restrict__ report = nullptr,
+                                    uint32_t* __restrict__ report2 = nullptr) {
     const uint32_t j = blockIdx.x * blockDim.x + threadIdx.x;
     if (j >= n) return;
     if (fallback) fallback += (size_t)blockIdx.y * fallback_stride;
+    if (count && j == 0) {
+        count += (size_t)blockIdx.y * fallback_stride;
+        if (blockIdx.y == 0) {
+            const uint32_t c = *count, f = *fallback;
+            if (report) { report[0] = c; report[1] = f; }
+            if (report2) { report2[0] = c; report2[1] = f; }
+        }
+        *count = 0u;
+    }
     if (fallback && *fallback == 0u) keys = prefilter_keys;
     const uint64_t key = keys ? keys[blockIdx.y * key_stride + j] : KEY_MAX;
     uint64_t* oi = idx + blockIdx.y * out_stride;
diff --git a/image_search_amd/csrc/pipeline.hip b/image_search_amd/csrc/pipeline.hip
--- a/image_search_amd/csrc/pipeline.hip
+++ b/image_search_amd/csrc/pipeline.hip
@@ -16,6 +16,8 @@
     float* d_q = nullptr;
     uint64_t *d_idx = nullptr, *h_idx = nullptr;
     float *d_dist = nullptr, *h_dist = nullptr;
+    uint32_t *d_report = nullptr, *h_report = nullptr;
+    bool reported = false;
     uint32_t cap_k = 0, k = 0;
     uint64_t* user_idx = nullptr;
     float* user_dist = nullptr;
@@ -53,15 +55,22 @@
 
 namespace {
 
-void deliver(QuerySlot& s) {
+void deliver(QuerySlot& s, mi_knn* t = nullptr, bool t_locked = false) {
     if (!s.busy) return;
     HIP_CHECK(hipEventSynchronize(s.done));
     if (s.user_idx) {
         std::memcpy(s.user_idx, s.h_idx, (size_t)s.k * sizeof(uint64_t));
         std::memcpy(s.user_dist, s.h_dist, (size_t)s.k * sizeof(float));
     }
+    if (s.reported && t) {
+        if (t_locked) knn_pref_report(t, s.h_report[0], s.h_report[1]);
+        else { std::lock_guard<std::mutex> l(t->mu); knn_pref_report(t, s.h_report[0], s.h_report[1]); }
+    }
+    s.reported = false;
     s.busy = false;
 }
+
+size_t record_bytes(uint32_t cap) { return (size_t)cap * 12 + 2 * sizeof(uint32_t); }
 
 void slot_reserve(QuerySlot& s, uint32_t dim, uint32_t k) {
     if (!s.done) HIP_CHECK(hipEventCreateWithFlags(&s.done, hipEventDisableTiming));
@@ -70,13 +79,15 @@
         HIP_CHECK(hipMalloc((void**)&s.d_q, (size_t)dim * 4));
     }
     if (k <= s.cap_k) return;
-    if (s.d_idx) { HIP_CHECK(hipFree(s.d_idx)); HIP_CHECK(hipFree(s.d_dist)); HIP_CHECK(hipHostFree(s.h_idx)); HIP_CHECK(hipHostFree(s.h_dist)); }
-    s.d_idx = nullptr; s.d_dist = nullptr; s.h_idx = nullptr; s.h_dist = nullptr; s.cap_k = 0;
+    if (s.d_idx) { HIP_CHECK(hipFree(s.d_idx)); HIP_CHECK(hipHostFree(s.h_idx)); }
+    s.d_idx = nullptr; s.d_dist = nullptr; s.d_report = nullptr; s.h_idx = nullptr; s.h_dist = nullptr; s.h_report = nullptr; s.cap_k = 0;
     const uint32_t cap = (k + 63) / 64 * 64;
-    HIP_CHECK(hipMalloc((void**)&s.d_idx, (size_t)cap * 8));
-    HIP_CHECK(hipMalloc((void**)&s.d_dist, (size_t)cap * 4));
-    HIP_CHECK(hipHostMalloc((void**)&s.h_idx, (size_t)cap * 8, hipHostMallocDefault));
-    HIP_CHECK(hipHostMalloc((void**)&s.h_dist, (size_t)cap * 4, hipHostMallocDefault));
+    HIP_CHECK(hipMalloc((void**)&s.d_idx, record_bytes(cap)));
+    HIP_CHECK(hipHostMalloc((void**)&s.h_idx, record_bytes(cap), hipHostMallocDefault));
+    s.d_dist = reinterpret_cast<float*>(s.d_idx + cap);
+    s.h_dist = reinterpret_cast<float*>(s.h_idx + cap);
+    s.d_report = reinterpret_cast<uint32_t*>(s.d_dist + cap);
+    s.h_report = reinterpret_cast<uint32_t*>(s.h_dist + cap);
     s.cap_k = cap;
 }
 
@@ -126,9 +137,7 @@
         if (s.h_q) (void)hipHostFree(s.h_q);
         if (s.d_q) (void)hipFree(s.d_q);
         if (s.d_idx) (void)hipFree(s.d_idx);
-        if (s.d_dist) (void)hipFree(s.d_dist);
         if (s.h_idx) (void)hipHostFree(s.h_idx);
-        if (s.h_dist) (void)hipHostFree(s.h_dist);
     }
     if (p->search) (void)hipStreamDestroy(p->search);
     for (Lane& ln : p->lanes) {
@@ -301,7 +310,7 @@
         DeviceGuard g(p->device);
         QuerySlot& s = p->slots[p->next_slot];
         p->next_slot = (p->next_slot + 1) % N_SLOTS;
-        deliver(s);
+        deliver(s, t, true);
         slot_reserve(s, t->dim, k);
         std::memcpy(s.h_q, q, (size_t)t->dim * 4);
         s.k = k; s.user_idx = idx; s.user_dist = dist;
@@ -309,11 +318,10 @@
         t->writes.begin(p->search);
         t->reads.begin(p->search);
         auto& sp = span_begin(p, p->scan, &p->n_scan, 1, p->search);
-        knn_search_one(t, s.d_q, k, s.d_idx, s.d_dist, p->search);
+        s.reported = knn_search_one(t, s.d_q, k, s.d_idx, s.d_dist, p->search, s.d_report);
         span_end(sp, p->search);
         t->reads.end(p->search);
-        HIP_CHECK(hipMemcpyAsync(s.h_idx, s.d_idx, (size_t)k * 8, hipMemcpyDeviceToHost, p->search));
-        HIP_CHECK(hipMemcpyAsync(s.h_dist, s.d_dist, (size_t)k * 4, hipMemcpyDeviceToHost, p->search));
+        HIP_CHECK(hipMemcpyAsync(s.h_idx, s.d_idx, record_bytes(s.cap_k), hipMemcpyDeviceToHost, p->search));
         HIP_CHECK(hipEventRecord(s.done, p->search));
         s.busy = true;
     });
@@ -331,10 +339,10 @@
         DeviceGuard g(p->device);
         QuerySlot& s = p->slots[p->next_slot];
         p->next_slot = (p->next_slot + 1) % N_SLOTS;
-        deliver(s);
+        deliver(s, t, true);
         slot_reserve(s, t->dim, 0);
         std::memcpy(s.h_q, q, (size_t)t->dim * 4);
-        s.k = k; s.user_idx = nullptr; s.user_dist = nullptr;
+        s.k = k; s.user_idx = nullptr; s.user_dist = nullptr; s.reported = false;
         HIP_CHECK(hipMemcpyAsync(s.d_q, s.h_q, (size_t)t->dim * 4, hipMemcpyHostToDevice, p->search));
         t->writes.begin(p->search);
         t->reads.begin(p->search);
@@ -366,7 +374,7 @@
         }
         DeviceGuard g(p->device);
         HIP_CHECK(hipStreamSynchronize(p->search));
-        for (auto& s : p->slots) deliver(s);
+        for (int i = 0; i < N_SLOTS; ++i) deliver(p->slots[(p->next_slot + i) % N_SLOTS], p->lanes[0].t);
         for (auto& sp : p->scan) collect(p, sp, 1);
     });
 }
@@ -385,7 +393,7 @@
         for (auto& s : p->slots) busy += s.busy ? 1 : 0;
         for (int i = 0; i < N_SLOTS && busy > leave_pending; ++i) {
             QuerySlot& s = p->slots[(p->next_slot + i) % N_SLOTS];
-            if (s.busy) { deliver(s); --busy; }
+            if (s.busy) { deliver(s, p->lanes[0].t); --busy; }
         }
     });
 }
diff --git a/image_search_amd/search.py b/image_search_amd/search.py
--- a/image_search_amd/search.py
+++ b/image_search_amd/search.py
@@ -225,6 +225,12 @@
         out = (ctypes.c_uint32 * 4)()
         check(lib().mi_knn_prefilter_state(self._h, out))
         return {"skips_left": out[0], "consecutive_fallbacks": out[1], "searches_skipped": out[2], "scales_taken_at_rows": out[3]}
+
+    def chain_stats(self):
+        out = (ctypes.c_uint64 * 6)()
+        check(lib().mi_knn_chain_stats(self._h, out))
+        return {"small_selects": out[0], "wide_selects": out[1], "token_fallbacks": out[2], "full_fallbacks": out[3],
+                "last_report": (out[4], bool(out[5]))}
 
     def insert(self, embeddings: np.ndarray):
         e = _f32(embeddings).reshape(-1, self.dim)
diff --git a/include/mi355clip.h b/include/mi355clip.h
--- a/include/mi355clip.h
+++ b/include/mi355clip.h
@@ -70,6 +70,7 @@
 int mi_knn_set_option(mi_knn* t, const char* key, int value);
 int mi_knn_prefilter_stats(mi_knn* t, uint32_t* candidates, uint32_t* fell_back);
 int mi_knn_prefilter_state(mi_knn* t, uint32_t out[4]);
+int mi_knn_chain_stats(mi_knn* t, uint64_t out[6]);
 int mi_knn_reserve(mi_knn* t, uint64_t rows);
 int mi_knn_size(const mi_knn* t, uint64_t* rows);
 
```

Measured after the change: 6480 images/s (median of 6 runs). No clear change (+0.4%).
